# ndas7/Parallel-Systems-MPI-TFIDF

Measured on AMD Instinct MI355X. Metric: corpus GB/s (TF-IDF hot path: tokenize->TF->DF->tf*idf->ordered output), higher is better.
Workload: dtype u8/u32 (f64 score)

## Files before the change

include/tfidf.h:

```cpp
#ifndef TFIDF_H
#define TFIDF_H

#include <stdint.h>
#include <stddef.h>

#ifdef __cplusplus
extern "C" {
#endif

#define TFIDF_ABI_VERSION 2

enum tfidf_status {
    TFIDF_OK = 0,
    TFIDF_E_INVAL = -1,
    TFIDF_E_NOMEM = -2,
    TFIDF_E_HIP = -3,
    TFIDF_E_RCCL = -4,
    TFIDF_E_NODEV = -5,
    TFIDF_E_NOINPUT = -6,
    TFIDF_E_NODOC = -7,
    TFIDF_E_OUTPUT = -8,
    TFIDF_E_CAPACITY = -9,
    TFIDF_E_STATE = -10,
    TFIDF_E_PEER = -11,
// ... 36 lines not shown
typedef struct tfidf_ctx tfidf_ctx;

int tfidf_open(int device, tfidf_ctx** out);
int tfidf_device_count(void);
void tfidf_close(tfidf_ctx* ctx);
const char* tfidf_strerror(int status);
int tfidf_abi_version(void);

#define TFIDF_UNIQUE_ID_BYTES 128
int tfidf_comm_unique_id(uint8_t id[TFIDF_UNIQUE_ID_BYTES]);
int tfidf_comm_init(tfidf_ctx* ctx, const uint8_t id[TFIDF_UNIQUE_ID_BYTES], int rank, int nranks);

#define TFIDF_GROUP_LOCAL 1u
typedef struct tfidf_group tfidf_group;
int tfidf_group_open(int nranks, const int* devices, uint32_t flags, tfidf_group** out);
int tfidf_group_size(const tfidf_group* g);
tfidf_ctx* tfidf_group_ctx(tfidf_group* g, int rank);
int tfidf_group_run(tfidf_group* g, const tfidf_corpus* shards);
int tfidf_group_write_output(tfidf_group* g, const char* path);
void tfidf_group_close(tfidf_group* g);

int tfidf_run(tfidf_ctx* ctx, const tfidf_corpus* corpus);

int tfidf_fetch(tfidf_ctx* ctx, tfidf_result* out);
void tfidf_result_free(tfidf_result* r);

typedef struct tfidf_run_info {
    uint64_t size;
    uint64_t nbytes;
    uint64_t ntokens;
    uint64_t npairs;
    uint32_t nterms;
    uint32_t nterms_global;
    uint64_t nchunks;
    uint64_t partial_records;
    uint32_t ndocs;
    uint32_t vocab_capacity;
    double   ms_total;
    double   ms_tokcount;
    double   ms_stage[16];
    uint32_t nstages;
    uint32_t flags;
    uint64_t device_allocs;
    uint64_t device_alloc_bytes;
    uint64_t idf_logs;
    double   ms_idf_host;
    double   ms_idf_wait;
    uint32_t k1_workgroups;
    uint32_t reserved2;
} tfidf_run_info;
#define TFIDF_RUN_K1_VS   2u
#define TFIDF_RUN_K1_ST   4u
#define TFIDF_RUN_K1_SL   8u
#define TFIDF_RUN_XCHG_DENSE 16u
int tfidf_last_run_info(tfidf_ctx* ctx, tfidf_run_info* info);
typedef struct tfidf_run_totals {
    uint64_t runs;
    double ms_tokcount, ms_total;
    uint64_t idf_logs;
    double ms_idf_host, ms_idf_wait;
} tfidf_run_totals;
int tfidf_run_totals_get(tfidf_ctx* ctx, tfidf_run_totals* out, int reset);
int tfidf_alloc_stats(uint64_t* allocs, uint64_t* bytes);
int tfidf_alloc_live(uint64_t* allocs, uint64_t* bytes);
int tfidf_grid_cus(tfidf_ctx* ctx, uint32_t* ncu);
const char* tfidf_stage_name(int stage);
int tfidf_set_timing(tfidf_ctx* ctx, int enable);
int tfidf_debug_k1_stamps(tfidf_ctx* ctx, uint64_t* out, int n);

int tfidf_hbm_probe(tfidf_ctx* ctx, uint64_t nbytes, int iters, double* read_gbps, double* copy_gbps);


int tfidf_format(tfidf_ctx* ctx, uint64_t* nbytes);
int tfidf_copy_text(tfidf_ctx* ctx, uint64_t off, void* dst, uint64_t n);
int tfidf_write_output_gpu(tfidf_ctx* ctx, const char* path, int append);
typedef struct tfidf_output_info {
    uint64_t size;
    uint64_t text_bytes;
    uint32_t writers;
    uint32_t formatted;
    double   ms_prepare;
    double   ms_d2h_busy;
    double   ms_write;
    double   ms_total;
} tfidf_output_info;
int tfidf_last_output_info(const tfidf_ctx* ctx, tfidf_output_info* info);
int tfidf_format_f64(tfidf_ctx* ctx, const double* vals, uint64_t n, char* out);

int tfidf_write_output(const tfidf_result* r, const char* path);
int tfidf_print_jobs(const tfidf_result* r);


#define TFIDF_QUERY_MAX_K 1024u
#define TFIDF_QUERY_MAX_QUERIES 65536u
typedef struct tfidf_queries {
    const uint8_t*  bytes;
    uint64_t        nbytes;
    const uint64_t* q_off;
    uint32_t        nqueries;
} tfidf_queries;
typedef struct tfidf_hits {
    uint32_t  nqueries, k;
    uint32_t* nhits;
    uint64_t* nmatch;
    uint32_t* nterms_found;
    uint32_t* doc;
// ... 702 lines not shown
```

parallel-systems-mpi-tfidf_amd/csrc/engine.cpp:

```cpp
#include <hip/hip_runtime.h>
#include <rccl/rccl.h>

#include <float.h>
#include <math.h>
#include <stdio.h>
#include <stdlib.h>
#include <string.h>

#include <fcntl.h>
#include <sys/stat.h>
#include <time.h>
#include <unistd.h>

#include <algorithm>
#include <atomic>
#include <chrono>
#include <condition_variable>
#include <memory>
#include <mutex>
#include <string>
#include <thread>
#include <unordered_map>
#include <vector>

// ... 79 lines not shown
    }
    std::atomic_thread_fence(std::memory_order_acquire);
    return hipSuccess;
}

static hipError_t spin_sync(tfidf_ctx* ctx, hipStream_t s) {
    if (g_live_ctx.load() > 1) return hipStreamSynchronize(s);
    hipError_t e = hipEventRecord(ctx->ev_spin, s);
    if (e != hipSuccess) return e;
    while ((e = hipEventQuery(ctx->ev_spin)) == hipErrorNotReady) {
    }
    return e;
}

extern "C" {

int tfidf_device_count(void) {
    int n = 0;
    return hipGetDeviceCount(&n) == hipSuccess && n > 0 ? n : 0;
}

int tfidf_open(int device, tfidf_ctx** out) {
    if (!out) return TFIDF_E_INVAL;
    *out = nullptr;
    int n = 0;
    if (hipGetDeviceCount(&n) != hipSuccess || n <= 0 || device < 0 || device >= n) return TFIDF_E_NODEV;
    hipDeviceProp_t prop;
    if (hipGetDeviceProperties(&prop, device) != hipSuccess) return TFIDF_E_NODEV;
    if (strncmp(prop.gcnArchName, "gfx950", 6) != 0) {
        fprintf(stderr, "tfidf: device %d is %s, need gfx950\n", device, prop.gcnArchName);
        return TFIDF_E_NODEV;
    }
    if (hipSetDevice(device) != hipSuccess) return TFIDF_E_NODEV;
    std::unique_ptr<tfidf_ctx> ctx(new tfidf_ctx());
    ctx->device = device;
    const char* km = getenv("TFIDF_K1");
    if (km && !strcmp(km, "general")) ctx->k1_mode = 2;
    if (km && !strcmp(km, "vs")) ctx->k1_mode = 1;
    if (km && !strcmp(km, "sl")) ctx->k1_mode = 3;
    const char* ks = getenv("TFIDF_STAMPS");
    ctx->stamps_on = ks && ks[0] == '1';
    const char* kx = getenv("TFIDF_TEST_XFAIL_RANK");
    ctx->xfail_rank = kx ? atoi(kx) : -1;
    const char* kxm = getenv("TFIDF_XCHG");
    if (kxm && !strcmp(kxm, "owner")) ctx->xchg_mode = 1;
    if (kxm && !strcmp(kxm, "dense")) ctx->xchg_mode = 2;
    if (kxm && !strcmp(kxm, "dense_table")) ctx->xchg_mode = 3;
    const char* kxa = getenv("TFIDF_XAGG");
    ctx->xagg_table = kxa && !strcmp(kxa, "table");
    const char* kxb = getenv("TFIDF_XB_STAGE_MAX");
    ctx->xb_stage_max = kxb ? (uint32_t)atoi(kxb) : ~0u;
    const char* kds = getenv("TFIDF_DF_SPLIT");
    ctx->df_split = !(kds && !strcmp(kds, "0"));
    const char* kn = getenv("TFIDF_TEST_XNOMEM_RANK");
    ctx->xnomem_rank = kn ? atoi(kn) : -1;
    static_assert(K1_SL_MAX_CAP == 1ull << 25, "knobs.h: TFIDF_SL_MAXCAP's upper bound");
    for (int i = 0; i < KNOB_COUNT; ++i) {
        uint64_t v = 0;
        if (!knob_parse(kKnobs[i], getenv(kKnobs[i].name), &v)) continue;
        switch (i) {
            case KNOB_SL_MAXCAP: ctx->sl_maxcap = v; break;
            case KNOB_QUERY_ACC_MB: ctx->query_acc_bytes = v; break;
            case KNOB_TERMS_MB: ctx->terms_bytes = v; break;
            case KNOB_TRANSFORM_MB: ctx->transform_bytes = v; break;
            case KNOB_DEDUP_MB: ctx->dedup_bytes = v; break;
            case KNOB_NB_MB: ctx->nb_bytes = v; break;
            case KNOB_KMEANS_MB: ctx->kmeans_bytes = v; break;
            case KNOB_KMEANS_SPLIT: ctx->kmeans_split = (uint32_t)v; break;
            case KNOB_AN_GRID: ctx->an_grid = (uint32_t)v; break;
            case KNOB_GRID_CUS: ctx->grid_cus = (uint32_t)v; break;
            case KNOB_VCAP: ctx->vcap = v; break;
            case KNOB_VLOAD_BIG: ctx->vload_big_pct = (uint32_t)v; break;
            case KNOB_VLOAD: ctx->vload_pct = (uint32_t)v; break;
        }
    }
    HIPCHK(ctx->stream.create());
    HIPCHK(ctx->stream2.create());
    HIPCHK(ctx->stream3.create());
    for (Event* e : {&ctx->ev_fork, &ctx->ev_order, &ctx->ev_spin, &ctx->ev_idf_up, &ctx->ev_vrank, &ctx->ev_dfmain})
        HIPCHK(e->create_untimed());
    for (Event& e : ctx->ev) HIPCHK(e.create());
    if (arena_reset(ctx.get(), 64ull << 20) != 0) return TFIDF_E_NOMEM;
    if (ctx->counters.ensure(256) != 0) return TFIDF_E_NOMEM;
    if (ctx->hpin.alloc(256, hipHostMallocCoherent) != hipSuccess) return TFIDF_E_NOMEM;
    if (hipHostGetDevicePointer((void**)&ctx->hpin_dev, ctx->hpin, 0) != hipSuccess || !ctx->hpin_dev) return TFIDF_E_NOMEM;
    if (ctx->k1out_host.alloc(sizeof(K1Out)) != hipSuccess || ctx->k1out_dev.ensure(sizeof(K1Out)) != 0) return TFIDF_E_NOMEM;
    g_live_ctx.fetch_add(1);
    ctx->live = true;
    *out = ctx.release();
    return TFIDF_OK;
}

void tfidf_close(tfidf_ctx* ctx) {
    if (ctx) delete ctx;
}

int tfidf_set_timing(tfidf_ctx* ctx, int enable) {
    if (!ctx) return TFIDF_E_INVAL;
    ctx->timing = enable == 2 ? 2 : (enable != 0 ? 1 : 0);
    return TFIDF_OK;
}

const char* tfidf_stage_name(int stage) { return (stage >= 0 && stage < S_NSTAGES) ? kStageNames[stage] : "?"; }

int tfidf_comm_unique_id(uint8_t id[TFIDF_UNIQUE_ID_BYTES]) {
    ncclUniqueId u;
// ... 316 lines not shown
    if (!rc && any_long) {
        agreed = false;
        rc = exchange_long_check(ctx, V, bytes, &agreed);
    }
    if (rc && rc != TFIDF_E_PEER && !agreed) ctx->xp->abort();
    return rc;
}

static int enqueue_doc_order(tfidf_ctx* ctx, const uint32_t* dev_ids, uint32_t N, hipStream_t s2) {
    ENSURE(ctx->dkey0, (size_t)N * 8 + 8);
    ENSURE(ctx->dkey1, (size_t)N * 8 + 8);
    ENSURE(ctx->dseq0, (size_t)N * 4 + 4);
    ENSURE(ctx->dseq1, (size_t)N * 4 + 4);
    {
        const size_t need2 = (size_t)256 * 4 * ((N + 2047) / 2048 + 1) + (size_t)N * 20 + (1u << 20);
        if (need2 > ctx->arena2_buf.cap && ctx->arena2_buf.ensure(need2) != 0) return TFIDF_E_NOMEM;
        ctx->arena2.base = (uint8_t*)ctx->arena2_buf.p;
        ctx->arena2.cap = ctx->arena2_buf.cap;
        ctx->arena2.used = 0;
        HIPCHK(hipStreamWaitEvent(s2, ctx->ev_fork, 0));
        LCHK(launch_doc_keys(dev_ids, N, ctx->dkey0.as<uint64_t>(), ctx->dseq0.as<uint32_t>(), s2));
        int dc = N <= SORT_TILE_MAXN
            ? tile_sort_u64(ctx->dkey0.as<uint64_t>(), ctx->dseq0.as<uint32_t>(), ctx->dkey1.as<uint64_t>(),
                            ctx->dseq1.as<uint32_t>(), N, ctx->arena2, s2)
            : radix_sort_u64(ctx->dkey0.as<uint64_t>(), ctx->dseq0.as<uint32_t>(), ctx->dkey1.as<uint64_t>(),
                             ctx->dseq1.as<uint32_t>(), N, 0x1Fu, ctx->arena2, s2);
        LCHK(dc);
        ctx->order = dc ? ctx->dseq1.as<uint32_t>() : ctx->dseq0.as<uint32_t>();
        HIPCHK(hipEventRecord(ctx->ev_order, s2));
    }
    return 0;
}

static int run_local(tfidf_ctx* ctx, const CorpusDev& c, const uint32_t* dev_ids, uint64_t Nt) {
    hipStream_t s = ctx->stream;
    Arena& ar = ctx->arena;
    const uint32_t N = c.ndocs;
    ar.used = 0;
    ctx->run_N = N;
    ctx->run_V = 0;
    mark(ctx, S_PREP);
    HIPCHK(hipEventRecord(ctx->ev_fork, s));
    if (ctx->xp) {
        const size_t R = (size_t)ctx->nranks;
        ENSURE(ctx->x_cnt, ((R + 1) * (R + 4)) * 4);
    }
    const uint64_t span = c.hi - c.lo;
    const bool aligned = (((uintptr_t)c.bytes & 15u) == 0);
    ctx->k1_vs = aligned && ctx->k1_mode != 2;
    if (ctx->k1_vs && ctx->vcap > K1_VS_MAX_CAP) return TFIDF_E_CAPACITY;
    ctx->k1_sl = ctx->k1_vs && (ctx->k1_mode == 0 || ctx->k1_mode == 3) &&
                 ctx->vcap <= ctx->sl_maxcap;
    const uint32_t cb = ctx->k1_sl ? (ctx->vcap > K1_ST_MAX_CAP ? CHUNK_BYTES : CHUNK_BYTES_ST) : CHUNK_BYTES;
    const uint64_t nchunks = span ? (span + cb - 1) / cb : 0;
    if (ctx->rec_cap == 0) ctx->rec_cap = span / 6 + 4096;
    if (ctx->part_cap == 0) ctx->part_cap = span / 64 + 4096;
    ENSURE(ctx->chunk_start, (nchunks + 1) * 8);
    ENSURE(ctx->chunk_doc, (nchunks + 1) * 4);
    ENSURE(ctx->vkeys, ctx->vcap * 16);
    ENSURE(ctx->vrep, ctx->vcap * 8);
    ENSURE(ctx->rec_slot, ctx->rec_cap * 4);
    ENSURE(ctx->rec_cnt, ctx->rec_cap * 4);
    ENSURE(ctx->part_doc, ctx->part_cap * 4);
    ENSURE(ctx->part_slot, ctx->part_cap * 4);
    ENSURE(ctx->part_cnt, ctx->part_cap * 4);
    ENSURE(ctx->doc_recoff, (size_t)N * 8 + 8);
    ENSURE(ctx->doc_npairs, (size_t)N * 4 + 4);
    ENSURE(ctx->doc_size, (size_t)N * 4 + 4);
    ENSURE(ctx->doc_flags, (size_t)N + 1);
    unsigned long long* cnt = ctx->counters.as<unsigned long long>();
    {
        FillList fl{};
        auto add = [&](void* p, uint64_t bytes, uint32_t byte) {
            fl.p[fl.n] = p;
            fl.bytes[fl.n] = bytes;
            fl.val[fl.n] = byte * 0x01010101u;
            ++fl.n;
        };
        add(ctx->vkeys.p, ctx->vcap * 16, 0xEEu);
        add(cnt, 256, 0u);
        add(ctx->doc_npairs.p, (size_t)N * 4 + 4, 0u);
        add(ctx->doc_size.p, (size_t)N * 4 + 4, 0u);
        add(ctx->doc_flags.p, (size_t)N + 1, 0u);
        LCHK(launch_fill_multi(fl, s));
    }
    ENSURE(ctx->big_list, (size_t)BIG_LIST_CAP * 4);
    if (nchunks)
        LCHK(launch_plan_chunks(c, nchunks, cb, ctx->chunk_start.as<uint64_t>(), ctx->chunk_doc.as<uint32_t>(),
                                ctx->big_list.as<uint32_t>(), cnt + 6, s));
    mark(ctx, S_TOKCOUNT);
    VocabDev vd{ctx->vkeys.as<uint4>(), ctx->vrep.as<uint64_t>(), ctx->vcap - 1};
    K1Out o{};
    o.rec_slot = ctx->rec_slot.as<uint32_t>();
    o.rec_cnt = ctx->rec_cnt.as<uint32_t>();
    o.rec_alloc = cnt + 0;
    o.rec_cap = ctx->rec_cap;
    o.part_doc = ctx->part_doc.as<uint32_t>();
    o.part_slot = ctx->part_slot.as<uint32_t>();
    o.part_cnt = ctx->part_cnt.as<uint32_t>();
    o.part_alloc = cnt + 1;
    o.part_cap = ctx->part_cap;
    o.doc_recoff = ctx->doc_recoff.as<uint64_t>();
    o.doc_npairs = ctx->doc_npairs.as<uint32_t>();
    o.doc_size = ctx->doc_size.as<uint32_t>();
    o.doc_flags = ctx->doc_flags.as<uint8_t>();
    o.ntokens = cnt + 2;
    o.chunk_ctr = cnt + 5;
    o.chunk_shard = cnt + 16;
    o.status = (uint32_t*)(cnt + 3);
    o.stamps = nullptr;
    if (ctx->stamps_on) {
        ENSURE(ctx->stamps, 8 * K1_DEBUG_WORDS);
        HIPCHK(hipMemsetAsync(ctx->stamps.p, 0, 8 * K1_DEBUG_WORDS, s));
        o.stamps = ctx->stamps.as<unsigned long long>();
    }
    uint32_t k1_wgs = 0;
    if (nchunks && ctx->k1_sl) {
        if (!ctx->k1out_valid || memcmp(ctx->k1out_host, &o, sizeof(K1Out)) != 0) {
            ctx->k1out_valid = false;
            *ctx->k1out_host = o;
            HIPCHK(hipMemcpyAsync(ctx->k1out_dev.p, ctx->k1out_host, sizeof(K1Out), hipMemcpyHostToDevice, s));
            ctx->k1out_valid = true;
        }
        LCHK(launch_tokcount_sl(c, ctx->chunk_start.as<uint64_t>(), ctx->chunk_doc.as<uint32_t>(), 0, nchunks, vd,
                                ctx->k1out_dev.as<K1Out>(), s, ctx_ncu(ctx), &k1_wgs));
    } else if (nchunks && ctx->k1_vs)
        LCHK(launch_tokcount_vs(c, ctx->chunk_start.as<uint64_t>(), ctx->chunk_doc.as<uint32_t>(), 0, nchunks, vd, o, s,
                                ctx_ncu(ctx), &k1_wgs));
    else if (nchunks) {
        LCHK(launch_tokcount(c, ctx->chunk_start.as<uint64_t>(), ctx->chunk_doc.as<uint32_t>(), 0, nchunks, vd, o, s));
        k1_wgs = (uint32_t)nchunks;
    }
    ctx->k1_workgroups = k1_wgs;
    mark(ctx, S_VOCAB);
    const uint64_t cap = ctx->vcap;
    ENSURE(ctx->dense, (cap + 1) * 4);
    LCHK(launch_vocab_flags(vd, cap, ctx->dense.as<uint32_t>(), s));
    LCHK(scan_excl_u32(ctx->dense.as<uint32_t>(), ctx->dense.as<uint32_t>(), cap, ar, s));
    uint64_t* hp = ctx->hpin;
    {
        WordList wl{};
        for (int i = 0; i < 8; ++i) { wl.src[i] = cnt + i; wl.bytes[i] = 8; }
        wl.src[8] = ctx->dense.as<uint32_t>() + cap;
        wl.bytes[8] = 4;
        wl.n = 9;
        HIPCHK(words_wait(ctx, wl, 0, s));
    }
    const uint32_t V = (uint32_t)hp[8];
    unsigned long long hc[8];
    for (int i = 0; i < 8; ++i) hc[i] = hp[i];
    const uint64_t R_main = hc[0], Q = hc[1], nbig = hc[6];
    const uint32_t st = (uint32_t)hc[3];
    ctx->local_long = (st & ST_HAS_LONG) != 0;
    ctx->ntokens = hc[2];
    ctx->nchunks = nchunks;
    ctx->nrec_part = Q;
    if (st & (ST_VOCAB_SPIN | ST_TERM_LONG)) return TFIDF_E_CAPACITY;
    if (st & ST_LONG_COLLIDE) {
        fprintf(stderr, "tfidf: two distinct terms of 16 bytes or more share their 120-bit identity key\n");
        return TFIDF_E_CAPACITY;
    }
    bool retry = false;
    if (st & ST_BOUNDS) {
        fprintf(stderr, "tfidf: internal bounds check tripped in K1 (status 0x%x)\n", st);
        return TFIDF_E_STATE;
    }
    if (st & ST_VOCAB_FULL) {
        if (ctx->vcap >= K1_VS_MAX_CAP) return TFIDF_E_CAPACITY;
        ctx->vcap = ctx->vcap * 4 < K1_VS_MAX_CAP ? ctx->vcap * 4 : K1_VS_MAX_CAP;
        retry = true;
    }
    if (st & ST_REC_FULL) { ctx->rec_cap = R_main + R_main / 4 + 4096; retry = true; }
    if (st & ST_PART_FULL) { ctx->part_cap = Q + Q / 4 + 4096; retry = true; }
    if (retry) return 1;
    if (N > SORT_TILE_MAXN) {
        const int rc = enqueue_doc_order(ctx, dev_ids, N, ctx->stream2);
        if (rc) return rc;
    }
    ctx->V = V;
    if ((uint64_t)V * 100 > cap * (cap < VOCAB_LOW_LOAD_CAP ? ctx->vload_pct : ctx->vload_big_pct)) {
        while ((uint64_t)V * 100 > ctx->vcap * (ctx->vcap < VOCAB_LOW_LOAD_CAP ? ctx->vload_pct : ctx->vload_big_pct))
            ctx->vcap *= 2;
        if (ctx->vcap > K1_VS_MAX_CAP && cap < K1_VS_MAX_CAP) ctx->vcap = K1_VS_MAX_CAP;
        if (ctx->vcap != cap) return 1;
    }
    ENSURE(ctx->vslot, (size_t)V * 4 + 4);
    ENSURE(ctx->skey0, (size_t)V * 16 + 16);
    ENSURE(ctx->skey1, (size_t)V * 16 + 16);
    ENSURE(ctx->seq0, (size_t)V * 4 + 4);
    ENSURE(ctx->seq1, (size_t)V * 4 + 4);
    ENSURE(ctx->rank_of_slot, cap * 4);
    ENSURE(ctx->slot_of_rank, (size_t)V * 4 + 4);
    LCHK(launch_vocab_compact(vd, cap, ctx->dense.as<uint32_t>(), c, ctx->vslot.as<uint32_t>(), ctx->skey0.as<uint4>(),
                              ctx->seq0.as<uint32_t>(), s));
    if (V <= SORT_TILE_MAXN) {
        const int cur = tile_sort_u128(ctx->skey0.as<uint4>(), ctx->seq0.as<uint32_t>(), ctx->skey1.as<uint4>(),
                             ctx->seq1.as<uint32_t>(), V, ar, s);
        LCHK(cur);
        ctx->sorted_skey = cur ? ctx->skey1.as<uint4>() : ctx->skey0.as<uint4>();
        ctx->sorted_dense = cur ? ctx->seq1.as<uint32_t>() : ctx->seq0.as<uint32_t>();
    } else {
        uint32_t vm = 0;
        LCHK(key_varying_bytes_u128(ctx->skey0.as<uint4>(), V, &vm, ar, s));
        uint64_t* const ka = (uint64_t*)ctx->skey1.p;
        uint64_t* const kb = ka + V;
        uint32_t* const sa = ctx->seq0.as<uint32_t>();
        uint32_t* const sbq = ctx->seq1.as<uint32_t>();
        LCHK(launch_sortkey_half(ctx->skey0.as<uint4>(), V, nullptr, 1, ka, s));
        const int c1 = radix_sort_u64(ka, sa, kb, sbq, V, (vm >> 8) & 0xFFu, ar, s);
        LCHK(c1);
        ctx->sorted_dense = c1 ? sbq : sa;
        LCHK(launch_vocab_prefix_ties(c1 ? kb : ka, ctx->sorted_dense, ctx->skey0.as<uint4>(), V, vm & 0xFFu, ar, s));
        ctx->sorted_skey = nullptr;
        if (st & ST_HAS_LONG) {
            LCHK(launch_gather_u128(ctx->skey0.as<uint4>(), ctx->sorted_dense, V, ctx->skey1.as<uint4>(), s));
            ctx->sorted_skey = ctx->skey1.as<uint4>();
        }
    }
    if (st & ST_HAS_LONG)
        LCHK(launch_vocab_long_fixup(ctx->sorted_skey, ctx->sorted_dense, ctx->vslot.as<uint32_t>(), vd, c, V, ar, s));
    uint16_t* r16 = nullptr;
    if (V <= 65536u) { ENSURE(ctx->rank16, cap * 2); r16 = ctx->rank16.as<uint16_t>(); }
    LCHK(launch_vocab_rank(ctx->sorted_dense, ctx->vslot.as<uint32_t>(), V, ctx->rank_of_slot.as<uint32_t>(),
                           ctx->slot_of_rank.as<uint32_t>(), r16, s));
    if (N <= SORT_TILE_MAXN) {
        const int rc = enqueue_doc_order(ctx, dev_ids, N, ctx->stream2);
        if (rc) return rc;
    }
    const bool df_split = ctx->df_split && Q && R_main;
    ENSURE(ctx->df_local, (size_t)V * 4 + 4);
    ENSURE(ctx->df_global, (size_t)V * 4 + 4);
    if (df_split) {
        if (R_main + Q > ctx->rec_cap) {
            uint64_t ncap = R_main + Q + (R_main + Q) / 8 + 4096;
            if (ctx->rec_slot.grow_keep(ncap * 4, R_main * 4, s) || ctx->rec_cnt.grow_keep(ncap * 4, R_main * 4, s))
                return TFIDF_E_NOMEM;
            ctx->rec_cap = ncap;
        }
        const size_t dneed = df_hist_scratch(R_main, V);
        ENSURE(ctx->df_scratch, dneed > ctx->df_scratch_min ? dneed : ctx->df_scratch_min);
        Arena da;
        da.base = (uint8_t*)ctx->df_scratch.p;
        da.cap = ctx->df_scratch.cap;
        HIPCHK(hipEventRecord(ctx->ev_vrank, s));
        HIPCHK(hipStreamWaitEvent(ctx->stream2, ctx->ev_vrank, 0));
        const int dl = launch_df_hist(ctx->rec_slot.as<uint32_t>(), R_main, nullptr, R_main, ctx->rank_of_slot.as<uint32_t>(),
                                      r16, V, cap, (uint32_t*)(cnt + 3), ctx->df_local.as<uint32_t>(), da, ctx->stream2);
        if (dl == -2) {
            ctx->df_scratch_min = da.peak + da.peak / 2 + 4096;
            return 1;
        }
        LCHK(dl);
        HIPCHK(hipEventRecord(ctx->ev_dfmain, ctx->stream2));
    }
    if (ctx->idf_pool.busy && !ctx->idf_early && idf_done(ctx)) {
        idf_join(ctx);
        ENSURE(ctx->idf_vals, (size_t)(Nt + 1) * 8);
        HIPCHK(hipMemcpyAsync(ctx->idf_vals.p, ctx->idf_pin, (size_t)(Nt + 1) * 8, hipMemcpyHostToDevice,
                              ctx->stream3));
        HIPCHK(hipEventRecord(ctx->ev_idf_up, ctx->stream3));
        ctx->idf_pin_busy = true;
        ctx->idf_early = true;
    }
    mark(ctx, S_MERGE);
    uint64_t R_total = R_main;
    const uint32_t* merged_count = nullptr;
    {
        const uint64_t Qc = Q < (1ull << 20) ? (1ull << 20) : Q;
        ENSURE(ctx->pkey0, Qc * 8);
        ENSURE(ctx->pkey1, Qc * 8);
        ENSURE(ctx->pseq0, Qc * 4);
        ENSURE(ctx->pseq1, Qc * 4);
        ENSURE(ctx->phead, (Qc + 1) * 4);
    }
    if (Q) {
        if (R_main + Q > ctx->rec_cap) {
            uint64_t ncap = R_main + Q + (R_main + Q) / 8 + 4096;
            if (ctx->rec_slot.grow_keep(ncap * 4, R_main * 4, s) || ctx->rec_cnt.grow_keep(ncap * 4, R_main * 4, s))
                return TFIDF_E_NOMEM;
            ctx->rec_cap = ncap;
        }
        uint32_t nb = 0;
        if (nbig && V) {
            const uint64_t lim = (256ull << 20) / (4ull * V * DENSE_REP);
            uint64_t m = nbig < (uint64_t)BIG_LIST_CAP ? nbig : (uint64_t)BIG_LIST_CAP;
            nb = (uint32_t)(m < lim ? m : lim);
        }
        uint64_t Qs = Q;
        const uint32_t* scnt = ctx->part_cnt.as<uint32_t>();
        if (nb) {
            ENSURE(ctx->big_idx, (size_t)N * 4 + 4);
            ENSURE(ctx->dense_cnt, (size_t)nb * V * 4 * DENSE_REP);
            ENSURE(ctx->kcnt, Q * 4);
            uint32_t* nkeep = (uint32_t*)(cnt + 7);
            HIPCHK(hipMemsetAsync(ctx->big_idx.p, 0xFF, (size_t)N * 4 + 4, s));
            HIPCHK(hipMemsetAsync(ctx->dense_cnt.p, 0, (size_t)nb * V * 4 * DENSE_REP, s));
            LCHK(launch_set_big_idx(ctx->big_list.as<uint32_t>(), nb, ctx->big_idx.as<uint32_t>(), s));
            LCHK(launch_part_dense(ctx->part_doc.as<uint32_t>(), ctx->part_slot.as<uint32_t>(), ctx->part_cnt.as<uint32_t>(),
                                   Q, ctx->big_idx.as<uint32_t>(), ctx->rank_of_slot.as<uint32_t>(), V,
                                   ctx->dense_cnt.as<uint32_t>(), ctx->pkey0.as<uint64_t>(), ctx->pseq0.as<uint32_t>(),
// ... 6 lines not shown
            scnt = ctx->kcnt.as<uint32_t>();
        } else {
            LCHK(launch_part_keys(ctx->part_doc.as<uint32_t>(), ctx->part_slot.as<uint32_t>(),
                                  ctx->rank_of_slot.as<uint32_t>(), Q, ctx->pkey0.as<uint64_t>(),
                                  ctx->pseq0.as<uint32_t>(), s));
        }
        uint32_t* ph = ctx->phead.as<uint32_t>();
        if (Qs) {
            uint32_t pm = 0;
            {
                const uint32_t rb = V > 1 ? 32u - (uint32_t)__builtin_clz(V - 1) : 1u;
                const uint32_t db = N > 1 ? 32u - (uint32_t)__builtin_clz(N - 1) : 1u;
                for (uint32_t b = 0; b < (rb + 7) / 8; ++b) pm |= 1u << b;
                for (uint32_t b = 0; b < (db + 7) / 8; ++b) pm |= 1u << (4 + b);
            }
            int pc = Qs <= SORT_TILE_MAXN
                ? tile_sort_u64(ctx->pkey0.as<uint64_t>(), ctx->pseq0.as<uint32_t>(), ctx->pkey1.as<uint64_t>(),
                                ctx->pseq1.as<uint32_t>(), Qs, ar, s)
                : radix_sort_u64(ctx->pkey0.as<uint64_t>(), ctx->pseq0.as<uint32_t>(), ctx->pkey1.as<uint64_t>(),
                                 ctx->pseq1.as<uint32_t>(), Qs, pm, ar, s);
            LCHK(pc);
            uint64_t* pk = pc ? ctx->pkey1.as<uint64_t>() : ctx->pkey0.as<uint64_t>();
            uint32_t* ps = pc ? ctx->pseq1.as<uint32_t>() : ctx->pseq0.as<uint32_t>();
            LCHK(launch_part_heads(pk, Qs, ph, s));
            LCHK(scan_excl_u32(ph, ph, Qs, ar, s));
            LCHK(launch_part_merge(pk, ps, scnt, ph, Qs, ctx->slot_of_rank.as<uint32_t>(), R_main,
                                   ctx->rec_slot.as<uint32_t>(), ctx->rec_cnt.as<uint32_t>(),
                                   ctx->doc_recoff.as<uint64_t>(), ctx->doc_npairs.as<uint32_t>(),
                                   ctx->doc_flags.as<uint8_t>(), s));
        } else {
            HIPCHK(hipMemsetAsync(ph, 0, 4, s));
        }
        if (nb) {
            const uint64_t nt = ((uint64_t)V + 1023) / 1024;
            ENSURE(ctx->tile_cnt, (nt * nb + 1) * 4);
            LCHK(launch_dense_emit(ctx->dense_cnt.as<uint32_t>(), nb, V, ctx->big_list.as<uint32_t>(),
                                   ctx->slot_of_rank.as<uint32_t>(), R_main, ph + Qs, ctx->tile_cnt.as<uint32_t>(),
                                   ctx->rec_slot.as<uint32_t>(), ctx->rec_cnt.as<uint32_t>(),
                                   ctx->doc_recoff.as<uint64_t>(), ctx->doc_npairs.as<uint32_t>(),
                                   ctx->doc_flags.as<uint8_t>(), ar, s));
        }
        merged_count = ph + Qs;
        R_total = R_main + Q;
    }
    mark(ctx, S_DF);
    if (df_split) {
        HIPCHK(hipStreamWaitEvent(s, ctx->ev_dfmain, 0));
        LCHK(launch_df_hist(ctx->rec_slot.as<uint32_t>() + R_main, 0, merged_count, R_total - R_main,
                            ctx->rank_of_slot.as<uint32_t>(), r16, V, cap, (uint32_t*)(cnt + 3),
                            ctx->df_local.as<uint32_t>(), ar, s, true));
    } else {
        LCHK(launch_df_hist(ctx->rec_slot.as<uint32_t>(), R_main, merged_count, R_total,
                            ctx->rank_of_slot.as<uint32_t>(), r16, V, cap, (uint32_t*)(cnt + 3),
                            ctx->df_local.as<uint32_t>(), ar, s));
    }
    ctx->run_V = V;
    ctx->run_cap = cap;
    ctx->run_R_total = R_total;
    ctx->run_merged = merged_count;
    const size_t post_need = scan_scratch(Nt + 1) + (size_t)(Nt + 2) * 4 + 512 + scan_scratch(N) +
                             scan_scratch(3ull * ((N + 255) / 256) + 1);
    if (ar.cap - ar.used < post_need) {
        ar.peak = ar.used + post_need > ar.peak ? ar.used + post_need : ar.peak;
        return 1;
    }
    return 0;
}

#define IDF_POOL 8
static void idf_worker(tfidf_ctx::IdfPool* P, unsigned i) {
    uint64_t seen = 0;
    for (;;) {
        std::unique_lock<std::mutex> lk(P->mu);
        P->go.wait(lk, [&] { return P->stop || P->gen != seen; });
        if (P->stop) return;
        seen = P->gen;
        if (i >= P->active) continue;
        double* lut = P->lut;
        const uint32_t* vals = P->vals;
        const uint64_t Nt = P->Nt, n = P->n, lo = (n * i) / P->active, hi = (n * (i + 1)) / P->active;
        const uint32_t mode = P->mode;
        const auto t0 = P->t0;
        lk.unlock();
        if (mode != TFIDF_IDF_REF) {
            if (vals)
                for (uint64_t k = lo; k < hi; ++k) lut[k] = tfidf_weight_idf(mode, Nt, vals[k]);
            else
                for (uint64_t d = lo + 1; d < hi + 1; ++d) lut[d] = tfidf_weight_idf(mode, Nt, (uint32_t)d);
        } else if (vals)
            for (uint64_t k = lo; k < hi; ++k) lut[k] = log(1.0 * (double)Nt / (double)vals[k]);
        else
            for (uint64_t d = lo + 1; d < hi + 1; ++d) lut[d] = log(1.0 * (double)Nt / (double)d);
        const int64_t e = std::chrono::duration_cast<std::chrono::nanoseconds>(std::chrono::steady_clock::now() - t0).count();
        lk.lock();
        P->end_ns = e > P->end_ns ? e : P->end_ns;
        if (--P->left == 0) P->done.notify_all();
    }
}
static void idf_pool_stop(tfidf_ctx* ctx) {
    tfidf_ctx::IdfPool& P = ctx->idf_pool;
    {
        std::unique_lock<std::mutex> lk(P.mu);
        P.done.wait(lk, [&] { return P.left == 0; });
        P.stop = true;
    }
    P.go.notify_all();
    for (auto& t : P.th) t.join();
// ... 117 lines not shown
        if (idf_pin_reserve(ctx, (size_t)K + 1)) return TFIDF_E_NOMEM;
        if (K) {
            if (K < 2 * 16384) {
                const auto t0 = std::chrono::steady_clock::now();
                for (uint32_t k = 0; k < K; ++k) ctx->idf_pin[k] = log(1.0 * (double)Nt / (double)vals[k]);
                ctx->ms_idf_host = std::chrono::duration<double, std::milli>(std::chrono::steady_clock::now() - t0).count();
            } else {
                idf_post(ctx, ctx->idf_pin, Nt, vals.data(), K);
                idf_join(ctx);
            }
            HIPCHK(hipMemcpyAsync(ctx->idf_vals.p, ctx->idf_pin, (size_t)K * 8, hipMemcpyHostToDevice, s));
            ctx->idf_pin_busy = true;
        }
        ctx->idf_logs = K;
    }
    const uint64_t Pmax = R_total;
    mark(ctx, S_SCORE);
    ENSURE(ctx->out_term, Pmax * 4 + 4);
    ENSURE(ctx->out_cnt, Pmax * 4 + 4);
    ENSURE(ctx->out_score, Pmax * 8 + 8);
    ENSURE(ctx->idf_rank, (size_t)V * 8 + 8);
    ENSURE(ctx->large_list, (size_t)N * 8 + 16);
    K5Args a{};
    a.order = ctx->order;
    a.meta = ctx->doc_meta.as<uint4>();
    a.out_off = ctx->out_off.as<uint64_t>();
    a.doc_recoff = ctx->doc_recoff.as<uint64_t>();
    a.doc_npairs = ctx->doc_npairs.as<uint32_t>();
    a.doc_size = ctx->doc_size.as<uint32_t>();
    a.doc_flags = ctx->doc_flags.as<uint8_t>();
    a.rec_slot = ctx->rec_slot.as<uint32_t>();
    a.rec_cnt = ctx->rec_cnt.as<uint32_t>();
    a.rank_of_slot = ctx->rank_of_slot.as<uint32_t>();
    a.df_of_rank = df_of_run(ctx);
    a.idf_idx = full_lut ? nullptr : ctx->present.as<uint32_t>();
    a.idf = ctx->idf_vals.as<double>();
    a.idf_rank = ctx->idf_rank.as<double>();
    a.idf_by_df = (full_lut && V > (1u << 21)) ? 1u : 0u;
    a.large_list = ctx->large_list.as<uint32_t>() + 1;
    a.large_count = ctx->large_list.as<uint32_t>();
    a.cls_nblk = (N + 255) / 256;
    a.cls_list = ctx->large_list.as<uint32_t>() + N + 2;
    ENSURE(ctx->cls_off, ((size_t)3 * a.cls_nblk + 8) * 4);
    a.cls_off = ctx->cls_off.as<uint32_t>();
    {
        const uint64_t cap_t = 2 * R_total / 4096 + 64;
        ENSURE(ctx->split_tasks, cap_t * 8 + 8);
        a.split_count = ctx->split_tasks.as<uint32_t>();
        a.split_tasks = ctx->split_tasks.as<uint2>() + 1;
        a.split_cap = (uint32_t)(cap_t < 0xFFFFFFFFull ? cap_t : 0xFFFFFFFFull);
    }
    a.ndocs = N;
    a.nterms = V;
    a.rank_bits = V > 1 ? 32u - (uint32_t)__builtin_clz(V - 1) : 1u;
    a.rec_total = R_total;
    a.slot_cap = cap;
    a.status = (uint32_t*)(cnt + 3);
    a.out_term = ctx->out_term.as<uint32_t>();
    a.out_cnt = ctx->out_cnt.as<uint32_t>();
    a.out_score = ctx->out_score.as<double>();
    XCHK(launch_score_order(a, ar, s, ctx->stream2, ctx->ev_fork, ctx->ev_order, ctx_ncu(ctx)));
    mark(ctx, S_NSTAGES);
    {
        WordList wl{};
        wl.src[0] = cnt + 3;
        wl.bytes[0] = 4;
        wl.src[1] = ctx->out_off.as<uint64_t>() + N;
        wl.bytes[1] = 8;
        wl.src[2] = cnt + 12;
        wl.bytes[2] = 4;
        wl.n = ctx->xp ? 3 : 2;
        if (ctx->xp) {
            XCHK(launch_words_to_host(wl, ctx->hpin_dev + 24, s));
            XSYNC(s);
        } else {
            HIPCHK(words_wait(ctx, wl, 24, s));
        }
    }
    ctx->idf_pin_busy = false;
    const uint32_t st_end = (uint32_t)ctx->hpin[24];
    const uint64_t P = ctx->hpin[25];
    ctx->npairs = P;
    if (ctx->xp) ctx->Vg = (uint32_t)ctx->hpin[26];
    if (st_end & ST_BOUNDS) {
        fprintf(stderr, "tfidf: internal bounds check tripped (status 0x%x)\n", st_end);
        return TFIDF_E_STATE;
    }
    return 0;
}

static int run_once(tfidf_ctx* ctx, const CorpusDev& c, const uint32_t* dev_ids, uint64_t Nt) {
    int rc = run_local(ctx, c, dev_ids, Nt);
    mark(ctx, S_EXCHANGE);
    if (ctx->xp) {
        rc = exchange_df(ctx, rc, ctx->run_V, c.bytes);
        if (rc) return rc;
    } else {
        if (rc) return rc;
        ctx->Vg = ctx->run_V;
    }
    return run_post(ctx, Nt);
}

static int run_prepare(tfidf_ctx* ctx, const tfidf_corpus* in, CorpusDev& c, const uint32_t*& dev_ids, uint64_t& Nt) {
    if (in->ndocs && !in->doc_off) return TFIDF_E_INVAL;
    if (in->nbytes && !in->bytes) return TFIDF_E_INVAL;
    HIPCHK(hipSetDevice(ctx->device));
// ... 160 lines not shown
    }
    if (!rc) {
        *read_gbps = ms_r > 0 ? (double)nbytes * iters / (ms_r * 1e-3) / 1e9 : 0.0;
        *copy_gbps = ms_c > 0 ? 2.0 * (double)nbytes * iters / (ms_c * 1e-3) / 1e9 : 0.0;
    }
    (void)hipEventDestroy(e0);
    (void)hipEventDestroy(e1);
    (void)hipStreamSynchronize(s);
    return rc;
}

extern "C" int tfidf_grid_cus(tfidf_ctx* ctx, uint32_t* ncu) {
    if (!ctx || !ncu) return TFIDF_E_INVAL;
    *ncu = ctx_ncu(ctx);
    return TFIDF_OK;
}

extern "C" int tfidf_alloc_stats(uint64_t* allocs, uint64_t* bytes) {
    if (!allocs || !bytes) return TFIDF_E_INVAL;
    *allocs = g_dev_allocs.load(std::memory_order_relaxed);
    *bytes = g_dev_alloc_bytes.load(std::memory_order_relaxed);
    return TFIDF_OK;
}

extern "C" int tfidf_alloc_live(uint64_t* allocs, uint64_t* bytes) {
    if (!allocs || !bytes) return TFIDF_E_INVAL;
    *allocs = g_dev_allocs.load(std::memory_order_relaxed) - g_dev_frees.load(std::memory_order_relaxed);
    *bytes = g_dev_alloc_bytes.load(std::memory_order_relaxed) - g_dev_free_bytes.load(std::memory_order_relaxed);
    return TFIDF_OK;
}

extern "C" int tfidf_last_run_info(tfidf_ctx* ctx, tfidf_run_info* out) {
    tfidf_run_info* info = out;
    if (!ctx || !info || info->size < 16) return TFIDF_E_INVAL;
    if (!ctx->have_info) return TFIDF_E_STATE;
    const size_t want = info->size < sizeof(tfidf_run_info) ? (size_t)info->size : sizeof(tfidf_run_info);
    tfidf_run_info full;
    memset(&full, 0, sizeof(full));
    info = &full;
    info->nbytes = ctx->run_nbytes;
    info->ntokens = ctx->ntokens;
    info->npairs = ctx->info_npairs;
    info->nterms = ctx->info_V;
    info->nterms_global = ctx->Vg;
    info->nchunks = ctx->nchunks;
    info->partial_records = ctx->nrec_part;
    info->ndocs = ctx->ndocs;
    info->vocab_capacity = (uint32_t)ctx->vcap;
    info->ms_total = ctx->ms_total;
    info->ms_tokcount = ctx->ms_stage[S_TOKCOUNT];
    for (int i = 0; i < S_NSTAGES; ++i) info->ms_stage[i] = ctx->ms_stage[i];
    info->nstages = S_NSTAGES;
    info->flags = (ctx->k1_vs ? TFIDF_RUN_K1_VS : 0u) | (ctx->k1_sl ? TFIDF_RUN_K1_SL : 0u) |
                  (ctx->xp && ctx->last_dense ? TFIDF_RUN_XCHG_DENSE : 0u);
    info->device_allocs = g_dev_allocs.load(std::memory_order_relaxed);
    info->device_alloc_bytes = g_dev_alloc_bytes.load(std::memory_order_relaxed);
    info->idf_logs = ctx->idf_logs;
    info->ms_idf_host = ctx->ms_idf_host;
    info->ms_idf_wait = ctx->ms_idf_wait;
    info->k1_workgroups = ctx->k1_workgroups;
    full.size = want;
    memcpy(out, &full, want);
    return TFIDF_OK;
}


extern "C" void tfidf_result_free(tfidf_result* r) {
    if (!r) return;
    free(r->pair_doc); free(r->pair_term); free(r->pair_count); free(r->pair_docsize); free(r->pair_df);
    free(r->pair_score); free(r->doc_id); free(r->doc_size); free(r->term_off); free(r->term_bytes);
    free(r->term_df);
    memset(r, 0, sizeof(*r));
}

extern "C" int tfidf_fetch(tfidf_ctx* ctx, tfidf_result* r) {
    if (!ctx || !r) return TFIDF_E_INVAL;
    if (!ctx->have_result) return TFIDF_E_STATE;
    HIPCHK(hipSetDevice(ctx->device));
    hipStream_t s = ctx->stream;
    memset(r, 0, sizeof(*r));
    const uint64_t P = ctx->npairs;
    const uint32_t N = ctx->ndocs, V = ctx->V;
    r->npairs = P;
    r->ndocs = N;
    r->nterms = V;
    r->ndocs_total = ctx->ndocs_total;
    size_t p4 = (size_t)P * 4 + 4;
    r->pair_doc = (uint32_t*)malloc(p4);
    r->pair_term = (uint32_t*)malloc(p4);
    r->pair_count = (uint32_t*)malloc(p4);
    r->pair_docsize = (uint32_t*)malloc(p4);
    r->pair_df = (uint32_t*)malloc(p4);
    r->pair_score = (double*)malloc((size_t)P * 8 + 8);
    r->doc_id = (uint32_t*)malloc((size_t)N * 4 + 4);
    r->doc_size = (uint32_t*)malloc((size_t)N * 4 + 4);
    r->term_df = (uint32_t*)malloc((size_t)V * 4 + 4);
    r->term_off = (uint64_t*)malloc(((size_t)V + 1) * 8);
    if (!r->pair_doc || !r->pair_term || !r->pair_count || !r->pair_docsize || !r->pair_df || !r->pair_score ||
        !r->doc_id || !r->doc_size || !r->term_df || !r->term_off) {
        tfidf_result_free(r);
        return TFIDF_E_NOMEM;
    }
    std::vector<uint32_t> order(N);
    std::vector<uint64_t> ooff((size_t)N + 1);
    if (P) {
        HIPCHK(hipMemcpyAsync(r->pair_term, ctx->out_term.p, P * 4, hipMemcpyDeviceToHost, s));
// ... 380 lines not shown
```

parallel-systems-mpi-tfidf_amd/csrc/engine_ctx.h:

```cpp
#ifndef TFIDF_ENGINE_CTX_H
#define TFIDF_ENGINE_CTX_H

#include <hip/hip_runtime.h>

#include <stdio.h>
#include <stdlib.h>
#include <string.h>

#include <chrono>
#include <condition_variable>
#include <mutex>
#include <thread>
#include <vector>

#include "../../include/tfidf.h"
#include "kernels.h"
#include "xport.h"
#include "devbuf.h"

struct Stream {
    hipStream_t s = nullptr;
    Stream() = default;
    Stream(const Stream&) = delete;
    Stream& operator=(const Stream&) = delete;
// ... 13 lines not shown
};
template <typename T> struct Pinned {
    T* p = nullptr;
    Pinned() = default;
    Pinned(const Pinned&) = delete;
    Pinned& operator=(const Pinned&) = delete;
    ~Pinned() { release(); }
    operator T*() const { return p; }
    T* operator->() const { return p; }
    hipError_t alloc(size_t bytes, unsigned flags = hipHostMallocDefault) {
        release();
        const hipError_t e = hipHostMalloc((void**)&p, bytes, flags);
        if (e != hipSuccess) p = nullptr;
        return e;
    }
    void release() {
        if (p) (void)hipHostFree(p);
        p = nullptr;
    }
};
enum Stage { S_PREP, S_TOKCOUNT, S_VOCAB, S_MERGE, S_DF, S_EXCHANGE, S_IDF, S_ORDER, S_SCORE, S_NSTAGES };

struct tfidf_ctx {
    ~tfidf_ctx();
    bool live = false;
    int device = 0;
    Stream stream;
    Xport* xp = nullptr;
    int rank = 0, nranks = 1;
    int timing = 1;
    int k1_mode = 0;
    bool stamps_on = false;
    int xfail_rank = -1;
    int xnomem_rank = -1;
    DevBuf stamps;
    bool k1_vs = false;
    bool k1_sl = false;
    uint64_t sl_maxcap = K1_SL_MAX_CAP;
    Pinned<K1Out> k1out_host;
    DevBuf k1out_dev;
    bool k1out_valid = false;
    Event ev[S_NSTAGES + 1];
    Arena arena;
    DevBuf arena_buf;
    Stream stream2;
    Event ev_fork, ev_order;
    Event ev_spin;
    uint64_t wait_token = 0;
    Stream stream3;
    Event ev_idf_up;
    bool idf_early = false;
    bool df_split = true;
    Event ev_vrank, ev_dfmain;
    DevBuf df_scratch;
    size_t df_scratch_min = 0;
    Arena arena2;
    DevBuf arena2_buf;
    DevBuf in_bytes, in_off, in_ids;
    DevBuf syn_bytes, syn_off, syn_ids, syn_ntok, syn_blkfirst, syn_blkbytes, syn_cdf;
    DevBuf chunk_start, chunk_doc;
    DevBuf vkeys, vrep;
    uint64_t vcap = 1ull << 20;
#define VOCAB_LOW_LOAD_CAP (1ull << 24)
#define IDF_FULL_MAX (1ull << 18)
    uint32_t vload_pct = 12;
    uint32_t vload_big_pct = 45;
    DevBuf rec_slot, rec_cnt;
    uint64_t rec_cap = 0;
    DevBuf part_doc, part_slot, part_cnt;
    uint64_t part_cap = 0;
    DevBuf doc_recoff, doc_npairs, doc_size, doc_flags;
    DevBuf counters;
    Pinned<uint64_t> hpin;
    uint64_t* hpin_dev = nullptr;
    DevBuf dense, vslot, skey0, skey1, seq0, seq1, rank_of_slot, slot_of_rank, rank16;
    DevBuf pkey0, pkey1, pseq0, pseq1, phead;
    DevBuf big_list, big_idx, dense_cnt, kcnt, tile_cnt;
    DevBuf df_local, df_global, present, idf_vals;
    uint64_t idf_full_n = 0;
    Pinned<double> idf_pin;
    size_t idf_pin_n = 0;
    bool idf_pin_busy = false;
    struct IdfPool {
        std::mutex mu;
        std::condition_variable go, done;
        std::vector<std::thread> th;
        uint64_t gen = 0;
        bool stop = false, busy = false;
        unsigned active = 0, left = 0;
        double* lut = nullptr;
        uint64_t Nt = 0;
        const uint32_t* vals = nullptr;
        uint64_t n = 0;
        uint32_t mode = 0;
        std::chrono::steady_clock::time_point t0;
        int64_t end_ns = 0;
    } idf_pool;
    uint64_t idf_logs = 0;
    tfidf_run_totals totals{};
    double ms_idf_host = 0, ms_idf_wait = 0;
    DevBuf dkey0, dkey1, dseq0, dseq1, npairs_ord, out_off, doc_meta;
    DevBuf out_term, out_cnt, out_score, idf_rank, large_list, split_tasks, cls_off;
    DevBuf x_mine, x_srec, x_sidx, x_back, x_cnt;
    DevBuf x_rrec, x_rslot, x_reply, x_tkey, x_tdf;
    DevBuf x_gkeys, x_pos, x_dense;
    DevBuf x_lloc, x_lsend, x_lgath, x_ltab;
// ... 298 lines not shown
```

parallel-systems-mpi-tfidf_amd/csrc/finalize.hip:

```cpp
#include "dev_common.h"
#include "dev_vocab.h"
#include "kernels.h"
#include "synth.h"

#include <type_traits>
#define G(p) ((GLOBAL_AS std::remove_pointer_t<decltype(p)>*)(p))
template <class T> __device__ __forceinline__ void sto(T* p, T v) { *(GLOBAL_AS T*)p = v; }

namespace {
constexpr int NT = 256;
inline unsigned grid_for(uint64_t n, int nt = NT) { return n ? (unsigned)((n + nt - 1) / nt) : 1u; }
inline int ok() { return hipGetLastError() == hipSuccess ? 0 : -1; }

__device__ __forceinline__ uint4 u128_from(uint64_t lo, uint64_t hi) {
    return make_uint4((uint32_t)lo, (uint32_t)(lo >> 32), (uint32_t)hi, (uint32_t)(hi >> 32));
}
__device__ __forceinline__ bool u128_eq(uint4 a, uint4 b) { return a.x == b.x && a.y == b.y && a.z == b.z && a.w == b.w; }
}


__global__ void k_vocab_flags(VocabDev v, uint64_t cap, uint32_t* __restrict__ flags) {
    uint64_t s = (uint64_t)blockIdx.x * blockDim.x + threadIdx.x;
    if (s >= cap) return;
    uint4 k = v.keys[s];
// ... 585 lines not shown
    uint32_t v[4], c = 0;
#pragma unroll
    for (int k = 0; k < 4; ++k) {
        v[k] = r0 + k < V ? dense_sum(dense, b, V, r0 + k) : 0u;
        c += v[k] ? 1u : 0u;
    }
    uint32_t tot;
    uint32_t o = block_excl_scan<NT, false>(c, wsum, &tot);
    const uint64_t base = rec_base + *merged_count + tile_off[(uint64_t)b * nt + t];
#pragma unroll
    for (int k = 0; k < 4; ++k)
        if (v[k]) { rec_slot[base + o] = r0 + k; rec_cnt[base + o] = v[k]; ++o; }
    if (t == 0 && threadIdx.x == 0) {
        const uint32_t d = big_list[b];
        const uint64_t first = tile_off[(uint64_t)b * nt], last = tile_off[(uint64_t)(b + 1) * nt];
        doc_recoff[d] = rec_base + *merged_count + first;
        doc_npairs[d] = (uint32_t)(last - first);
        doc_flags[d] = DF_PARTIAL | DF_PRESORTED;
    }
}
__global__ void k_add_count(uint32_t* __restrict__ merged_count, const uint32_t* __restrict__ add) {
    merged_count[0] += add[0];
}
int launch_dense_emit(const uint32_t* dense, uint32_t nb, uint32_t V, const uint32_t* big_list,
                      const uint32_t* slot_of_rank, uint64_t rec_base, uint32_t* merged_count, uint32_t* tile_cnt,
                      uint32_t* rec_slot, uint32_t* rec_cnt, uint64_t* doc_recoff, uint32_t* doc_npairs,
                      uint8_t* doc_flags, Arena& ar, hipStream_t s) {
    if (!nb || !V) return 0;
    const uint32_t nt = (V + DENSE_TILE - 1) / DENSE_TILE;
    const dim3 grid(nt, nb);
    k_dense_count<<<grid, NT, 0, s>>>(dense, V, nt, tile_cnt);
    if (ok()) return -1;
    if (scan_excl_u32(tile_cnt, tile_cnt, (uint64_t)nt * nb, ar, s)) return -1;
    k_dense_write<<<grid, NT, 0, s>>>(dense, V, nt, big_list, slot_of_rank, rec_base, merged_count, tile_cnt, rec_slot,
                                      rec_cnt, doc_recoff, doc_npairs, doc_flags);
    if (ok()) return -1;
    k_add_count<<<1, 1, 0, s>>>(merged_count, tile_cnt + (uint64_t)nt * nb);
    return ok();
}


constexpr uint32_t DFH_ROUNDS = 4;

constexpr int DFH_NT = 1024;
#ifndef DFH_B_N
#define DFH_B_N 16
#endif
constexpr int DFH_B = DFH_B_N;
#ifndef DFH_CK_BITS
#define DFH_CK_BITS 12
#endif
constexpr uint32_t DFH_CK = 1u << DFH_CK_BITS;
__device__ __forceinline__ uint32_t dfh_cslot(uint32_t slot) { return (slot * 0x9E3779B1u) >> (32 - DFH_CK_BITS); }
template <bool WIDE>
__global__ __launch_bounds__(DFH_NT) void k_df_hist_lds(uint32_t* __restrict__ rec_slot, uint64_t nrec,
                                                        const uint32_t* __restrict__ nrec_extra,
                                                        const uint32_t* __restrict__ rank_of_slot,
                                                        const uint16_t* __restrict__ rank16, uint32_t V,
                                                        uint64_t slot_cap, uint64_t ranked_from,
                                                        uint32_t* __restrict__ status, uint64_t per,
                                                        uint32_t* __restrict__ part ,
                                                        uint32_t* __restrict__ df) {
    extern __shared__ __attribute__((aligned(16))) uint32_t bins[];
    const uint32_t W = (V + 1) / 2;
    for (uint32_t k = threadIdx.x; k < W; k += DFH_NT) bins[k] = 0;
    unsigned long long* cache = reinterpret_cast<unsigned long long*>(bins + ((W + 1) & ~1u));
    for (uint32_t k = threadIdx.x; k < DFH_CK; k += DFH_NT) cache[k] = 0ull;
    __syncthreads();
    if (nrec_extra) nrec += *nrec_extra;
    const uint64_t r0 = (uint64_t)blockIdx.x * per;
    const uint64_t r1 = r0 + per < nrec ? r0 + per : nrec;
    const uint32_t nr = r1 > r0 ? (uint32_t)(r1 - r0) : 0u;
    const uint32_t rk = ranked_from <= r0 ? 0u : ranked_from - r0 >= nr ? nr : (uint32_t)(ranked_from - r0);
    const __amdgpu_buffer_rsrc_t rs = __builtin_amdgcn_make_buffer_rsrc((void*)(rec_slot + r0), 0, (int)(nr * 4u),
                                                                        0x00020000);
    const __amdgpu_buffer_rsrc_t ms = __builtin_amdgcn_make_buffer_rsrc(
        rank16 ? (void*)rank16 : (void*)rank_of_slot, 0,
        (int)(slot_cap * (rank16 ? 2u : 4u) < 0x7FFFFFF0ull ? slot_cap * (rank16 ? 2u : 4u) : 0x7FFFFFF0ull), 0x00020000);
    uint32_t rp[DFH_B];
    uint32_t pofs = 0xFFFFFFF0u;
    uint32_t pvalid = 0;
#pragma unroll
    for (int q = 0; q < DFH_B; ++q) rp[q] = 0u;
    auto store_prev = [&]() {
#pragma unroll
        for (int q = 0; q < DFH_B; ++q)
            __builtin_amdgcn_raw_buffer_store_b32(rp[q], rs,
                                                  ((pvalid >> q) & 1u) ? pofs + (uint32_t)q * DFH_NT * 4u : 0xFFFFFFF0u,
                                                  0, 2 );
    };
    for (uint32_t j = threadIdx.x; j < nr; j += (uint32_t)DFH_B * DFH_NT) {
        uint32_t sl[DFH_B], r[DFH_B], g[DFH_B];
        const uint32_t ofs = j * 4u;
#pragma unroll
        for (int q = 0; q < DFH_B; ++q) {
            const uint32_t v = __builtin_amdgcn_raw_buffer_load_b32(rs, ofs + (uint32_t)q * DFH_NT * 4u, 0, 2 );
            sl[q] = j + (uint32_t)q * DFH_NT < nr ? v : 0xFFFFFFFFu;
        }
        store_prev();
        uint32_t miss = 0;
#pragma unroll
        for (int q = 0; q < DFH_B; ++q) {
            const bool ranked = j + (uint32_t)q * DFH_NT >= rk;
            if (sl[q] != 0xFFFFFFFFu && sl[q] >= (ranked ? (uint64_t)V : slot_cap)) {
                atomicOr(status, ST_BOUNDS);
                sl[q] = 0xFFFFFFFFu;
            }
            const unsigned long long e = cache[dfh_cslot(sl[q])];
            const bool hit = (uint32_t)(e >> 32) == sl[q] + 1u;
            const bool need = sl[q] != 0xFFFFFFFFu && !ranked && !hit;
            miss |= need ? 1u << q : 0u;
            r[q] = ranked ? sl[q] : (uint32_t)e;
        }
        if (rank16) {
#pragma unroll
            for (int q = 0; q < DFH_B; ++q)
                g[q] = __builtin_amdgcn_raw_buffer_load_b16(ms, ((miss >> q) & 1u) ? sl[q] * 2u : 0u, 0, 0);
        } else {
#pragma unroll
            for (int q = 0; q < DFH_B; ++q)
                g[q] = __builtin_amdgcn_raw_buffer_load_b32(ms, ((miss >> q) & 1u) ? sl[q] * 4u : 0u, 0, 0);
        }
#pragma unroll
        for (int q = 0; q < DFH_B; ++q) {
            if ((miss >> q) & 1u) {
                r[q] = g[q];
                cache[dfh_cslot(sl[q])] = ((unsigned long long)(sl[q] + 1u) << 32) | r[q];
            }
        }
        pvalid = 0;
#pragma unroll
        for (int q = 0; q < DFH_B; ++q) {
            rp[q] = r[q];
            pvalid |= sl[q] != 0xFFFFFFFFu && j + (uint32_t)q * DFH_NT < rk ? 1u << q : 0u;
            if (sl[q] == 0xFFFFFFFFu) continue;
            const uint32_t sh = 16 * (r[q] & 1);
            if (WIDE) {
                const uint32_t old = atomicAdd(&bins[r[q] >> 1], 1u << sh);
                if (((old >> sh) & 0xFFFFu) == 0x7FFFu) {
                    atomicSub(&bins[r[q] >> 1], 0x8000u << sh);
                    atomicAdd(&df[r[q]], 0x8000u);
                }
            } else {
                atomicAdd(&bins[r[q] >> 1], 1u << sh);
            }
        }
        pofs = ofs;
    }
    store_prev();
    __syncthreads();
    uint32_t* out = part + (uint64_t)blockIdx.x * W;
    for (uint32_t k = threadIdx.x; k < W; k += DFH_NT) out[k] = bins[k];
}
constexpr uint32_t DFC_G = 32;
__global__ void k_df_colsum(const uint32_t* __restrict__ part, uint32_t nparts, uint32_t V, uint32_t* __restrict__ df) {
    const uint32_t r = blockIdx.x * blockDim.x + threadIdx.x;
    if (r >= V) return;
    const uint32_t W = (V + 1) / 2, sh = 16 * (r & 1);
    const uint32_t p0 = blockIdx.y * DFC_G;
    uint32_t v[DFC_G];
#pragma unroll
    for (uint32_t q = 0; q < DFC_G; ++q)
        v[q] = p0 + q < nparts ? part[(uint64_t)(p0 + q) * W + (r >> 1)] : 0u;
    uint32_t sum = 0;
#pragma unroll
    for (uint32_t q = 0; q < DFC_G; ++q) sum += (v[q] >> sh) & 0xFFFFu;
    if (sum) atomicAdd(&df[r], sum);
}
constexpr int DFA_B = 8;
__global__ void k_df_hist_atomic(uint32_t* __restrict__ rec_slot, uint64_t nrec, const uint32_t* __restrict__ nrec_extra,
                                 const uint32_t* __restrict__ rank_of_slot, uint64_t slot_cap, uint64_t ranked_from,
                                 uint32_t V, uint32_t* __restrict__ status, uint32_t* __restrict__ df) {
    if (nrec_extra) nrec += *nrec_extra;
    const uint64_t stride = (uint64_t)gridDim.x * blockDim.x;
    for (uint64_t i0 = (uint64_t)blockIdx.x * blockDim.x + threadIdx.x; i0 < nrec; i0 += stride * DFA_B) {
        uint32_t sl[DFA_B], r[DFA_B];
#pragma unroll
        for (int k = 0; k < DFA_B; ++k) {
            const uint64_t i = i0 + (uint64_t)k * stride;
            sl[k] = i < nrec ? rec_slot[i] : 0xFFFFFFFFu;
        }
#pragma unroll
        for (int k = 0; k < DFA_B; ++k) {
            const bool ranked = i0 + (uint64_t)k * stride >= ranked_from;
            r[k] = ranked ? sl[k] : sl[k] < slot_cap ? rank_of_slot[sl[k]] : 0xFFFFFFFFu;
        }
// ... 80 lines not shown
    for (uint32_t i0 = b + threadIdx.x; i0 < e; i0 += B * DFS_NT) {
        uint32_t r[B];
#pragma unroll
        for (int q = 0; q < B; ++q) r[q] = i0 + q * DFS_NT < e ? part[i0 + q * DFS_NT] : 0xFFFFFFFFu;
#pragma unroll
        for (int q = 0; q < B; ++q)
            if (r[q] != 0xFFFFFFFFu) atomicAdd(&sbins[r[q] - s0], 1u);
    }
    __syncthreads();
    for (uint32_t j = threadIdx.x; j < sw; j += DFS_NT) df[s0 + j] = accumulate ? df[s0 + j] + sbins[j] : sbins[j];
}

static void df_lds_plan(uint64_t nrec_max, uint32_t V, uint64_t* per_out, uint32_t* nparts_out) {
    uint64_t nparts = (nrec_max + DFH_RECS - 1) / DFH_RECS;
    const uint32_t W = (V + 1) / 2;
    static int ncu = 0;
    if (!ncu) {
        int dev = 0;
        if (hipGetDevice(&dev) != hipSuccess ||
            hipDeviceGetAttribute(&ncu, hipDeviceAttributeMultiprocessorCount, dev) != hipSuccess || ncu <= 0)
            ncu = 256;
    }
    const uint64_t wg_lds = (uint64_t)((W + 1) & ~1u) * 4 + (uint64_t)DFH_CK * 8;
    const uint64_t per_cu = (uint64_t)163840 / wg_lds >= 2 ? 2 : 1;
    const uint64_t slots = (uint64_t)ncu * per_cu;
    uint64_t full = (nparts + slots - 1) / slots * slots;
    if (full > DFH_ROUNDS * slots) full = slots;
    const char* fe = getenv("TFIDF_DF_WGS");
    const uint64_t forced = fe ? strtoull(fe, nullptr, 0) : 0ull;
    if (forced >= 1 && forced <= (1u << 20)) full = forced;
    uint64_t per = (nrec_max + full - 1) / full;
    if (per < 8192u && !forced) per = 8192u;
    if (per > (1u << 28)) per = 1u << 28;
    if (per == 0) per = 1;
    *per_out = per;
    *nparts_out = (uint32_t)((nrec_max + per - 1) / per);
}

size_t df_hist_scratch(uint64_t nrec_max, uint32_t V) {
    if (V == 0 || nrec_max == 0) return 256;
    if (V <= DFH_MAXV) {
        uint64_t per = 0;
        uint32_t nparts = 0;
        df_lds_plan(nrec_max, V, &per, &nparts);
        return (size_t)nparts * ((V + 1) / 2) * 4 + 256;
    }
    const uint64_t nsl = ((uint64_t)V + DFS_SLICE - 1) / DFS_SLICE;
    const uint64_t ntiles = (nrec_max + DFS_TILE - 1) / DFS_TILE;
    return (size_t)((ntiles * nsl + 1) * 4 + nrec_max * 4 + (ntiles * nsl) / 16 + 8192 + 1024);
}

int launch_df_hist(uint32_t* rec_slot, uint64_t nrec, const uint32_t* nrec_extra, uint64_t nrec_max,
                   const uint32_t* rank_of_slot, const uint16_t* rank16, uint32_t V, uint64_t slot_cap,
                   uint32_t* status, uint32_t* df, Arena& ar, hipStream_t s, bool accumulate) {
    const uint64_t ranked_from = nrec;
    if (V == 0) return 0;
    if (nrec_max < nrec) nrec_max = nrec;
    if (nrec_max == 0)
        return accumulate ? 0 : hipMemsetAsync(df, 0, (size_t)V * 4, s) == hipSuccess ? 0 : -1;
    if (V <= DFH_MAXV) {
        uint64_t per = 0;
        uint32_t nparts = 0;
        df_lds_plan(nrec_max, V, &per, &nparts);
        const uint32_t W = (V + 1) / 2;
        size_t m = ar.mark();
        uint32_t* part = (uint32_t*)ar.get((size_t)nparts * W * 4);
        if (!part) return -2;
        if (!accumulate && hipMemsetAsync(df, 0, (size_t)V * 4, s) != hipSuccess) return -1;
        const size_t lds = (size_t)((W + 1) & ~1u) * 4 + (size_t)DFH_CK * 8;
        if (per > DFH_RECS)
            k_df_hist_lds<true><<<nparts, DFH_NT, lds, s>>>(rec_slot, nrec, nrec_extra, rank_of_slot, rank16, V,
                                                            slot_cap, ranked_from, status, per, part, df);
        else
            k_df_hist_lds<false><<<nparts, DFH_NT, lds, s>>>(rec_slot, nrec, nrec_extra, rank_of_slot, rank16, V,
                                                             slot_cap, ranked_from, status, per, part, df);
        k_df_colsum<<<dim3(grid_for(V), (nparts + DFC_G - 1) / DFC_G), NT, 0, s>>>(part, nparts, V, df);
        ar.release(m);
        return ok();
    }
    {
        const uint32_t nsl = (uint32_t)(((uint64_t)V + DFS_SLICE - 1) / DFS_SLICE);
        const uint64_t ntiles = (nrec_max + DFS_TILE - 1) / DFS_TILE;
        if (nsl <= DFS_MAXSL && nrec_max < (1ull << 32) && ntiles * nsl < (1ull << 31)) {
            size_t m = ar.mark();
            uint32_t* cnt = (uint32_t*)ar.get((size_t)(ntiles * nsl + 1) * 4);
            uint32_t* part = (uint32_t*)ar.get((size_t)nrec_max * 4);
            if (!cnt || !part) return -2;
            {
                k_dfs_count<<<(uint32_t)ntiles, DFS_NT, 0, s>>>(rec_slot, nrec, nrec_extra, rank_of_slot, slot_cap,
                                                               ranked_from, V, nsl, status, cnt);
                if (ok()) return -1;
                if (scan_excl_u32(cnt, cnt, ntiles * nsl, ar, s)) return -1;
                k_dfs_scatter<<<(uint32_t)ntiles, DFS_NT, 0, s>>>(rec_slot, nrec, nrec_extra, V, nsl, cnt, part);
                if (ok()) return -1;
                k_dfs_slice<<<nsl, DFS_NT, (size_t)(V < DFS_SLICE ? V : DFS_SLICE) * 4, s>>>(part, cnt, (uint32_t)ntiles,
                                                                                           V, df, accumulate);
                ar.release(m);
                return ok();
            }
        }
    }
    if (!accumulate && hipMemsetAsync(df, 0, (size_t)V * 4, s) != hipSuccess) return -1;
    k_df_hist_atomic<<<4096, NT, 0, s>>>(rec_slot, nrec, nrec_extra, rank_of_slot, slot_cap, ranked_from, V, status,
                                         df);
    return ok();
}

__global__ void k_df_mark(const uint32_t* __restrict__ df, uint32_t V, uint32_t* __restrict__ present) {
    uint32_t r = blockIdx.x * blockDim.x + threadIdx.x;
    if (r < V) present[df[r]] = 1u;
}
int launch_df_mark(const uint32_t* df, uint32_t V, uint32_t* present, hipStream_t s) {
    if (!V) return 0;
    k_df_mark<<<grid_for(V), NT, 0, s>>>(df, V, present);
    return ok();
}
__global__ void k_df_list(const uint32_t* __restrict__ ps, uint64_t nvals, uint32_t* __restrict__ vals) {
    const uint64_t stride = (uint64_t)gridDim.x * blockDim.x;
    for (uint64_t x = (uint64_t)blockIdx.x * blockDim.x + threadIdx.x; x < nvals; x += stride)
        if (ps[x + 1] != ps[x]) vals[ps[x]] = (uint32_t)x;
}
int launch_df_list(const uint32_t* present_scan, uint64_t nvals, uint32_t* vals, hipStream_t s) {
    const unsigned full = grid_for(nvals), cap = 1u << 20;
    k_df_list<<<full < cap ? full : cap, NT, 0, s>>>(present_scan, nvals, vals);
    return ok();
}


__global__ void k_doc_keys(const uint32_t* __restrict__ ids, uint32_t n, uint64_t* __restrict__ keys,
                           uint32_t* __restrict__ seq) {
    uint32_t i = blockIdx.x * blockDim.x + threadIdx.x;
    if (i >= n) return;
    uint32_t id = ids ? ids[i] : i + 1;
    uint32_t dg[10];
    int k = 0;
    do { dg[k++] = id % 10; id /= 10; } while (id);
    uint64_t key = 0;
    for (int p = 0; p < 10; ++p) key = key * 11 + (p < k ? dg[k - 1 - p] : 10u);
    keys[i] = key;
    seq[i] = i;
}
int launch_doc_keys(const uint32_t* doc_ids, uint32_t ndocs, uint64_t* keys, uint32_t* seq, hipStream_t s) {
    if (!ndocs) return 0;
    k_doc_keys<<<grid_for(ndocs), NT, 0, s>>>(doc_ids, ndocs, keys, seq);
    return ok();
}
__global__ void k_gather_meta(const uint32_t* __restrict__ order, const uint32_t* __restrict__ np,
                              const uint64_t* __restrict__ recoff, const uint32_t* __restrict__ dsize,
                              const uint8_t* __restrict__ flags, uint32_t n, uint64_t* __restrict__ out,
                              uint4* __restrict__ meta) {
    uint32_t i = blockIdx.x * blockDim.x + threadIdx.x;
    if (i >= n) return;
    const uint32_t d = order[i];
    const uint32_t c = np[d];
    const uint64_t rb = c ? recoff[d] : 0ull;
    out[i] = c;
    meta[i] = make_uint4((uint32_t)rb, (uint32_t)(rb >> 32), (c & 0x3FFFFFFFu) | ((uint32_t)(flags[d] & 3u) << 30), dsize[d]);
}
int launch_gather_meta(const uint32_t* order, const uint32_t* doc_npairs, const uint64_t* doc_recoff,
                       const uint32_t* doc_size, const uint8_t* doc_flags, uint32_t ndocs, uint64_t* npairs_ord,
// ... 6 lines not shown


constexpr int K5_MAX = K5_MAX_PAIRS;
constexpr uint32_t K5_SMALL = 64;
constexpr int K5_BATCH = 8;
#ifndef K5_EB
#define K5_EB 4
#endif
#ifndef K5_EMIT
#define K5_EMIT 2
#endif
#ifndef K5_WPS
#define K5_WPS 4
#endif
#ifndef K5_WPS_WIDE
#define K5_WPS_WIDE 4
#endif
constexpr uint32_t K5_NB = 1u << K5_NB_BITS;
#ifndef K5L_EB
#define K5L_EB 8
#endif

__global__ void k_idf_of_rank(const uint32_t* __restrict__ df_of_rank, const uint32_t* __restrict__ idf_idx,
                              const double* __restrict__ idf, uint32_t V, double* __restrict__ out) {
    uint32_t r = blockIdx.x * blockDim.x + threadIdx.x;
    if (r < V) out[r] = idf_idx ? idf[idf_idx[df_of_rank[r]]] : idf[df_of_rank[r]];
}

template <bool BYDF>
__device__ __forceinline__ double k5_idf(const K5Args& a, uint32_t r) {
    if constexpr (BYDF) return G(a.idf)[G(a.df_of_rank)[r]];
    else return G(a.idf_rank)[r];
}

template <bool BYDF>
__device__ __forceinline__ void k5_emit(const K5Args& a, uint64_t o, double ds, uint32_t rank, uint32_t cnt) {
    const double tf = (double)cnt / ds;
    sto(&a.out_term[o], (uint32_t)(rank));
    sto(&a.out_cnt[o], (uint32_t)(cnt));
    sto(&a.out_score[o], (double)(tf * k5_idf<BYDF>(a, rank)));
}

__device__ __forceinline__ uint32_t k5_rank(const K5Args& a, uint32_t r) {
    if (r >= a.nterms) { atomicOr(a.status, ST_BOUNDS); r = 0; }
    return r;
}

constexpr uint32_t K5_WIDE_BITS = 32 - K5_IDX_BITS + K5_NB_BITS;
__device__ __forceinline__ bool k5_by_wave(const K5Args& a, uint32_t n, bool presorted) {
    if (presorted) return n <= K5_WAVE;
    return n <= K5_SMALL || (n <= K5_WAVE && a.rank_bits <= K5_WIDE_BITS);
}

__device__ __noinline__ void k5_radix(uint32_t rank_bits, const uint32_t* rec_cnt, const double* idf_rank,
                                      uint32_t* out_term, uint32_t* out_cnt, double* out_score, uint32_t* buf0,
                                      uint32_t* buf1, uint32_t* h, uint32_t n, uint64_t rb, uint64_t ob, double ds) {
    const uint32_t lane = threadIdx.x & 63;
    const uint64_t below = (1ull << lane) - 1ull;
    uint32_t cur = 0;
    for (uint32_t sh = K5_IDX_BITS; sh < K5_IDX_BITS + rank_bits; sh += 8) {
        const uint32_t* src = cur ? buf1 : buf0;
        uint32_t* dst = cur ? buf0 : buf1;
        h[4 * lane] = 0; h[4 * lane + 1] = 0; h[4 * lane + 2] = 0; h[4 * lane + 3] = 0;
        __builtin_amdgcn_fence(__ATOMIC_RELEASE, "wavefront");
        __builtin_amdgcn_fence(__ATOMIC_ACQUIRE, "wavefront");
        for (uint32_t j = lane; j < n; j += 64) atomicAdd(&h[(src[j] >> sh) & 0xFFu], 1u);
        __builtin_amdgcn_fence(__ATOMIC_RELEASE, "wavefront");
        __builtin_amdgcn_fence(__ATOMIC_ACQUIRE, "wavefront");
        {
            const uint32_t v0 = h[4 * lane], v1 = h[4 * lane + 1], v2 = h[4 * lane + 2], v3 = h[4 * lane + 3];
            const uint32_t tot = v0 + v1 + v2 + v3;
            const uint32_t ex = wave_incl_scan(tot) - tot;
            h[4 * lane] = ex; h[4 * lane + 1] = ex + v0; h[4 * lane + 2] = ex + v0 + v1; h[4 * lane + 3] = ex + v0 + v1 + v2;
        }
        __builtin_amdgcn_fence(__ATOMIC_RELEASE, "wavefront");
        __builtin_amdgcn_fence(__ATOMIC_ACQUIRE, "wavefront");
        for (uint32_t r0 = 0; r0 < n; r0 += 64) {
            const uint32_t j = r0 + lane;
            const bool valid = j < n;
            const uint32_t key = valid ? src[j] : 0u;
            const uint32_t dg = (key >> sh) & 0xFFu;
            uint64_t m = __ballot(valid);
#pragma unroll
            for (int b = 0; b < 8; ++b) {
                const bool bit = (dg >> b) & 1u;
                const uint64_t bb = __ballot(valid && bit);
                m &= bit ? bb : ~bb;
            }
            const uint32_t lrank = (uint32_t)__popcll(m & below);
            const uint32_t cnt = (uint32_t)__popcll(m);
            const uint32_t base = valid ? h[dg] : 0u;
            __builtin_amdgcn_fence(__ATOMIC_RELEASE, "wavefront");
            __builtin_amdgcn_fence(__ATOMIC_ACQUIRE, "wavefront");
            if (valid) {
                dst[base + lrank] = key;
                if (lrank == cnt - 1u) h[dg] = base + cnt;
            }
            __builtin_amdgcn_fence(__ATOMIC_RELEASE, "wavefront");
            __builtin_amdgcn_fence(__ATOMIC_ACQUIRE, "wavefront");
        }
        cur ^= 1u;
    }
    const uint32_t* fin = cur ? buf1 : buf0;
    for (uint32_t j0 = 0; j0 < n; j0 += 64 * K5_BATCH) {
        uint32_t key[K5_BATCH], cnt[K5_BATCH];
        double idf[K5_BATCH];
#pragma unroll
        for (int q = 0; q < K5_BATCH; ++q) {
            const uint32_t j = j0 + 64 * q + lane;
            key[q] = j < n ? fin[j] : 0u;
        }
#pragma unroll
        for (int q = 0; q < K5_BATCH; ++q) {
            cnt[q] = rec_cnt[rb + (key[q] & ((1u << K5_IDX_BITS) - 1u))];
            idf[q] = G(idf_rank)[key[q] >> K5_IDX_BITS];
        }
#pragma unroll
        for (int q = 0; q < K5_BATCH; ++q) {
            const uint32_t j = j0 + 64 * q + lane;
            if (j < n) {
                sto(&out_term[ob + j], (uint32_t)(key[q] >> K5_IDX_BITS));
                sto(&out_cnt[ob + j], (uint32_t)(cnt[q]));
                sto(&out_score[ob + j], (double)(((double)cnt[q] / ds) * idf[q]));
            }
        }
    }
}

constexpr int K5_PF = 8;
constexpr int K5_RQ = K5_WAVE / 64;
__device__ __forceinline__ void k5_prefetch(const K5Args& a, const uint4& m, uint32_t lane, uint32_t (&s)[K5_PF],
                                            uint32_t (&c)[K5_PF]) {
    const uint32_t n = m.z & 0x3FFFFFFFu;
    const uint64_t rb = ((uint64_t)m.y << 32) | m.x;
    const bool ok = n != 0u && n <= K5_WAVE && rb + n <= a.rec_total;
#pragma unroll
    for (int q = 0; q < K5_PF; ++q) {
        const uint32_t j = 64u * q + lane;
        const bool v = ok && j < n;
        s[q] = v ? a.rec_slot[rb + j] : 0u;
        c[q] = v ? a.rec_cnt[rb + j] : 0u;
    }
}

__device__ __forceinline__ uint32_t lane_id_fresh() {
    uint32_t l;
    asm volatile("v_mbcnt_lo_u32_b32 %0, -1, 0\n\tv_mbcnt_hi_u32_b32 %0, -1, %0" : "=v"(l));
    return l;
}

template <bool WIDE, bool BYDF>
__global__ __launch_bounds__(NT, WIDE ? K5_WPS_WIDE : K5_WPS) void k_score_wave(K5Args a) {
    static_assert(WIDE || !BYDF, "idf by df only with wide ranks (V > 2^21; k5_radix reads idf by rank)");
    __shared__ __attribute__((aligned(16))) uint32_t kb[NT / 64][2][K5_WAVE];
    __shared__ uint32_t hist[NT / 64][K5_NB];
    const uint32_t w = threadIdx.x >> 6, lane = threadIdx.x & 63;
    const uint32_t stride = gridDim.x * (NT / 64);
    uint32_t* buf0 = kb[w][0];
    uint32_t* buf1 = kb[w][1];
    uint32_t* h = hist[w];
    const uint32_t* L = nullptr;
    uint32_t lcount = a.ndocs;
    if (a.cls_list) {
        const uint32_t lo = G(a.cls_off)[a.cls_nblk];
        L = a.cls_list + lo;
        lcount = G(a.cls_off)[2 * a.cls_nblk] - lo;
    }
    auto pos_of = [&](uint32_t li) -> uint32_t { return L ? G(L)[li] : li; };
    uint32_t li = blockIdx.x * (NT / 64) + w;
    uint32_t i_cur = li < lcount ? pos_of(li) : 0u;
    uint32_t i_nxt = li + stride < lcount ? pos_of(li + stride) : 0u;
    uint4 m_cur = li < lcount ? gload(a.meta + (i_cur)) : make_uint4(0, 0, 0, 0);
    uint4 m_nxt = li + stride < lcount ? gload(a.meta + (i_nxt)) : make_uint4(0, 0, 0, 0);
    uint64_t ob_cur = li < lcount ? G(a.out_off)[i_cur] : 0ull;
    uint32_t s_cur[K5_PF], c_cur[K5_PF];
    k5_prefetch(a, m_cur, lane, s_cur, c_cur);
    for (; li < lcount; li += stride) {
        const uint32_t lane = lane_id_fresh();
        const uint32_t i = i_cur;
        const uint4 mc = m_cur;
        const uint64_t ob = ob_cur;
        const uint32_t n = mc.z & 0x3FFFFFFFu;
        const bool presorted = ((mc.z >> 30) & DF_PRESORTED) != 0;
        const uint64_t rb = ((uint64_t)mc.y << 32) | mc.x;
        const double ds = (double)mc.w;
        const bool small_doc = n != 0u && k5_by_wave(a, n, presorted) && rb + n <= a.rec_total;
        uint32_t r[K5_RQ];
#pragma unroll
        for (int q = 0; q < K5_PF; ++q) {
            const uint32_t j = 64u * q + lane;
            r[q] = (small_doc && j < n) ? k5_rank(a, s_cur[q]) : 0xFFFFFFFFu;
            if (small_doc && j < n) buf0[j] = c_cur[q];
        }
        if (small_doc && n > 64u * K5_PF) {
            uint32_t sx[K5_RQ - K5_PF];
#pragma unroll
            for (int q = K5_PF; q < K5_RQ; ++q) {
                const uint32_t j = 64u * q + lane;
                sx[q - K5_PF] = j < n ? a.rec_slot[rb + j] : 0u;
                if (j < n) buf0[j] = a.rec_cnt[rb + j];
            }
#pragma unroll
            for (int q = K5_PF; q < K5_RQ; ++q) {
                const uint32_t j = 64u * q + lane;
                r[q] = j < n ? k5_rank(a, sx[q - K5_PF]) : 0xFFFFFFFFu;
            }
        } else {
#pragma unroll
            for (int q = K5_PF; q < K5_RQ; ++q) r[q] = 0xFFFFFFFFu;
        }
        __builtin_amdgcn_fence(__ATOMIC_RELEASE, "wavefront");
        __builtin_amdgcn_fence(__ATOMIC_ACQUIRE, "wavefront");
        {
            const uint32_t inx = li + stride;
            m_cur = m_nxt;
            i_cur = i_nxt;
            ob_cur = inx < lcount ? G(a.out_off)[i_cur] : 0ull;
            i_nxt = inx + stride < lcount ? pos_of(inx + stride) : 0u;
            m_nxt = inx + stride < lcount ? gload(a.meta + (i_nxt)) : make_uint4(0, 0, 0, 0);
            k5_prefetch(a, m_cur, lane, s_cur, c_cur);
        }
        if (n == 0) continue;
        if (!k5_by_wave(a, n, presorted)) {
            if (WIDE && lane == 0) G(a.large_list)[atomicAdd(a.large_count, 1u)] = i;
            continue;
        }
        if (rb + n > a.rec_total) { if (lane == 0) atomicOr(a.status, ST_BOUNDS); continue; }
        if (presorted) {
#pragma unroll
            for (int q = 0; q < K5_RQ; ++q) {
                const uint32_t j = 64u * q + lane;
                if (j < n) k5_emit<BYDF>(a, ob + j, ds, r[q], buf0[j]);
            }
            continue;
        }
#ifndef K5_CNT
#define K5_CNT 128
#endif
        if (n <= (uint32_t)K5_CNT) {
            constexpr int QC = K5_CNT / 64;
#pragma unroll
            for (int q = 0; q < QC; ++q) {
                const uint32_t j = 64u * q + lane;
                if (j < n) buf1[j] = r[q];
            }
            const uint32_t n4 = (n + 3u) & ~3u;
            if (lane < 4u && n + lane < n4) buf1[n + lane] = 0xFFFFFFFFu;
            __builtin_amdgcn_fence(__ATOMIC_RELEASE, "wavefront");
            __builtin_amdgcn_fence(__ATOMIC_ACQUIRE, "wavefront");
            uint32_t pos[QC];
#pragma unroll
            for (int q = 0; q < QC; ++q) pos[q] = 0u;
            const uint4* k4p = reinterpret_cast<const uint4*>(buf1);
            for (uint32_t i4 = 0; i4 < n4 / 4u; ++i4) {
                const uint4 k4 = k4p[i4];
#pragma unroll
                for (int q = 0; q < QC; ++q)
                    pos[q] += (k4.x < r[q] ? 1u : 0u) + (k4.y < r[q] ? 1u : 0u) + (k4.z < r[q] ? 1u : 0u) +
                              (k4.w < r[q] ? 1u : 0u);
            }
            double idf[QC];
#pragma unroll
            for (int q = 0; q < QC; ++q) idf[q] = (64u * q + lane < n) ? k5_idf<BYDF>(a, r[q]) : 0.0;
#pragma unroll
            for (int q = 0; q < QC; ++q) {
                const uint32_t j = 64u * q + lane;
                if (j < n) {
                    const uint64_t o = ob + pos[q];
                    const uint32_t cnt = buf0[j];
                    sto(&a.out_term[o], (uint32_t)(r[q]));
                    sto(&a.out_cnt[o], (uint32_t)(cnt));
                    sto(&a.out_score[o], (double)(((double)cnt / ds) * idf[q]));
                }
            }
            __builtin_amdgcn_fence(__ATOMIC_RELEASE, "wavefront");
            __builtin_amdgcn_fence(__ATOMIC_ACQUIRE, "wavefront");
            continue;
        }
        if (n <= K5_SMALL) {
            uint32_t key = r[0], val = lane < n ? buf0[lane] : 0u;
#pragma unroll
            for (uint32_t k = 2; k <= 64; k <<= 1) {
#pragma unroll
                for (uint32_t j = k >> 1; j > 0; j >>= 1) {
                    uint32_t pk = __shfl_xor(key, j, 64), pv = __shfl_xor(val, j, 64);
                    bool take_min = ((lane & k) == 0) == ((lane & j) == 0);
                    if (take_min ? (pk < key) : (pk > key)) { key = pk; val = pv; }
                }
            }
            if (lane < n) k5_emit<BYDF>(a, ob + lane, ds, key, val);
            continue;
        }
        const uint32_t hsh = a.rank_bits > K5_NB_BITS ? a.rank_bits - K5_NB_BITS : 0u;
#pragma unroll
        for (uint32_t q = 0; q < K5_NB / 64; ++q) h[q * 64 + lane] = 0;
        __builtin_amdgcn_fence(__ATOMIC_RELEASE, "wavefront");
        __builtin_amdgcn_fence(__ATOMIC_ACQUIRE, "wavefront");
#pragma unroll
        for (int q = 0; q < K5_RQ; ++q)
            if (64u * q + lane < n) atomicAdd(&h[r[q] >> hsh], 1u);
        __builtin_amdgcn_fence(__ATOMIC_RELEASE, "wavefront");
        __builtin_amdgcn_fence(__ATOMIC_ACQUIRE, "wavefront");
        uint32_t gmax;
        {
            constexpr uint32_t PER = K5_NB / 64;
            uint32_t v[PER], tot = 0, mx = 0;
#pragma unroll
            for (uint32_t q = 0; q < PER; ++q) { v[q] = h[lane * PER + q]; tot += v[q]; mx = v[q] > mx ? v[q] : mx; }
            uint32_t run = wave_incl_scan(tot) - tot;
#pragma unroll
            for (uint32_t q = 0; q < PER; ++q) { h[lane * PER + q] = run; run += v[q]; }
            gmax = wave_max(mx);
        }
        __builtin_amdgcn_fence(__ATOMIC_RELEASE, "wavefront");
        __builtin_amdgcn_fence(__ATOMIC_ACQUIRE, "wavefront");
        const bool wide = WIDE;
        if (gmax > K5_GROUP_MAX && wide) {
            if (lane == 0) G(a.large_list)[atomicAdd(a.large_count, 1u)] = i;
            continue;
        }
        if constexpr (WIDE) if (wide) {
            const uint32_t lm = (1u << hsh) - 1u;
#pragma unroll
            for (int q = 0; q < K5_RQ; ++q) {
                const uint32_t j = 64u * q + lane;
                if (j < n) buf1[atomicAdd(&h[r[q] >> hsh], 1u)] = ((r[q] & lm) << K5_IDX_BITS) | j;
            }
            __builtin_amdgcn_fence(__ATOMIC_RELEASE, "wavefront");
            __builtin_amdgcn_fence(__ATOMIC_ACQUIRE, "wavefront");
            constexpr int EB = K5_EB;
#pragma unroll
            for (int q0 = 0; q0 < K5_RQ; q0 += EB) {
                if (64u * q0 >= n) continue;
                uint32_t pos[EB], cnt[EB];
                double idf[EB];
#pragma unroll
                for (int e = 0; e < EB; ++e) {
                    const uint32_t j = 64u * (q0 + e) + lane;
                    const uint32_t rk = r[q0 + e];
                    pos[e] = 0u;
                    cnt[e] = 0u;
                    if (j < n) {
                        const uint32_t d = rk >> hsh, k = ((rk & lm) << K5_IDX_BITS) | j;
                        const uint32_t gs = d ? h[d - 1] : 0u, ge = h[d];
                        uint32_t less = 0;
                        for (uint32_t f = gs; f < ge; ++f) less += buf1[f] < k ? 1u : 0u;
                        pos[e] = gs + less;
                        cnt[e] = buf0[j];
                    }
                    idf[e] = j < n ? k5_idf<BYDF>(a, rk) : 0.0;
                }
#pragma unroll
                for (int e = 0; e < EB; ++e) {
                    if (64u * (q0 + e) + lane < n) {
                        const uint64_t o = ob + pos[e];
                        sto(&a.out_term[o], (uint32_t)(r[q0 + e]));
                        sto(&a.out_cnt[o], (uint32_t)(cnt[e]));
                        sto(&a.out_score[o], (double)(((double)cnt[e] / ds) * idf[e]));
                    }
                }
            }
            __builtin_amdgcn_fence(__ATOMIC_RELEASE, "wavefront");
            __builtin_amdgcn_fence(__ATOMIC_ACQUIRE, "wavefront");
            continue;
        }
        if (gmax > K5_GROUP_MAX) {
#pragma unroll
            for (int q = 0; q < K5_RQ; ++q) {
                const uint32_t j = 64u * q + lane;
                if (j < n) buf0[j] = (r[q] << K5_IDX_BITS) | j;
            }
            __builtin_amdgcn_fence(__ATOMIC_RELEASE, "wavefront");
            __builtin_amdgcn_fence(__ATOMIC_ACQUIRE, "wavefront");
            if constexpr (!WIDE)
                k5_radix(a.rank_bits, a.rec_cnt, a.idf_rank, a.out_term, a.out_cnt, a.out_score, buf0, buf1, h, n,
                         rb, ob, ds);
            continue;
        }
#pragma unroll
        for (int q = 0; q < K5_RQ; ++q) {
            const uint32_t j = 64u * q + lane;
            if (j < n) buf1[atomicAdd(&h[r[q] >> hsh], 1u)] = (r[q] << K5_IDX_BITS) | j;
        }
        __builtin_amdgcn_fence(__ATOMIC_RELEASE, "wavefront");
        __builtin_amdgcn_fence(__ATOMIC_ACQUIRE, "wavefront");
        uint32_t pp[K5_RQ];
#pragma unroll
        for (int q = 0; q < K5_RQ; ++q) {
            const uint32_t j = 64u * q + lane;
            pp[q] = 0u;
            if (j < n) {
                const uint32_t k = (r[q] << K5_IDX_BITS) | j, d = r[q] >> hsh;
                const uint32_t gs = d ? h[d - 1] : 0u, ge = h[d];
                uint32_t less = 0;
                for (uint32_t f = gs; f < ge; ++f) less += buf1[f] < k ? 1u : 0u;
                pp[q] = gs + less;
            }
        }
        __builtin_amdgcn_fence(__ATOMIC_RELEASE, "wavefront");
        __builtin_amdgcn_fence(__ATOMIC_ACQUIRE, "wavefront");
#pragma unroll
        for (int q = 0; q < K5_RQ; ++q)
            if (64u * q + lane < n) buf1[pp[q]] = (r[q] << K5_IDX_BITS) | (64u * q + lane);
        __builtin_amdgcn_fence(__ATOMIC_RELEASE, "wavefront");
        __builtin_amdgcn_fence(__ATOMIC_ACQUIRE, "wavefront");
        constexpr int EB = K5_EMIT;
        for (uint32_t j0 = 0; j0 < n; j0 += 64 * EB) {
            double idf[EB];
#pragma unroll
            for (int q = 0; q < EB; ++q) {
                const uint32_t j = j0 + 64 * q + lane;
                idf[q] = k5_idf<BYDF>(a, (j < n ? buf1[j] : 0u) >> K5_IDX_BITS);
            }
#pragma unroll
            for (int q = 0; q < EB; ++q) {
                const uint32_t j = j0 + 64 * q + lane;
                if (j < n) {
                    const uint32_t key = buf1[j], cnt = buf0[key & ((1u << K5_IDX_BITS) - 1u)];
                    sto(&a.out_term[ob + j], (uint32_t)(key >> K5_IDX_BITS));
                    sto(&a.out_cnt[ob + j], (uint32_t)(cnt));
                    sto(&a.out_score[ob + j], (double)(((double)cnt / ds) * idf[q]));
                }
            }
        }
        __builtin_amdgcn_fence(__ATOMIC_RELEASE, "wavefront");
        __builtin_amdgcn_fence(__ATOMIC_ACQUIRE, "wavefront");
    }
}

template <uint32_t MAXN, uint32_t NBB, bool BYDF>
__global__ __launch_bounds__(NT) void k_score_large(K5Args a) {
    constexpr uint32_t NB = 1u << NBB;
    __shared__ uint32_t kbuf[2][MAXN];
    __shared__ uint32_t vbuf[2][MAXN];
    union Scratch {
        struct {
            uint32_t hist[256], run[256];
            uint32_t wcnt[NT / 64][256];
        } r;
        uint32_t bh[NB];
    };
    __shared__ Scratch U;
    uint32_t (&hist)[256] = U.r.hist;
    uint32_t (&run)[256] = U.r.run;
    uint32_t (&wcnt)[NT / 64][256] = U.r.wcnt;
    uint32_t (&bh)[NB] = U.bh;
    __shared__ uint32_t wsum[NT / 64];
    __shared__ uint32_t bmax;
    const uint32_t tid = threadIdx.x, lane = tid & 63, w = tid >> 6;
    const uint32_t* LL = a.large_list;
    uint32_t nlarge;
    if (a.cls_list) {
        const uint32_t lo = G(a.cls_off)[2 * a.cls_nblk];
        LL = a.cls_list + lo;
        nlarge = G(a.cls_off)[3 * a.cls_nblk] - lo;
    } else {
        nlarge = *a.large_count;
    }
    for (uint32_t li = blockIdx.x; li < nlarge; li += gridDim.x) {
    const uint32_t i = G(LL)[li];
    const uint32_t d = G(a.order)[i];
    const uint32_t n = G(a.doc_npairs)[d];
    const bool presorted = (G(a.doc_flags)[d] & DF_PRESORTED) != 0;
    if (MAXN < (uint32_t)K5_MAX ? (!presorted && n > MAXN) : (presorted || n <= (uint32_t)K5_MAX / 2)) continue;
    const uint64_t ob = G(a.out_off)[i], rb = G(a.doc_recoff)[d];
    const double ds = (double)G(a.doc_size)[d];
    if (rb + n > a.rec_total) {
        if (tid == 0) atomicOr(a.status, ST_BOUNDS);
        continue;
    }
    if (presorted || n > (uint32_t)K5_MAX) {
        if (n > (uint32_t)K5_MAX && !presorted) { if (tid == 0) atomicOr(a.status, ST_BOUNDS); continue; }
        for (uint32_t j0 = 0; j0 < n; j0 += NT * K5L_EB) {
            uint32_t rk[K5L_EB], cn[K5L_EB];
            double f[K5L_EB];
#pragma unroll
            for (int e = 0; e < K5L_EB; ++e) {
                const uint32_t j = j0 + NT * e + tid;
                rk[e] = j < n ? a.rec_slot[rb + j] : 0u;
                cn[e] = j < n ? a.rec_cnt[rb + j] : 0u;
            }
#pragma unroll
            for (int e = 0; e < K5L_EB; ++e) {
                const uint32_t j = j0 + NT * e + tid;
                if (j < n) rk[e] = k5_rank(a, rk[e]);
                f[e] = j < n ? k5_idf<BYDF>(a, rk[e]) : 0.0;
            }
#pragma unroll
            for (int e = 0; e < K5L_EB; ++e) {
                const uint32_t j = j0 + NT * e + tid;
                if (j < n) {
                    sto(&a.out_term[ob + j], (uint32_t)(rk[e]));
                    sto(&a.out_cnt[ob + j], (uint32_t)(cn[e]));
                    sto(&a.out_score[ob + j], (double)(((double)cn[e] / ds) * f[e]));
                }
            }
        }
        continue;
    }
    for (uint32_t j0 = 0; j0 < n; j0 += NT * K5L_EB) {
        uint32_t sl[K5L_EB], cn[K5L_EB];
#pragma unroll
        for (int e = 0; e < K5L_EB; ++e) {
            const uint32_t j = j0 + NT * e + tid;
            sl[e] = j < n ? a.rec_slot[rb + j] : 0u;
            cn[e] = j < n ? a.rec_cnt[rb + j] : 0u;
        }
#pragma unroll
        for (int e = 0; e < K5L_EB; ++e) {
            const uint32_t j = j0 + NT * e + tid;
            if (j < n) {
                kbuf[0][j] = k5_rank(a, sl[e]);
                vbuf[0][j] = cn[e];
            }
        }
    }
    {
        const uint32_t hsh = a.rank_bits > NBB ? a.rank_bits - NBB : 0u;
        for (uint32_t q = tid; q < NB; q += NT) bh[q] = 0u;
        if (tid == 0) bmax = 0u;
        __syncthreads();
        for (uint32_t j = tid; j < n; j += NT) atomicAdd(&bh[kbuf[0][j] >> hsh], 1u);
        __syncthreads();
        constexpr uint32_t PER = NB / NT;
        uint32_t v[PER], tot = 0, mx = 0;
#pragma unroll
        for (uint32_t q = 0; q < PER; ++q) { v[q] = bh[tid * PER + q]; tot += v[q]; mx = v[q] > mx ? v[q] : mx; }
        uint32_t all;
        uint32_t run = block_excl_scan<NT>(tot, wsum, &all);
#pragma unroll
        for (uint32_t q = 0; q < PER; ++q) { bh[tid * PER + q] = run; run += v[q]; }
        mx = wave_max(mx);
        if (lane == 0) atomicMax(&bmax, mx);
        __syncthreads();
        if (bmax <= K5L_GROUP_MAX) {
            for (uint32_t j = tid; j < n; j += NT) {
                const uint32_t k = kbuf[0][j];
                const uint32_t q = atomicAdd(&bh[k >> hsh], 1u);
                kbuf[1][q] = k;
                vbuf[1][q] = j;
            }
            __syncthreads();
            for (uint32_t p0 = 0; p0 < n; p0 += NT * K5L_EB) {
                uint32_t kk[K5L_EB], ps[K5L_EB], cn[K5L_EB];
                double f[K5L_EB];
#pragma unroll
                for (int e = 0; e < K5L_EB; ++e) {
                    const uint32_t p = p0 + NT * e + tid;
                    kk[e] = 0u; ps[e] = 0u; cn[e] = 0u;
                    if (p < n) {
                        const uint32_t k = kbuf[1][p], d = k >> hsh;
                        const uint32_t gs = d ? bh[d - 1] : 0u, ge = bh[d];
                        uint32_t less = 0;
                        for (uint32_t g = gs; g < ge; ++g) less += kbuf[1][g] < k ? 1u : 0u;
                        kk[e] = k;
                        ps[e] = gs + less;
                        cn[e] = vbuf[0][vbuf[1][p]];
                    }
                    f[e] = p < n ? k5_idf<BYDF>(a, kk[e]) : 0.0;
                }
#pragma unroll
                for (int e = 0; e < K5L_EB; ++e) {
                    if (p0 + NT * e + tid < n) {
                        const uint64_t o = ob + ps[e];
                        sto(&a.out_term[o], (uint32_t)(kk[e]));
                        sto(&a.out_cnt[o], (uint32_t)(cn[e]));
// ... 69 lines not shown
    if (threadIdx.x < 3) c3[threadIdx.x] = 0u;
    __syncthreads();
    const uint32_t i = blockIdx.x * 256u + threadIdx.x;
    const uint32_t c = k5_class(a, i);
    if (c >= 1u && c <= 3u) atomicAdd(&c3[c - 1u], 1u);
    if (c == 4u) {
        const uint32_t n = gload(a.meta + (i)).z & 0x3FFFFFFFu;
        const uint32_t nt = (n + K5_PS_SPLIT - 1) / K5_PS_SPLIT;
        const uint32_t b = atomicAdd(a.split_count, nt);
        for (uint32_t k = 0; k < nt; ++k) {
            if (b + k < a.split_cap) a.split_tasks[b + k] = make_uint2(i, k);
            else atomicOr(a.status, ST_BOUNDS);
        }
    }
    __syncthreads();
    if (threadIdx.x < 3) a.cls_off[threadIdx.x * a.cls_nblk + blockIdx.x] = c3[threadIdx.x];
    if (blockIdx.x == 0 && threadIdx.x == 3) a.cls_off[3 * a.cls_nblk] = 0u;
}
__global__ __launch_bounds__(256) void k_k5_scatter(K5Args a) {
    __shared__ uint32_t wc[4][3];
    const uint32_t i = blockIdx.x * 256u + threadIdx.x, lane = threadIdx.x & 63, w = threadIdx.x >> 6;
    const uint32_t c = k5_class(a, i);
    uint32_t rk = 0;
#pragma unroll
    for (uint32_t k = 1; k <= 3; ++k) {
        const uint64_t m = __ballot(c == k);
        if (lane == 0) wc[w][k - 1] = (uint32_t)__popcll(m);
        if (c == k) rk = (uint32_t)__popcll(m & ((1ull << lane) - 1ull));
    }
    __syncthreads();
    if (c >= 1u && c <= 3u) {
        uint32_t base = G(a.cls_off)[(c - 1) * a.cls_nblk + blockIdx.x];
        for (uint32_t q = 0; q < w; ++q) base += wc[q][c - 1];
        a.cls_list[base + rk] = i;
    }
}

struct K5SDoc {
    uint64_t rb, ob;
    uint32_t n;
    bool presorted;
    double ds;
};
__device__ __forceinline__ void k5s_batch(const K5Args& a, const uint32_t* L, uint32_t d, uint32_t d1, uint4& m,
                                          uint64_t& ob) {
    m = make_uint4(0, 0, 0, 0);
    ob = 0;
    if (d < d1) {
        const uint32_t i = G(L)[d];
        m = gload(a.meta + i);
        ob = G(a.out_off)[i];
    }
}
template <bool BYDF>
__global__ __launch_bounds__(256, K5S_OCC) void k_score_small(K5Args a) {
    __shared__ __attribute__((aligned(16))) uint32_t kb[K5S_WG][K5_SMALL_DOC + 4];
    __shared__ uint4 bm[K5S_WG][64];
    __shared__ uint64_t bo[K5S_WG][64];
    constexpr int Q = K5_SMALL_DOC / 64;
    const uint32_t w = threadIdx.x >> 6, lane = threadIdx.x & 63;
    uint32_t* buf = kb[w];
    const uint32_t nsmall = G(a.cls_off)[a.cls_nblk];
    const uint32_t nw = gridDim.x * K5S_WG, wid = blockIdx.x * K5S_WG + w;
    const uint32_t per = (nsmall + nw - 1) / nw;
    const uint32_t d0 = wid * per;
    const uint32_t d1 = d0 + per < nsmall ? d0 + per : nsmall;
    if (d0 >= d1) return;
    const uint32_t cnt = d1 - d0;
    const uint32_t* L = a.cls_list;
    uint4 mnxt;
    uint64_t onxt;
    k5s_batch(a, L, d0 + lane, d1, mnxt, onxt);
    bm[w][lane] = mnxt;
    bo[w][lane] = onxt;
    k5s_batch(a, L, d0 + 64 + lane, d1, mnxt, onxt);
    __builtin_amdgcn_fence(__ATOMIC_RELEASE, "wavefront");
    __builtin_amdgcn_fence(__ATOMIC_ACQUIRE, "wavefront");
    uint32_t curb = 0;
    auto doc_at = [&](uint32_t k) -> K5SDoc {
        K5SDoc d;
        if (k >= cnt) { d.rb = 0; d.ob = 0; d.n = 0; d.presorted = true; d.ds = 1.0; return d; }
        const int l = (int)(k & 63u);
        uint32_t mx, my, mz, mw, olo, ohi;
        if ((k >> 6) == curb) {
            const uint4 m = bm[w][l];
            const uint64_t o = bo[w][l];
            mx = __builtin_amdgcn_readfirstlane(m.x); my = __builtin_amdgcn_readfirstlane(m.y);
            mz = __builtin_amdgcn_readfirstlane(m.z); mw = __builtin_amdgcn_readfirstlane(m.w);
            olo = __builtin_amdgcn_readfirstlane((uint32_t)o);
            ohi = __builtin_amdgcn_readfirstlane((uint32_t)(o >> 32));
        } else {
            mx = __builtin_amdgcn_readlane(mnxt.x, l); my = __builtin_amdgcn_readlane(mnxt.y, l);
            mz = __builtin_amdgcn_readlane(mnxt.z, l); mw = __builtin_amdgcn_readlane(mnxt.w, l);
            olo = __builtin_amdgcn_readlane((uint32_t)onxt, l);
            ohi = __builtin_amdgcn_readlane((uint32_t)(onxt >> 32), l);
        }
        d.rb = ((uint64_t)my << 32) | mx;
        d.ob = ((uint64_t)ohi << 32) | olo;
        d.n = mz & 0x3FFFFFFFu;
        d.presorted = ((mz >> 30) & DF_PRESORTED) != 0;
        d.ds = (double)mw;
        if (d.n > K5_SMALL_DOC || d.rb + d.n > a.rec_total) {
            if (lane == 0) atomicOr(a.status, ST_BOUNDS);
            d.n = 0;
        }
        return d;
    };
    auto load_rec = [&](const K5SDoc& d, uint32_t (&r)[Q], uint32_t (&c)[Q]) {
#pragma unroll
        for (int q = 0; q < Q; ++q) {
            const uint32_t j = 64u * q + lane;
            const bool v = j < d.n;
            r[q] = v ? a.rec_slot[d.rb + j] : 0xFFFFFFFFu;
            c[q] = v ? a.rec_cnt[d.rb + j] : 0u;
        }
    };
    auto load_idf = [&](const K5SDoc& d, uint32_t (&r)[Q], double (&f)[Q]) {
#pragma unroll
        for (int q = 0; q < Q; ++q) {
            const bool v = 64u * q + lane < d.n;
            if (v) r[q] = k5_rank(a, r[q]);
            f[q] = v ? k5_idf<BYDF>(a, r[q]) : 0.0;
        }
    };
    K5SDoc D0 = doc_at(0), D1 = doc_at(1);
    uint32_t r0[Q], c0[Q], r1[Q], c1[Q];
    double f0[Q];
    load_rec(D0, r0, c0);
    load_rec(D1, r1, c1);
    load_idf(D0, r0, f0);
    for (uint32_t k = 0; k < cnt; ++k) {
        if (k && (k & 63u) == 0u) {
            bm[w][lane] = mnxt;
            bo[w][lane] = onxt;
            __builtin_amdgcn_fence(__ATOMIC_RELEASE, "wavefront");
            __builtin_amdgcn_fence(__ATOMIC_ACQUIRE, "wavefront");
            ++curb;
            k5s_batch(a, L, d0 + 64u * (curb + 1) + lane, d1, mnxt, onxt);
        }
        const K5SDoc D2 = doc_at(k + 2);
        uint32_t r2[Q], c2[Q];
        double f1[Q];
        load_rec(D2, r2, c2);
        load_idf(D1, r1, f1);
        const uint32_t n = D0.n;
        uint32_t pos[Q];
#pragma unroll
        for (int q = 0; q < Q; ++q) pos[q] = 64u * q + lane;
        if (!D0.presorted && n > 1u) {
#pragma unroll
            for (int q = 0; q < Q; ++q) {
                const uint32_t j = 64u * q + lane;
                if (j < n) buf[j] = r0[q];
            }
            const uint32_t n4 = (n + 3u) & ~3u;
            if (lane < 4u && n + lane < n4) buf[n + lane] = 0xFFFFFFFFu;
            __builtin_amdgcn_fence(__ATOMIC_RELEASE, "wavefront");
            __builtin_amdgcn_fence(__ATOMIC_ACQUIRE, "wavefront");
#pragma unroll
            for (int q = 0; q < Q; ++q) pos[q] = 0u;
            const uint4* k4p = reinterpret_cast<const uint4*>(buf);
            for (uint32_t i4 = 0; i4 < n4 / 4u; ++i4) {
                const uint4 k4 = k4p[i4];
#pragma unroll
                for (int q = 0; q < Q; ++q)
                    pos[q] += (k4.x < r0[q] ? 1u : 0u) + (k4.y < r0[q] ? 1u : 0u) + (k4.z < r0[q] ? 1u : 0u) +
                              (k4.w < r0[q] ? 1u : 0u);
            }
            __builtin_amdgcn_fence(__ATOMIC_RELEASE, "wavefront");
            __builtin_amdgcn_fence(__ATOMIC_ACQUIRE, "wavefront");
        }
#pragma unroll
        for (int q = 0; q < Q; ++q) {
            if (64u * q + lane < n) {
                const uint64_t o = D0.ob + pos[q];
                sto(&a.out_term[o], (uint32_t)(r0[q]));
                sto(&a.out_cnt[o], (uint32_t)(c0[q]));
                sto(&a.out_score[o], (double)(((double)c0[q] / D0.ds) * f0[q]));
            }
        }
        D0 = D1;
        D1 = D2;
#pragma unroll
        for (int q = 0; q < Q; ++q) {
            r0[q] = r1[q]; c0[q] = c1[q]; f0[q] = f1[q];
            r1[q] = r2[q]; c1[q] = c2[q];
        }
    }
}
template <bool BYDF>
__global__ __launch_bounds__(256) void k_emit_split(K5Args a) {
    const uint32_t nt = *a.split_count < a.split_cap ? *a.split_count : a.split_cap;
    for (uint32_t t = blockIdx.x; t < nt; t += gridDim.x) {
        const uint2 tk = a.split_tasks[t];
        const uint4 m = gload(a.meta + tk.x);
        const uint32_t n = m.z & 0x3FFFFFFFu;
        const uint64_t rb = ((uint64_t)m.y << 32) | m.x;
        const uint64_t ob = G(a.out_off)[tk.x];
        const double ds = (double)m.w;
        if (rb + n > a.rec_total) { if (threadIdx.x == 0) atomicOr(a.status, ST_BOUNDS); continue; }
        const uint32_t j1 = (tk.y + 1) * K5_PS_SPLIT < n ? (tk.y + 1) * K5_PS_SPLIT : n;
        for (uint32_t j0 = tk.y * K5_PS_SPLIT; j0 < j1; j0 += 256 * K5L_EB) {
            uint32_t rk[K5L_EB], cn[K5L_EB];
            double f[K5L_EB];
#pragma unroll
            for (int e = 0; e < K5L_EB; ++e) {
                const uint32_t j = j0 + 256u * e + threadIdx.x;
                rk[e] = j < j1 ? a.rec_slot[rb + j] : 0u;
                cn[e] = j < j1 ? a.rec_cnt[rb + j] : 0u;
            }
#pragma unroll
            for (int e = 0; e < K5L_EB; ++e) {
                const uint32_t j = j0 + 256u * e + threadIdx.x;
                if (j < j1) rk[e] = k5_rank(a, rk[e]);
                f[e] = j < j1 ? k5_idf<BYDF>(a, rk[e]) : 0.0;
            }
#pragma unroll
            for (int e = 0; e < K5L_EB; ++e) {
                const uint32_t j = j0 + 256u * e + threadIdx.x;
                if (j < j1) {
                    sto(&a.out_term[ob + j], (uint32_t)(rk[e]));
                    sto(&a.out_cnt[ob + j], (uint32_t)(cn[e]));
                    sto(&a.out_score[ob + j], (double)(((double)cn[e] / ds) * f[e]));
                }
            }
        }
    }
}
static void launch_score_wave(const K5Args& a, bool wide, uint32_t wg, hipStream_t s) {
    if (!wide) k_score_wave<false, false><<<wg, NT, 0, s>>>(a);
    else if (a.idf_by_df) k_score_wave<true, true><<<wg, NT, 0, s>>>(a);
    else k_score_wave<true, false><<<wg, NT, 0, s>>>(a);
}
static void launch_emit_split(const K5Args& a, int ncu, hipStream_t s) {
    if (a.idf_by_df) k_emit_split<true><<<(unsigned)ncu * 4u, 256, 0, s>>>(a);
    else k_emit_split<false><<<(unsigned)ncu * 4u, 256, 0, s>>>(a);
}
static void launch_score_large(const K5Args& a, uint32_t grid, hipStream_t s) {
    static_assert(K5_MAX % 2 == 0 && K5_MAX / 2 >= 1024, "k_score_large instances");
    if (a.idf_by_df) {
        k_score_large<(uint32_t)K5_MAX / 2, 10, true><<<grid, NT, 0, s>>>(a);
        k_score_large<(uint32_t)K5_MAX, 11, true><<<grid, NT, 0, s>>>(a);
    } else {
        k_score_large<(uint32_t)K5_MAX / 2, 10, false><<<grid, NT, 0, s>>>(a);
        k_score_large<(uint32_t)K5_MAX, 11, false><<<grid, NT, 0, s>>>(a);
    }
}
int launch_score_order(const K5Args& a, Arena& ar, hipStream_t s, hipStream_t s2, hipEvent_t ev_fork,
                       hipEvent_t ev_join, uint32_t ncu_ctx) {
    if (!a.ndocs) return 0;
    {
        FillList fl{};
        fl.p[0] = a.large_count;
        fl.bytes[0] = 4;
        fl.n = 1;
        if (a.split_count) {
            fl.p[1] = a.split_count;
            fl.bytes[1] = 4;
            fl.n = 2;
        }
        if (launch_fill_multi(fl, s)) return -1;
    }
    if (!a.idf_by_df)
        k_idf_of_rank<<<grid_for(a.nterms ? a.nterms : 1), NT, 0, s>>>(a.df_of_rank, a.idf_idx, a.idf, a.nterms,
                                                                      a.idf_rank);
    static int ncu_dev = 0;
    if (!ncu_ctx && !ncu_dev) {
        int dev = 0;
        if (hipGetDevice(&dev) != hipSuccess ||
            hipDeviceGetAttribute(&ncu_dev, hipDeviceAttributeMultiprocessorCount, dev) != hipSuccess || ncu_dev <= 0)
            ncu_dev = 256;
    }
    const int ncu = ncu_ctx ? (int)ncu_ctx : ncu_dev;
    const uint32_t wg_need = (a.ndocs + NT / 64 - 1) / (NT / 64);
    const bool wide = a.rank_bits + K5_IDX_BITS > 32;
    const uint32_t wg_cu = wide ? (uint32_t)K5_WPS_WIDE : 4u;
    const uint32_t wg = wg_need < (uint32_t)ncu * wg_cu ? wg_need : (uint32_t)ncu * wg_cu;
    const uint32_t grid = a.ndocs < 2048u ? a.ndocs : 2048u;
    K5Args hand = a;
    hand.cls_list = nullptr;
    if (!a.cls_list || !a.cls_off) return -1;
    k_k5_classify<<<a.cls_nblk, 256, 0, s>>>(a);
    if (scan_excl_u32(a.cls_off, a.cls_off, 3ull * a.cls_nblk + 1, ar, s)) return -1;
    k_k5_scatter<<<a.cls_nblk, 256, 0, s>>>(a);
    if (a.idf_by_df && !wide) return -1;
    if (a.idf_by_df) k_score_small<true><<<(unsigned)ncu * (unsigned)K5S_OCC, 256, 0, s>>>(a);
    else k_score_small<false><<<(unsigned)ncu * (unsigned)K5S_OCC, 256, 0, s>>>(a);
    launch_score_wave(a, wide, wg, s);
    if (a.split_count) launch_emit_split(a, ncu, s);
    launch_score_large(a, grid, s);
    if (wide) launch_score_large(hand, grid, s);
    return ok();
}


__global__ void k_keys_by_rank(const uint4* __restrict__ vkeys, const uint32_t* __restrict__ slot_of_rank, uint32_t V,
                               uint4* __restrict__ out) {
    uint32_t r = blockIdx.x * blockDim.x + threadIdx.x;
    if (r < V) out[r] = vkeys[slot_of_rank[r]];
}
int launch_keys_by_rank(const uint4* vkeys, const uint32_t* slot_of_rank, uint32_t V, uint4* out, hipStream_t s) {
    if (!V) return 0;
    k_keys_by_rank<<<grid_for(V), NT, 0, s>>>(vkeys, slot_of_rank, V, out);
    return ok();
}
__device__ __forceinline__ uint32_t owner_of(const uint4 k, uint32_t R) {
    const uint64_t lo = ((uint64_t)k.y << 32) | k.x, hi = ((uint64_t)k.w << 32) | k.z;
    const uint64_t h = mix64(lo ^ (hi * 0x9E3779B97F4A7C15ull) ^ 0x5851F42D4C957F2Dull);
    return (uint32_t)(((h >> 32) * (uint64_t)R) >> 32);
}
constexpr uint32_t XO_MAXR = 1024;
__device__ __forceinline__ uint4 owner_key(const OwnerKeySrc& ks, uint32_t i) {
    const uint4 s = gload(ks.skey + i);
    const uint32_t b15 = s.x & 0xFFu;
    if (b15 == 0x00u || b15 == 0x09u)
        return make_uint4(__builtin_bswap32(s.w), __builtin_bswap32(s.z), __builtin_bswap32(s.y), __builtin_bswap32(s.x));
    return gload(ks.vkeys + G(ks.slot_of_rank)[i]);
}
__global__ void k_owner_count(const OwnerKeySrc ks, uint32_t V, uint32_t R, uint32_t* __restrict__ cnt) {
    __shared__ uint32_t h[XO_MAXR];
    for (uint32_t o = threadIdx.x; o < R; o += blockDim.x) h[o] = 0;
    __syncthreads();
    for (uint32_t r = blockIdx.x * blockDim.x + threadIdx.x; r < V; r += gridDim.x * blockDim.x)
        atomicAdd(&h[owner_of(owner_key(ks, r), R)], 1u);
    __syncthreads();
    for (uint32_t o = threadIdx.x; o < R; o += blockDim.x)
        if (h[o]) atomicAdd(&cnt[o], h[o]);
}
__global__ void k_owner_scatter(const OwnerKeySrc ks, const uint32_t* __restrict__ df, uint32_t V, uint32_t R,
                                const uint32_t* __restrict__ cnt, uint32_t* __restrict__ cur, uint32_t* __restrict__ srec,
                                uint32_t* __restrict__ sidx) {
    __shared__ uint32_t h[XO_MAXR], base[XO_MAXR], seg[XO_MAXR];
    if (threadIdx.x == 0) {
        uint32_t acc = 0;
        for (uint32_t o = 0; o < R; ++o) { seg[o] = acc; acc += cnt[o]; }
    }
    for (uint32_t o = threadIdx.x; o < R; o += blockDim.x) h[o] = 0;
    __syncthreads();
    const uint32_t r0 = blockIdx.x * blockDim.x * 8;
    uint32_t own[8], pos[8];
// ... 704 lines not shown
```

parallel-systems-mpi-tfidf_amd/csrc/kernels.h:

```cpp
#ifndef TFIDF_KERNELS_H
#define TFIDF_KERNELS_H

#include <hip/hip_runtime.h>
#include <stdint.h>

#include "prims.h"

#define K1_NT        256
#define K1_WIN       (K1_NT * 16)
#ifndef CHUNK_BYTES
#define CHUNK_BYTES  12288u
#endif
#ifndef CHUNK_BYTES_ST
#define CHUNK_BYTES_ST 24576u
#endif
#ifndef DENSE_DOC
#define DENSE_DOC    (4ull << 20)
#endif
#define BIG_LIST_CAP 4096u
#define DENSE_REP    16u
#ifndef BIG_DOC
#define BIG_DOC      49152u
#endif
#ifndef K5_MAX_PAIRS
// ... 35 lines not shown
struct CorpusDev {
    const uint8_t* bytes;
    uint64_t nbytes;
    const uint64_t* doc_off;
    uint32_t ndocs;
    uint64_t lo, hi;
};

struct VocabDev {
    uint4* keys;
    uint64_t* rep;
    uint64_t mask;
};

struct K1Out {
    uint32_t* rec_slot;
    uint32_t* rec_cnt;
    unsigned long long* rec_alloc;
    uint64_t rec_cap;
    uint32_t* part_doc;
    uint32_t* part_slot;
    uint32_t* part_cnt;
    unsigned long long* part_alloc;
    uint64_t part_cap;
    uint64_t* doc_recoff;
    uint32_t* doc_npairs;
    uint32_t* doc_size;
    uint8_t* doc_flags;
    uint32_t* status;
    unsigned long long* ntokens;
    unsigned long long* chunk_ctr;
    unsigned long long* chunk_shard;
    unsigned long long* stamps;
};
#define K1_NSTAMP 17
#define K1_NCOUNT 4
#define K1_STAMP_WORDS (K1_NSTAMP + 1 + K1_NCOUNT)
#define K1_DEBUG_WORDS 16384

int launch_plan_chunks(const CorpusDev& c, uint64_t nchunks, uint32_t chunk_bytes, uint64_t* chunk_start,
                       uint32_t* chunk_doc, uint32_t* big_list, unsigned long long* big_ctr, hipStream_t s);
int launch_tokcount(const CorpusDev& c, const uint64_t* chunk_start, const uint32_t* chunk_doc,
                    uint64_t c0, uint64_t c1, const VocabDev& v, const K1Out& o, hipStream_t s);

int launch_tokcount_vs(const CorpusDev& c, const uint64_t* chunk_start, const uint32_t* chunk_doc, uint64_t c0,
                       uint64_t c1, const VocabDev& v, const K1Out& o, hipStream_t s, uint32_t ncu = 0,
                       uint32_t* grid = nullptr);
#define K1_VS_MAX_CAP (1ull << 28)

#define K1_ST_MAX_CAP (1ull << 22)
#define K1_SL_MAX_CAP (1ull << 25)
int launch_tokcount_sl(const CorpusDev& c, const uint64_t* chunk_start, const uint32_t* chunk_doc, uint64_t c0,
                       uint64_t c1, const VocabDev& v, const K1Out* o_dev, hipStream_t s, uint32_t ncu = 0,
                       uint32_t* grid = nullptr);


int launch_vocab_flags(const VocabDev& v, uint64_t cap, uint32_t* flags, hipStream_t s);
int launch_vocab_compact(const VocabDev& v, uint64_t cap, const uint32_t* dense_of_slot, const CorpusDev& c,
                         uint32_t* vslot, uint4* sortkey, uint32_t* seq, hipStream_t s);
int launch_sortkey_half(const uint4* k, uint64_t n, const uint32_t* seq, int hi, uint64_t* out, hipStream_t s);
int launch_gather_u128(const uint4* k, const uint32_t* seq, uint64_t n, uint4* out, hipStream_t s);
constexpr int FILL_MAX = 8;
struct FillList {
    void* p[FILL_MAX];
    uint64_t bytes[FILL_MAX];
    uint32_t val[FILL_MAX];
    uint32_t n;
};
int launch_fill_multi(const FillList& l, hipStream_t s);
constexpr int WORDS_MAX = 16;
struct WordList {
    const void* src[WORDS_MAX];
    uint32_t bytes[WORDS_MAX];
    uint32_t n;
    uint64_t token;
};
int launch_words_to_host(const WordList& l, uint64_t* host_dst, hipStream_t s);
int launch_vocab_rank(const uint32_t* sorted_dense, const uint32_t* vslot, uint32_t V, uint32_t* rank_of_slot,
                      uint32_t* slot_of_rank, uint16_t* rank16, hipStream_t s);
int launch_vocab_prefix_ties(const uint64_t* sorted_hi, uint32_t* sorted_dense, const uint4* skey, uint32_t V,
                             uint32_t low_mask, Arena& ar, hipStream_t s);
int launch_vocab_long_fixup(const uint4* sorted_keys, uint32_t* sorted_dense, const uint32_t* vslot,
                            const VocabDev& v, const CorpusDev& c, uint32_t V, Arena& ar, hipStream_t s);

int launch_part_keys(const uint32_t* part_doc, const uint32_t* part_slot, const uint32_t* rank_of_slot, uint64_t n,
                     uint64_t* keys, uint32_t* seq, hipStream_t s);
int launch_part_heads(const uint64_t* keys, uint64_t n, uint32_t* head, hipStream_t s);
int launch_part_merge(const uint64_t* keys, const uint32_t* seq, const uint32_t* part_cnt, const uint32_t* head_pos,
                      uint64_t n, const uint32_t* slot_of_rank, uint64_t rec_base, uint32_t* rec_slot,
                      uint32_t* rec_cnt, uint64_t* doc_recoff, uint32_t* doc_npairs, uint8_t* doc_flags,
                      hipStream_t s);
int launch_part_dense(const uint32_t* part_doc, const uint32_t* part_slot, const uint32_t* part_cnt, uint64_t q,
                      const uint32_t* big_idx, const uint32_t* rank_of_slot, uint32_t V, uint32_t* dense,
                      uint64_t* keys, uint32_t* seq, uint32_t* cnt_out, uint32_t* nkeep, hipStream_t s);
int launch_set_big_idx(const uint32_t* big_list, uint32_t nb, uint32_t* big_idx, hipStream_t s);
int launch_dense_emit(const uint32_t* dense, uint32_t nb, uint32_t V, const uint32_t* big_list,
                      const uint32_t* slot_of_rank, uint64_t rec_base, uint32_t* merged_count, uint32_t* tile_cnt,
                      uint32_t* rec_slot, uint32_t* rec_cnt, uint64_t* doc_recoff, uint32_t* doc_npairs,
                      uint8_t* doc_flags, Arena& ar, hipStream_t s);

int launch_df_hist(uint32_t* rec_slot, uint64_t nrec, const uint32_t* nrec_extra, uint64_t nrec_max,
                   const uint32_t* rank_of_slot, const uint16_t* rank16, uint32_t V, uint64_t slot_cap,
                   uint32_t* status, uint32_t* df, Arena& ar, hipStream_t s, bool accumulate = false);
size_t df_hist_scratch(uint64_t nrec_max, uint32_t V);
int launch_df_mark(const uint32_t* df, uint32_t V, uint32_t* present, hipStream_t s);
int launch_df_list(const uint32_t* present_scan, uint64_t nvals, uint32_t* vals, hipStream_t s);

int launch_doc_keys(const uint32_t* doc_ids, uint32_t ndocs, uint64_t* keys, uint32_t* seq, hipStream_t s);
int launch_gather_meta(const uint32_t* order, const uint32_t* doc_npairs, const uint64_t* doc_recoff,
                       const uint32_t* doc_size, const uint8_t* doc_flags, uint32_t ndocs, uint64_t* npairs_ord,
                       uint4* meta, hipStream_t s);
struct K5Args {
    const uint32_t* order;
    const uint4* meta;
    const uint64_t* out_off;
    const uint64_t* doc_recoff;
    const uint32_t* doc_npairs;
    const uint32_t* doc_size;
    const uint8_t* doc_flags;
    const uint32_t* rec_slot;
    const uint32_t* rec_cnt;
    const uint32_t* rank_of_slot;
    const uint32_t* df_of_rank;
    const uint32_t* idf_idx;
    const double* idf;
    double* idf_rank;
    uint32_t* large_list;
    uint32_t* large_count;
    uint32_t* cls_list;
    uint32_t* cls_off;
    uint32_t cls_nblk;
    uint2* split_tasks;
    uint32_t* split_count;
    uint32_t split_cap;
    uint32_t ndocs;
    uint32_t nterms;
    uint32_t rank_bits;
    uint32_t idf_by_df;
    uint64_t rec_total;
    uint64_t slot_cap;
    uint32_t* status;
    uint32_t* out_term;
    uint32_t* out_cnt;
    double* out_score;
};
int launch_score_order(const K5Args& a, Arena& ar, hipStream_t s, hipStream_t s2, hipEvent_t ev_fork,
                       hipEvent_t ev_join, uint32_t ncu = 0);

int launch_keys_by_rank(const uint4* vkeys, const uint32_t* slot_of_rank, uint32_t V, uint4* out, hipStream_t s);
struct OwnerKeySrc {
    const uint4* skey;
    const uint32_t* slot_of_rank;
    const uint4* vkeys;
};
int launch_owner_partition(const OwnerKeySrc& ks, const uint32_t* df, uint32_t V, uint32_t R, uint32_t* cnt, uint32_t* cur,
                           uint32_t* srec, uint32_t* sidx, hipStream_t s);
int launch_owner_offsets(const uint32_t* m, uint32_t R, uint32_t me, uint32_t* soff, uint32_t* roff, hipStream_t s);
int launch_owner_aggregate(const uint32_t* rrec, uint64_t n, const uint32_t* roff, uint32_t R, uint4* tkey, uint64_t tcap,
                           uint32_t* tdf, uint32_t* rslot, uint32_t* reply, unsigned long long* used, uint32_t* status,
                           hipStream_t s);
size_t owner_bucket_scratch(uint64_t n);
int launch_owner_aggregate_buckets(const uint32_t* rrec, uint64_t n, const uint32_t* roff, uint32_t R, void* scratch,
                                   size_t scratch_bytes, uint32_t* reply, unsigned long long* used, uint32_t* status,
                                   uint32_t stage_max, hipStream_t s);
int launch_owner_back(const uint32_t* back, const uint32_t* soff, uint32_t R, const uint32_t* sidx, uint32_t V,
                      uint32_t* df_global, uint32_t* vg, hipStream_t s);
int launch_sum_rows_u32(const uint32_t* rows, uint32_t nrows, uint64_t n, uint32_t* out, hipStream_t s);
#define XCOPY_MAX 64
struct XCopyList {
    const uint32_t* src[XCOPY_MAX];
    uint32_t* dst[XCOPY_MAX];
    uint64_t off[XCOPY_MAX + 1];
    uint32_t n;
};
int launch_xcopy(const XCopyList& l, hipStream_t s);
int launch_xsum_slice(const XCopyList& l, uint64_t lo, uint64_t len, uint32_t* out, hipStream_t s);
int launch_dense_ids(const uint4* gkeys, uint64_t n, uint4* tkey, uint32_t* tpos, uint64_t tcap,
                     unsigned long long* used, uint32_t* status, hipStream_t s);
int launch_dense_scatter(const uint4* mine, const uint32_t* df, uint32_t V, const uint4* tkey, uint64_t tcap,
                         const uint32_t* tpos, uint32_t* pos, uint32_t* dense, uint32_t* status, hipStream_t s);
int launch_dense_gather(const uint32_t* dense, const uint32_t* pos, uint32_t V, uint32_t* df_global, hipStream_t s);
int launch_dense_merge_ids(const uint4* gkeys, uint64_t maxv, uint32_t R, uint32_t me, uint32_t V, uint32_t* lbm,
                           const uint32_t* df, uint64_t sumv, uint32_t* pos, uint32_t* dense, hipStream_t s);

struct LongEnt {
    uint4 key;
    uint32_t len, pad;
    uint64_t boff;
};
int launch_long_list(const uint4* vkeys, const uint64_t* vrep, const uint32_t* slot_of_rank, uint32_t V, LongEnt* ents,
                     uint64_t* src, unsigned long long* cnt, hipStream_t s);
int launch_long_bytes(const LongEnt* ents, const uint64_t* src, uint32_t n, const uint8_t* bytes, uint8_t* blob,
                      hipStream_t s);
int launch_long_verify(const LongEnt* g, uint64_t n, uint64_t lcap, const uint8_t* gblob, uint64_t bcap, uint4* tkey,
                       uint32_t* tpos, uint64_t tcap, uint32_t* status, hipStream_t s);

struct SynSpecDev;
// ... 723 lines not shown
```

parallel-systems-mpi-tfidf_amd/csrc/tokcount_sl.hip:

```cpp
#include "dev_common.h"
#include "dev_vocab.h"
#include "kernels.h"

#if defined(SL_ABL_NOVOCAB) || defined(SL_ABL_NOCOUNT) || defined(SL_ABL_NOROUNDS) || defined(SL_ABL_NOWRITE) || \
    defined(SL_ABL_NOALLOC) || defined(SL_ABL_L2C)
#define SL_ABL 1
#else
#define SL_ABL 0
#endif
#ifdef SL_ABL_NOALLOC
#define SL_ABL_ST 0
#else
#define SL_ABL_ST SL_ABL
#endif

namespace {

#ifndef SL_NT
#define SL_NT 256
#endif
constexpr int NT = SL_NT;
constexpr int NWAVE = NT / 64;
#ifndef SL_WGCU
#define SL_WGCU 4
// ... 162 lines not shown
    return 0u;
}

__device__ __noinline__ uint32_t resolve_slow(const uint8_t* __restrict__ bytes, uint4* keys, uint64_t* reps,
                                              uint64_t mask, uint32_t* status, uint32_t kind, uint32_t k0,
                                              uint32_t k1, uint32_t k2, uint32_t k3, uint64_t p0, uint64_t dend) {
    if (kind == 1u)
        return vocab_insert_s(keys, reps, mask, ((uint64_t)k1 << 32) | k0, ((uint64_t)k3 << 32) | k2, 0, status);
    uint64_t p = p0;
    while (p < dend && !is_ws(bytes[p])) ++p;
    uint64_t n = 0;
    while (p0 + n < p && bytes[p0 + n] != 0) ++n;
    uint64_t klo, khi;
    if (n < 16) {
        uint64_t lo = 0, hi = 0;
        for (uint32_t k = 0; k < n; ++k) {
            const uint64_t b = bytes[p0 + k];
            if (k < 8) lo |= b << (8 * k); else hi |= b << (8 * (k - 8));
        }
        make_short_key(lo, hi, (uint32_t)n, &klo, &khi);
        return vocab_insert_s(keys, reps, mask, klo, khi, 0, status);
    }
    make_long_key(bytes + p0, n, &klo, &khi);
    if (n > 0xFFFFFFull) atomicOr(status, ST_TERM_LONG);
    const uint64_t rep = ((n < 0xFFFFFFull ? n : 0xFFFFFFull) << 40) | p0;
    return vocab_insert_s(keys, reps, mask, klo, khi, rep, status, bytes);
}

__device__ __forceinline__ void wave_agg_add(uint32_t* ctr, uint32_t idx) {
    const uint32_t i0 = (uint32_t)__builtin_amdgcn_readfirstlane((int)idx);
    const uint64_t am = __ballot(1);
    if (__ballot(idx != i0) == 0ull) {
        if (__builtin_amdgcn_mbcnt_hi((uint32_t)(am >> 32), __builtin_amdgcn_mbcnt_lo((uint32_t)am, 0u)) == 0u)
            atomicAdd(&ctr[i0], (uint32_t)__popcll(am));
    } else {
        atomicAdd(&ctr[idx], 1u);
    }
}
__device__ __forceinline__ uint32_t wave_agg_add_rtn(uint32_t* ctr, uint32_t idx) {
    const uint32_t i0 = (uint32_t)__builtin_amdgcn_readfirstlane((int)idx);
    const uint64_t am = __ballot(1);
    uint32_t k;
    if (__ballot(idx != i0) == 0ull) {
        const uint32_t rank = __builtin_amdgcn_mbcnt_hi((uint32_t)(am >> 32), __builtin_amdgcn_mbcnt_lo((uint32_t)am, 0u));
        uint32_t b = 0;
        if (rank == 0u) b = atomicAdd(&ctr[i0], (uint32_t)__popcll(am));
        k = (uint32_t)__builtin_amdgcn_readfirstlane((int)b) + rank;
    } else {
        k = atomicAdd(&ctr[idx], 1u);
    }
    return k;
}

__device__ __forceinline__ void sl_write_staged(SlShared& S, const K1Out* o, uint32_t gd0, uint32_t sb, uint32_t nrec,
                                                uint32_t npart, unsigned long long rb, unsigned long long pb,
                                                bool rec_ok, bool part_ok) {
    const int tid = threadIdx.x;
    uint32_t* const rec_slot = o->rec_slot;
    uint32_t* const rec_cnt = o->rec_cnt;
    uint32_t* const part_doc = o->part_doc;
    uint32_t* const part_slot = o->part_slot;
    uint32_t* const part_cnt = o->part_cnt;
    const uint32_t smask = (1u << sb) - 1u;
    lds_barrier();
    if (rec_ok && !SL_ABL_ST)
        for (uint32_t i = (uint32_t)tid; i < nrec; i += NT) {
            gmem(rec_slot)[rb + i] = S.TK[i] & smask;
            gmem(rec_cnt)[rb + i] = S.TC[i];
        }
    if (part_ok && !SL_ABL_ST)
        for (uint32_t i = (uint32_t)tid; i < npart; i += NT) {
            const uint32_t k = S.TK[nrec + i];
            gmem(part_doc)[pb + i] = gd0 + ((k & 0x7FFFFFFFu) >> sb);
            gmem(part_slot)[pb + i] = k & smask;
            gmem(part_cnt)[pb + i] = S.TC[nrec + i];
        }
    lds_barrier();
    uint4* t = reinterpret_cast<uint4*>(S.TK);
#pragma unroll
    for (int j = tid; j < 2 * TB / 4; j += NT) t[j] = make_uint4(0, 0, 0, 0);
}

__device__ __forceinline__ void sl_flush(SlShared& S, const K1Out* o, uint32_t gd0, uint32_t ng, uint32_t sb) {
    const int tid = threadIdx.x;
    lds_barrier();
    if (tid < GCAP) { S.f.dcnt[tid] = 0; S.f.drun[tid] = 0; }
    lds_barrier();
    uint32_t ek[EPT], ec[EPT];
#pragma unroll
    for (int j = 0; j < EPT; ++j) {
        ek[j] = S.TK[j * NT + tid];
        ec[j] = S.TC[j * NT + tid];
        if (ek[j]) wave_agg_add(&S.f.dcnt[0], (ek[j] & 0x7FFFFFFFu) >> sb);
    }
    lds_barrier();
    uint32_t packed = 0;
    if ((uint32_t)tid < ng) {
        uint8_t st = 0;
        const uint32_t cnt = S.f.dcnt[tid];
        const bool part = S.dpart[tid] != 0;
        if (cnt) {
            const bool complete = !part && S.dfull[tid] && cnt <= (uint32_t)K5_MAX_PAIRS;
            st = complete ? 2 : 1;
            packed = complete ? cnt : (cnt << 16);
        }
        if ((st == 1 || part) && !SL_ABL) gmem(o->doc_flags)[gd0 + tid] = DF_PARTIAL;
        S.f.dstate[tid] = st;
    }
    uint32_t tot;
    const uint32_t off = block_excl_scan<NT, true>(packed, S.wsum, &tot);
    if ((uint32_t)tid < ng) S.f.doff[tid] = off;
    const uint32_t nrec = tot & 0xFFFFu, npart = tot >> 16;
    if (tid == 0) {
        const unsigned long long rb = (nrec && !SL_ABL) ? gatomic_add(o->rec_alloc, (unsigned long long)nrec) : 0ull;
        if (rb + nrec > o->rec_cap) atomicOr(o->status, ST_REC_FULL);
        S.rec_base = rb;
    } else if (tid == 64) {
        const unsigned long long pb = (npart && !SL_ABL) ? gatomic_add(o->part_alloc, (unsigned long long)npart) : 0ull;
        if (pb + npart > o->part_cap) atomicOr(o->status, ST_PART_FULL);
        S.part_base = pb;
    }
    lds_barrier();
    const unsigned long long rb = S.rec_base, pb = S.part_base;
    const bool rec_ok = rb + nrec <= o->rec_cap, part_ok = pb + npart <= o->part_cap;
    if ((uint32_t)tid < ng && S.f.dstate[tid] == 2) {
        gmem(o->doc_recoff)[gd0 + tid] = rb + (off & 0xFFFFu);
        gmem(o->doc_npairs)[gd0 + tid] = SL_ABL ? 0u : S.f.dcnt[tid];
    }
#pragma unroll
    for (int j = 0; j < EPT; ++j) {
        const uint32_t key = ek[j];
        if (key) {
            const uint32_t rel = (key & 0x7FFFFFFFu) >> sb;
            const uint32_t k = wave_agg_add_rtn(&S.f.drun[0], rel);
            const uint32_t dof = S.f.doff[rel];
            const uint32_t loc = (S.f.dstate[rel] == 2 ? (dof & 0xFFFFu) : nrec + (dof >> 16)) + k;
            S.TK[loc] = key;
            S.TC[loc] = ec[j];
        }
    }
    sl_write_staged(S, o, gd0, sb, nrec, npart, rb, pb, rec_ok, part_ok);
}

constexpr uint32_t FEW = 8;
#ifdef SL_STAMPS
#define SLF_STAMP(k)                                                        \
    do {                                                                    \
        const unsigned long long t_ = __builtin_amdgcn_s_memtime();         \
        st_acc[k] += t_ - st_t;                                             \
        st_t = t_;                                                          \
    } while (0)
#define SLF_ARGS , unsigned long long* st_acc, unsigned long long& st_t
#else
#define SLF_STAMP(k) do {} while (0)
#define SLF_ARGS
#endif
__device__ __forceinline__ void sl_flush_few(SlShared& S, const K1Out* o, uint32_t gd0, uint32_t ng, uint32_t sb SLF_ARGS) {
    const int tid = threadIdx.x;
    const int lane = tid & 63, w = tid >> 6;
    lds_barrier();
    uint32_t ek[EPT], ec[EPT];
    uint32_t c4 = 0;
#pragma unroll
    for (int j = 0; j < EPT; ++j) {
        ek[j] = S.TK[j * NT + tid];
        ec[j] = S.TC[j * NT + tid];
        c4 += (ek[j] >> 31) << (4u * ((ek[j] & 0x7FFFFFFFu) >> sb));
    }
    static_assert(EPT < 16 && FEW == 8, "4-bit per-document entry counts of eight documents");
    uint32_t pk[FEW / 2], inc[FEW / 2];
#pragma unroll
    for (uint32_t q = 0; q < FEW / 2; ++q) {
        pk[q] = ((c4 >> (8u * q)) & 15u) | (((c4 >> (8u * q + 4u)) & 15u) << 16);
        inc[q] = wave_incl_scan(pk[q]);
        if (lane == 63) S.q.wtot[w * (FEW / 2) + q] = inc[q];
    }
    SLF_STAMP(9);
    lds_barrier();
    uint32_t rank[FEW / 2], tot[FEW / 2];
#pragma unroll
    for (uint32_t q = 0; q < FEW / 2; ++q) {
        uint32_t base = 0, t = 0;
#pragma unroll
        for (int k = 0; k < NWAVE; ++k) {
            const uint32_t x = S.q.wtot[k * (FEW / 2) + q];
            base += k < w ? x : 0u;
            t += x;
        }
        rank[q] = base + inc[q] - pk[q];
        tot[q] = t;
    }
    if (w == 0) {
        const uint32_t d = (uint32_t)lane;
        uint32_t cnt = 0, packed = 0;
        uint8_t st = 0;
        if (d < ng) {
#pragma unroll
            for (uint32_t q = 0; q < FEW / 2; ++q)
                if ((d >> 1) == q) cnt = (tot[q] >> (16 * (d & 1u))) & 0xFFFFu;
            const bool part = S.dpart[d] != 0;
            if (cnt) {
                const bool complete = !part && S.dfull[d] && cnt <= (uint32_t)K5_MAX_PAIRS;
                st = complete ? 2 : 1;
                packed = complete ? cnt : (cnt << 16);
            }
            if ((st == 1 || part) && !SL_ABL) gmem(o->doc_flags)[gd0 + d] = DF_PARTIAL;
        }
        const uint32_t incl = wave_incl_scan(packed);
        const uint32_t all = (uint32_t)__builtin_amdgcn_readlane((int)incl, 63);
        const uint32_t off = incl - packed;
        const uint32_t nrec = all & 0xFFFFu, npart = all >> 16;
        unsigned long long a0 = 0, a1 = 0;
        if (lane == 0 && nrec && !SL_ABL) a0 = gatomic_add(o->rec_alloc, (unsigned long long)nrec);
        if (lane == 32 && npart && !SL_ABL) a1 = gatomic_add(o->part_alloc, (unsigned long long)npart);
        const unsigned long long rb = ((unsigned long long)(uint32_t)__builtin_amdgcn_readlane((int)(a0 >> 32), 0) << 32) |
                                      (uint32_t)__builtin_amdgcn_readlane((int)(uint32_t)a0, 0);
        const unsigned long long pb = ((unsigned long long)(uint32_t)__builtin_amdgcn_readlane((int)(a1 >> 32), 32) << 32) |
                                      (uint32_t)__builtin_amdgcn_readlane((int)(uint32_t)a1, 32);
        const bool rec_ok = rb + nrec <= o->rec_cap, part_ok = pb + npart <= o->part_cap;
        if (lane == 0 && !rec_ok) atomicOr(o->status, ST_REC_FULL);
        if (lane == 0 && !part_ok) atomicOr(o->status, ST_PART_FULL);
        if (d < ng && st == 2) {
            gmem(o->doc_recoff)[gd0 + d] = rb + (off & 0xFFFFu);
            gmem(o->doc_npairs)[gd0 + d] = SL_ABL ? 0u : cnt;
        }
        if (d < FEW) S.lbase[d] = d >= ng ? 0u : (st == 2 ? (off & 0xFFFFu) : nrec + (off >> 16));
        if (lane == 0) {
            S.fl_nrec = nrec;
            S.fl_npart = npart;
            S.rec_base = rec_ok ? rb : ~0ull;
            S.part_base = part_ok ? pb : ~0ull;
        }
    }
    lds_barrier();
    SLF_STAMP(10);
    {
        const uint4 lb0 = *reinterpret_cast<const uint4*>(&S.lbase[0]);
        const uint4 lb1 = *reinterpret_cast<const uint4*>(&S.lbase[4]);
        S.q.lrank[tid] = make_uint4(rank[0] + (lb0.x | (lb0.y << 16)), rank[1] + (lb0.z | (lb0.w << 16)),
                                    rank[2] + (lb1.x | (lb1.y << 16)), rank[3] + (lb1.z | (lb1.w << 16)));
    }
    const uint16_t* const lr16 = reinterpret_cast<const uint16_t*>(&S.q.lrank[tid]);
    uint32_t run = 0;
#pragma unroll
    for (int j = 0; j < EPT; ++j) {
        const uint32_t key = ek[j];
        if (key) {
            const uint32_t rel4 = 4u * ((key & 0x7FFFFFFFu) >> sb);
            const uint32_t loc = (uint32_t)lr16[rel4 >> 2] + ((run >> rel4) & 15u);
            run += 1u << rel4;
            S.TK[loc] = key;
            S.TC[loc] = ec[j];
        }
    }
    const unsigned long long rb = S.rec_base, pb = S.part_base;
    sl_write_staged(S, o, gd0, sb, S.fl_nrec, S.fl_npart, rb, pb, rb != ~0ull, pb != ~0ull);
}

#ifdef SL_STAMPS
#define SL_STC , st_cnt
#define SL_STC_ARG , unsigned long long* st_cnt
#else
#define SL_STC
#define SL_STC_ARG
#endif
template <bool FAST> __device__ __forceinline__ bool claims_over(SlShared& S, uint32_t wclaims) {
    if (wclaims < WAVE_CLAIMS) return false;
    if (!FAST) return true;
    const uint32_t w = threadIdx.x >> 6;
    uint32_t sum = wclaims;
#pragma unroll
    for (uint32_t k = 0; k < (uint32_t)NWAVE; ++k)
        sum += k == w ? 0u : __hip_atomic_load(&S.wcl[k], __ATOMIC_RELAXED, __HIP_MEMORY_SCOPE_WORKGROUP);
    return sum >= (uint32_t)NWAVE * WAVE_CLAIMS;
}
__device__ __forceinline__ void claims_publish(SlShared& S, uint32_t wclaims) {
    __hip_atomic_store(&S.wcl[threadIdx.x >> 6], wclaims, __ATOMIC_RELAXED, __HIP_MEMORY_SCOPE_WORKGROUP);
}

template <bool FAST>
__device__ __forceinline__ uint32_t lds_count_full(SlShared& S, const K1Out* o, uint32_t key, uint32_t wclaims, uint32_t gd0,
                                                uint32_t sb SL_STC_ARG) {
    const bool over = claims_over<FAST>(S, wclaims);
    const uint32_t b = bkt_hash(key);
    const BktK kk = bkt_read(S.TK, b);
    const bool m0 = kk.a.x == key, m1 = kk.a.y == key, m2 = kk.a.z == key, m3 = kk.a.w == key;
    const bool m4 = kk.b.x == key, m5 = kk.b.y == key, m6 = kk.b.z == key, m7 = kk.b.w == key;
    const uint32_t j = ((m1 | m3 | m5 | m7) ? 1u : 0u) | ((m2 | m3 | m6 | m7) ? 2u : 0u) | ((m4 | m5 | m6 | m7) ? 4u : 0u);
    const bool found = m0 | m1 | m2 | m3 | m4 | m5 | m6 | m7;
    const uint32_t pref = bkt_pref(key);
    uint32_t occ = bkt_occ(kk);
    const uint32_t n = bkt_pick(occ, pref);
    const bool hit = key != 0u && found;
    const bool claim = key != 0u && !found && n < BW && !over;
    const uint32_t idx = bkt_slot(b, found ? j : (n & (BW - 1u)));
    const uint32_t old = atomicCAS(&S.TK[idx], hit ? key : (claim ? 0u : 0x7FFFFFFFu), key);
    const bool ok = key != 0u && (old == key || (claim && old == 0u));
    atomicAdd(&S.TC[idx], ok ? 1u : 0u);
    bool claimed = claim && old == 0u;
    bool slow = key != 0u && !ok;
#ifdef SL_STAMPS
    st_cnt[0] += __ballot(slow) != 0ull ? 1u : 0u;
    st_cnt[1] += (uint32_t)__popcll(__ballot(slow));
    st_cnt[2] += (uint32_t)__popcll(__ballot(claim && !ok));
    ++st_cnt[4];
#endif
    uint32_t nn = n;
#pragma unroll
    for (int t = 0; t < 2; ++t) {
// ... 76 lines not shown
#ifdef SL_STAMPS
    ++st_cnt[8];
    st_cnt[9] += (uint32_t)__popcll(__ballot(ok && old != 0u));
    st_cnt[10] += (uint32_t)__popcll(cm);
    st_cnt[11] += (uint32_t)__popcll(sm);
#endif
    if (sm != 0ull) {
        if (slow) pq[npend + __builtin_amdgcn_mbcnt_hi((uint32_t)(sm >> 32), __builtin_amdgcn_mbcnt_lo((uint32_t)sm, 0u))] = key;
        npend += (uint32_t)__popcll(sm);
        if (npend >= 64u) {
            pq_fence();
            npend -= 64u;
            claims_publish(S, wclaims);
            wclaims = lds_count_full<true>(S, o, pq[npend + (threadIdx.x & 63u)], wclaims, gd0, sb SL_STC);
        }
    }
    claims_publish(S, wclaims);
}
template <bool FAST>
__device__ __forceinline__ void lds_drain(SlShared& S, const K1Out* o, uint32_t& wclaims, uint32_t& npend, uint32_t* pq,
                                          uint32_t gd0, uint32_t sb SL_STC_ARG) {
    while (npend) {
        pq_fence();
        const uint32_t m = npend < 64u ? npend : 64u, l = threadIdx.x & 63u;
        npend -= m;
        wclaims = lds_count_full<FAST>(S, o, l < m ? pq[npend + l] : 0u, wclaims, gd0, sb SL_STC);
        claims_publish(S, wclaims);
    }
}

__device__ __forceinline__ uint32_t perm_sel(uint32_t n, uint32_t k) {
    uint32_t s = 0;
    for (uint32_t j = 0; j < 4; ++j) {
        const uint32_t p = 4 * k + j;
        const uint32_t b = p < n ? j : (p == n ? 4u : 12u);
        s |= b << (8 * j);
    }
    return s;
}

struct Round {
    uint32_t k0, k1, k2, k3;
    uint32_t h;
    uint32_t rel, kind;
    int32_t ap;
#ifdef SL_DEBUG
    uint32_t ent;
#endif
    uint4 s0, s1;
};

}

template <bool FAST>
__global__ __launch_bounds__(NT, WG_PER_CU * NT / 256) void k_tokcount_sl(CorpusDev c, const uint64_t* __restrict__ chunk_start,
                                                               const uint32_t* __restrict__ chunk_doc, uint64_t c0,
                                                               uint64_t c1, VocabDev v, const K1Out* __restrict__ o,
                                                               uint32_t sb, uint32_t gcap) {
    __shared__ __attribute__((aligned(16))) SlShared S;
    const int tid = threadIdx.x, lane = tid & 63;
    const int wid = __builtin_amdgcn_readfirstlane(tid >> 6);
    unsigned long long tokens_w = 0;
    bool clean = false;
#ifdef SL_STAMPS
    unsigned long long st_acc[SL_NPH] = {};
    unsigned long long st_t = __builtin_amdgcn_s_memtime(), st_chunks = 0;
    unsigned long long st_cnt[12] = {};
#define SL_STAMP(k)                                                         \
    do {                                                                    \
        const unsigned long long t_ = __builtin_amdgcn_s_memtime();         \
        st_acc[k] += t_ - st_t;                                             \
        st_t = t_;                                                          \
    } while (0)
#else
#define SL_STAMP(k) do {} while (0)
#endif
    if (tid == 0) S.next_chunk = c0 + gatomic_add(o->chunk_ctr, 1ull);
    lds_barrier();
    unsigned long long claim = 0;
    for (uint64_t chunk = (uint64_t)__builtin_amdgcn_readfirstlane((int)(uint32_t)S.next_chunk) |
                          ((uint64_t)__builtin_amdgcn_readfirstlane((int)(uint32_t)(S.next_chunk >> 32)) << 32);
         chunk < c1;) {
    if (tid == 0) claim = c0 + gatomic_add(o->chunk_ctr, 1ull);
    const uint64_t cs = chunk_start[chunk], ce = chunk_start[chunk + 1];
    const uint32_t dfirst = chunk_doc[chunk], dlast = chunk_doc[chunk + 1];
#ifdef SL_STAMPS
    ++st_chunks;
#endif
    if (cs < ce) {

    const uint64_t b0 = cs & ~(uint64_t)15;
    const uint64_t rb = b0 >= 16 ? b0 - 16 : 0;
    const int32_t shift = (int32_t)(b0 - rb);
    const uint64_t avail = c.nbytes > rb ? ((c.nbytes - rb + 15) & ~(uint64_t)15) : 0;
    const __amdgpu_buffer_rsrc_t crs = __builtin_amdgcn_make_buffer_rsrc(
        (void*)(c.bytes + rb), 0, (int)(avail < 0x7FFFFFF0ull ? avail : 0x7FFFFFF0ull), RSRC_WORD3);
    const __amdgpu_buffer_rsrc_t vrs = __builtin_amdgcn_make_buffer_rsrc((void*)v.keys, 0, (int)((v.mask + 1) * 16),
                                                                         RSRC_WORD3);
    const int32_t span = (int32_t)(ce - b0);
    const int32_t cs_rel = (int32_t)(cs - b0);
    const int32_t lo_rel = c.lo > b0 ? (c.lo - b0 > (uint64_t)span ? span : (int32_t)(c.lo - b0)) : -64;
    const int32_t hi_rel = c.hi - b0 > (uint64_t)span + 64 ? span + 64 : (int32_t)(c.hi - b0);

    const uint32_t ng0 = (dlast + 1 - dfirst) < gcap ? (dlast + 1 - dfirst) : gcap;
    const uint64_t dpre = (uint32_t)tid <= ng0 ? c.doc_off[dfirst + tid] : 0ull;
    uint4 pf = bload16<2>(crs, wid * WSTEP + 16 * lane - 16 + shift);
    if (!clean) {
// ... 193 lines not shown
                        }
                    } else {
                        uint32_t sm = starts, idx = incl - nmine;
                        while (sm) {
                            const uint32_t i = __builtin_ctz(sm);
                            sm &= sm - 1;
                            if (idx - tb < (uint32_t)TLW) {
                                const uint32_t e = ((stop32 >> i) & ~1u) | (nul32 >> i);
                                const uint32_t len = e ? (uint32_t)__builtin_ctz(e) : LEN_LONG;
                                uint32_t rel = base;
                                if (ds & ((2u << i) - 1u))
                                    while (rel + 1 < ng && S.gdoc[rel + 1] <= gpos + (int32_t)i) ++rel;
                                tl[idx - tb] = ((uint32_t)lane << 4 | i) | ((len < 16u ? len : LEN_LONG) << 10) | (rel << 16);
                                if (multi) atomicAdd(&S.dsz[rel], 1u);
                            }
                            ++idx;
                        }
                    }
                    __builtin_amdgcn_fence(__ATOMIC_RELEASE, "wavefront");
                    __builtin_amdgcn_wave_barrier();
                    __builtin_amdgcn_fence(__ATOMIC_ACQUIRE, "wavefront");
                    const uint32_t cnt = (ntok - tb) < (uint32_t)TLW ? (ntok - tb) : (uint32_t)TLW;
                    SL_STAMP(2);
                    for (uint32_t t = 0; t < cnt;) {
                        const uint32_t m = (64u - fill) < (cnt - t) ? (64u - fill) : (cnt - t);
                        if ((uint32_t)lane >= fill && (uint32_t)lane < fill + m) {
                            const uint32_t e = tl[t + (uint32_t)lane - fill];
                            build(acc, e, sbp);
                        }
                        t += m;
                        fill += m;
                        if (fill == 64u) {
                            SL_STAMP(3);
                            turn();
                            SL_STAMP(4);
                        }
                    }
                    __builtin_amdgcn_fence(__ATOMIC_RELEASE, "wavefront");
                    __builtin_amdgcn_wave_barrier();
                    __builtin_amdgcn_fence(__ATOMIC_ACQUIRE, "wavefront");
                }
            }
        }
        SL_STAMP(3);
        if (fill) turn();
        finish(pend);
        lds_drain<FAST>(S, o, wclaims, npend, pq, gd0, sb SL_STC);
#ifdef SL_STAMPS
        SL_STAMP(5);
        lds_barrier();
        SL_STAMP(7);
#endif
#ifdef SL_STAMPS
        if (ng <= FEW) sl_flush_few(S, o, gd0, ng, sb, st_acc, st_t);
#else
        if (ng <= FEW) sl_flush_few(S, o, gd0, ng, sb);
#endif
        else sl_flush(S, o, gd0, ng, sb);
        if ((uint32_t)tid < ng) {
            const uint32_t n = S.dsz[tid];
            if (n) {
                if (S.dfull[tid]) gmem(o->doc_size)[gd0 + tid] = n;
                else atomicAdd(&o->doc_size[gd0 + tid], n);
            }
        }
        lds_barrier();
        SL_STAMP(8);
        if (gd0 + gcap < gd0) break;
    }
    }
    if (tid == 0) S.next_chunk = claim;
    lds_barrier();
    chunk = (uint64_t)(uint32_t)__builtin_amdgcn_readfirstlane((int)(uint32_t)S.next_chunk) |
            ((uint64_t)(uint32_t)__builtin_amdgcn_readfirstlane((int)(uint32_t)(S.next_chunk >> 32)) << 32);
    SL_STAMP(6);
    }
    if (lane == 0 && tokens_w) atomicAdd(o->ntokens, tokens_w);
#ifdef SL_STAMPS
    SL_STAMP(6);
    if (lane == 0 && o->stamps) {
        for (int k = 0; k < SL_NPH; ++k) atomicAdd(&o->stamps[k], st_acc[k]);
        atomicAdd(&o->stamps[SL_NPH], st_chunks);
        atomicAdd(&o->stamps[SL_NPH + 1], 1ull);
        for (int k = 0; k < 12; ++k) atomicAdd(&o->stamps[SL_NPH + 2 + k], st_cnt[k]);
    }
#endif
}

int launch_tokcount_sl(const CorpusDev& c, const uint64_t* chunk_start, const uint32_t* chunk_doc, uint64_t c0,
                       uint64_t c1, const VocabDev& v, const K1Out* o_dev, hipStream_t s, uint32_t ncu_ctx,
                       uint32_t* grid_out) {
    if (grid_out) *grid_out = 0;
    if (c1 <= c0) return 0;
    if (v.mask >= (1ull << SLOT_BITS)) return -3;
    static_assert(sizeof(SlShared) * WG_PER_CU <= 163840, "LDS of WG_PER_CU workgroups per CU");
    static_assert(TB % NT == 0 && TB % BW == 0, "table rows");
    const uint32_t sbits = (uint32_t)__builtin_popcountll(v.mask);
    const uint32_t gcap = (1u << (31u - sbits)) >= (uint32_t)GCAP ? (uint32_t)GCAP : (1u << (31u - sbits));
    static int ncu = 0;
    if (!ncu_ctx && !ncu) {
        int dev = 0;
        if (hipGetDevice(&dev) != hipSuccess ||
            hipDeviceGetAttribute(&ncu, hipDeviceAttributeMultiprocessorCount, dev) != hipSuccess || ncu <= 0)
            ncu = 256;
    }
    const uint64_t wgs = (uint64_t)(ncu_ctx ? ncu_ctx : (uint32_t)ncu) * WG_PER_CU;
    const uint64_t grid = (c1 - c0) < wgs ? (c1 - c0) : wgs;
    if (grid_out) *grid_out = (uint32_t)grid;
    if (v.mask + 1 > K1_ST_MAX_CAP)
        k_tokcount_sl<false><<<(unsigned)grid, NT, 0, s>>>(c, chunk_start, chunk_doc, c0, c1, v, o_dev, sbits, gcap);
    else
        k_tokcount_sl<true><<<(unsigned)grid, NT, 0, s>>>(c, chunk_start, chunk_doc, c0, c1, v, o_dev, sbits, gcap);
    return hipGetLastError() == hipSuccess ? 0 : -1;
}
```

parallel-systems-mpi-tfidf_amd/python/tfidf_abi.py:

```python
from __future__ import annotations

import contextlib
import ctypes as C
import os

import numpy as np

PKG_DIR = os.path.dirname(os.path.dirname(os.path.abspath(__file__)))
_VARIANT = os.environ.get("TFIDF_LIB", "")
LIB_PATH = os.path.join(PKG_DIR, "lib", "libtfidf_hip_%s.so" % _VARIANT if _VARIANT else "libtfidf_hip.so")
CLI_PATH = os.path.join(PKG_DIR, "bin", "tfidf")

TFIDF_CORPUS_DEVICE = 1
UNIQUE_ID_BYTES = 128
RUN_K1_VS = 2
RUN_K1_ST = 4
RUN_K1_SL = 8
RUN_XCHG_DENSE = 16
ABI_VERSION = 2

EXPORTS = [
    "tfidf_open", "tfidf_close", "tfidf_strerror", "tfidf_abi_version", "tfidf_comm_unique_id",
    "tfidf_comm_init", "tfidf_run", "tfidf_fetch", "tfidf_result_free", "tfidf_last_run_info", "tfidf_alloc_stats",
    "tfidf_alloc_live", "tfidf_grid_cus",
    "tfidf_stage_name", "tfidf_set_timing", "tfidf_write_output", "tfidf_print_jobs",
    "tfidf_ingest_dir", "tfidf_free", "tfidf_synth_host", "tfidf_synth_device",
    "tfidf_format", "tfidf_copy_text", "tfidf_write_output_gpu", "tfidf_format_f64",
    "tfidf_ingest_dir_device", "tfidf_hbm_probe", "tfidf_group_open", "tfidf_group_size", "tfidf_group_ctx",
    "tfidf_group_run", "tfidf_group_write_output", "tfidf_group_close", "tfidf_plan_dir", "tfidf_plan_free",
    "tfidf_ingest_shard_device", "tfidf_doc_name_order", "tfidf_shard_split", "tfidf_device_count",
    "tfidf_last_output_info", "tfidf_run_totals_get",
    "tfidf_query", "tfidf_hits_free", "tfidf_group_query", "tfidf_last_query_info",
    "tfidf_top_terms", "tfidf_doc_terms_free", "tfidf_group_top_terms", "tfidf_last_terms_info",
    "tfidf_similar", "tfidf_neighbors_free", "tfidf_group_similar", "tfidf_last_similar_info",
    "tfidf_kmeans", "tfidf_clusters_free", "tfidf_last_kmeans_info",
    "tfidf_query_bm25", "tfidf_group_query_bm25", "tfidf_last_bm25_info",
    "tfidf_clauses_check", "tfidf_query_clauses", "tfidf_group_query_clauses", "tfidf_last_clause_info",
    "tfidf_transform", "tfidf_rows_free", "tfidf_group_transform", "tfidf_last_transform_info",
    "tfidf_model_check", "tfidf_model_export", "tfidf_group_model_export", "tfidf_model_import",
    "tfidf_model_save", "tfidf_model_load", "tfidf_model_free", "tfidf_last_model_info",
    "tfidf_analyzer_check", "tfidf_analyze_host", "tfidf_analyze", "tfidf_last_analyze_info",
    "tfidf_stem_porter",
    "tfidf_ngram_check", "tfidf_ngrams_host", "tfidf_ngrams", "tfidf_last_ngram_info",
    "tfidf_prune_check", "tfidf_prune", "tfidf_group_prune", "tfidf_last_prune_info", "tfidf_model_prune",
    "tfidf_weighting_check", "tfidf_reweight", "tfidf_weighting_get", "tfidf_group_reweight",
    "tfidf_last_reweight_info", "tfidf_result_reweight",
    "tfidf_dedup_check", "tfidf_minhash", "tfidf_signatures_free", "tfidf_near_dups", "tfidf_dups_free",
    "tfidf_last_dedup_info", "tfidf_result_minhash", "tfidf_result_near_dups", "tfidf_dedup_groups",
    "tfidf_nb_check", "tfidf_nb_model_free", "tfidf_nb_labels_free", "tfidf_nb_fit", "tfidf_nb_predict",
    "tfidf_nb_predict_rows", "tfidf_nb_export", "tfidf_last_nb_info", "tfidf_result_nb_fit", "tfidf_nb_model_predict",
    "tfidf_match_check", "tfidf_match_terms", "tfidf_term_matches_free", "tfidf_group_match_terms",
    "tfidf_model_match_terms", "tfidf_last_match_info",
    "tfidf_snippets_check", "tfidf_snippets_free", "tfidf_snippet", "tfidf_group_snippet", "tfidf_result_snippet",
    "tfidf_last_snippet_info",
]
QUERY_MAX_K = 1024
RANK_TFIDF = 0
RANK_BM25 = 1
CLAUSE_MAX_TERMS = 4095
CLAUSE_MAX_NOT = 255
TERMS_MAX_K = 1024
SIMILAR_MAX_K = 1024
KMEANS_MAX_K = 256
KMEANS_MAX_TERMS = 64
NO_CLUSTER = 0xFFFFFFFF
NO_POS = 0xFFFFFFFF
E_INVAL = -1
E_STATE = -10
TFIDF_GROUP_LOCAL = 1
# ... 1921 lines not shown
```

Baseline: 342.6.

## Pack per-record term count into slot word to halve record traffic

The tokenizer writes each (slot, count) record as one 32-bit word with the count in the high bits, instead of writing two separate arrays. The DF histogram and the scoring/ordering kernel read the packed word directly and carry the count through the radix sort key, so the rec_cnt gather goes away. When the packing does not fit the vocabulary, an unpack kernel restores the old layout. This cuts global memory writes and reads of record data. It adds overflow marking for large counts and more kernel template variants.

```diff
diff --git a/include/tfidf.h b/include/tfidf.h
--- a/include/tfidf.h
+++ b/include/tfidf.h
@@ -112,6 +112,8 @@
 #define TFIDF_RUN_K1_VS   2u
 #define TFIDF_RUN_K1_ST   4u
 #define TFIDF_RUN_K1_SL   8u
+#define TFIDF_RUN_REC_PACK 32u
+#define TFIDF_RUN_REC_PACK_KEPT 64u
 #define TFIDF_RUN_XCHG_DENSE 16u
 int tfidf_last_run_info(tfidf_ctx* ctx, tfidf_run_info* info);
 typedef struct tfidf_run_totals {
diff --git a/parallel-systems-mpi-tfidf_amd/csrc/engine.cpp b/parallel-systems-mpi-tfidf_amd/csrc/engine.cpp
--- a/parallel-systems-mpi-tfidf_amd/csrc/engine.cpp
+++ b/parallel-systems-mpi-tfidf_amd/csrc/engine.cpp
@@ -155,6 +155,8 @@
     ctx->xb_stage_max = kxb ? (uint32_t)atoi(kxb) : ~0u;
     const char* kds = getenv("TFIDF_DF_SPLIT");
     ctx->df_split = !(kds && !strcmp(kds, "0"));
+    const char* krp = getenv("TFIDF_REC_PACK");
+    ctx->rec_pack = !(krp && !strcmp(krp, "0"));
     const char* kn = getenv("TFIDF_TEST_XNOMEM_RANK");
     ctx->xnomem_rank = kn ? atoi(kn) : -1;
     static_assert(K1_SL_MAX_CAP == 1ull << 25, "knobs.h: TFIDF_SL_MAXCAP's upper bound");
@@ -577,6 +579,9 @@
     ctx->k1_sl = ctx->k1_vs && (ctx->k1_mode == 0 || ctx->k1_mode == 3) &&
                  ctx->vcap <= ctx->sl_maxcap;
     const uint32_t cb = ctx->k1_sl ? (ctx->vcap > K1_ST_MAX_CAP ? CHUNK_BYTES : CHUNK_BYTES_ST) : CHUNK_BYTES;
+    ctx->run_pack = ctx->rec_pack && ctx->k1_sl && ctx->vcap <= K1_ST_MAX_CAP;
+    ctx->run_pack_kept = false;
+    const uint32_t sbits = (uint32_t)__builtin_popcountll(ctx->vcap - 1);
     const uint64_t nchunks = span ? (span + cb - 1) / cb : 0;
     if (ctx->rec_cap == 0) ctx->rec_cap = span / 6 + 4096;
     if (ctx->part_cap == 0) ctx->part_cap = span / 64 + 4096;
@@ -648,7 +653,7 @@
             ctx->k1out_valid = true;
         }
         LCHK(launch_tokcount_sl(c, ctx->chunk_start.as<uint64_t>(), ctx->chunk_doc.as<uint32_t>(), 0, nchunks, vd,
-                                ctx->k1out_dev.as<K1Out>(), s, ctx_ncu(ctx), &k1_wgs));
+                                ctx->k1out_dev.as<K1Out>(), s, ctx_ncu(ctx), &k1_wgs, ctx->run_pack ? 1u : 0u));
     } else if (nchunks && ctx->k1_vs)
         LCHK(launch_tokcount_vs(c, ctx->chunk_start.as<uint64_t>(), ctx->chunk_doc.as<uint32_t>(), 0, nchunks, vd, o, s,
                                 ctx_ncu(ctx), &k1_wgs));
@@ -752,6 +757,10 @@
         const int rc = enqueue_doc_order(ctx, dev_ids, N, ctx->stream2);
         if (rc) return rc;
     }
+    ctx->run_pack_kept = ctx->run_pack && df_keeps_packed(V, sbits);
+    if (ctx->run_pack && !ctx->run_pack_kept)
+        LCHK(launch_rec_unpack(ctx->rec_slot.as<uint32_t>(), ctx->rec_cnt.as<uint32_t>(), R_main, sbits, s));
+    const uint32_t df_pack = ctx->run_pack_kept ? sbits : 0u;
     const bool df_split = ctx->df_split && Q && R_main;
     ENSURE(ctx->df_local, (size_t)V * 4 + 4);
     ENSURE(ctx->df_global, (size_t)V * 4 + 4);
@@ -770,7 +779,8 @@
         HIPCHK(hipEventRecord(ctx->ev_vrank, s));
         HIPCHK(hipStreamWaitEvent(ctx->stream2, ctx->ev_vrank, 0));
         const int dl = launch_df_hist(ctx->rec_slot.as<uint32_t>(), R_main, nullptr, R_main, ctx->rank_of_slot.as<uint32_t>(),
-                                      r16, V, cap, (uint32_t*)(cnt + 3), ctx->df_local.as<uint32_t>(), da, ctx->stream2);
+                                      r16, V, cap, (uint32_t*)(cnt + 3), ctx->df_local.as<uint32_t>(), da, ctx->stream2,
+                                      false, df_pack);
         if (dl == -2) {
             ctx->df_scratch_min = da.peak + da.peak / 2 + 4096;
             return 1;
@@ -883,7 +893,7 @@
     } else {
         LCHK(launch_df_hist(ctx->rec_slot.as<uint32_t>(), R_main, merged_count, R_total,
                             ctx->rank_of_slot.as<uint32_t>(), r16, V, cap, (uint32_t*)(cnt + 3),
-                            ctx->df_local.as<uint32_t>(), ar, s));
+                            ctx->df_local.as<uint32_t>(), ar, s, false, df_pack));
     }
     ctx->run_V = V;
     ctx->run_cap = cap;
@@ -1107,7 +1117,9 @@
     }
     a.ndocs = N;
     a.nterms = V;
-    a.rank_bits = V > 1 ? 32u - (uint32_t)__builtin_clz(V - 1) : 1u;
+    a.rank_bits = k5_rank_bits(V);
+    a.rec_pack = ctx->run_pack_kept ? 1u : 0u;
+    a.pack_cb = ctx->run_pack_kept ? 32u - a.rank_bits : 0u;
     a.rec_total = R_total;
     a.slot_cap = cap;
     a.status = (uint32_t*)(cnt + 3);
@@ -1374,6 +1386,7 @@
     for (int i = 0; i < S_NSTAGES; ++i) info->ms_stage[i] = ctx->ms_stage[i];
     info->nstages = S_NSTAGES;
     info->flags = (ctx->k1_vs ? TFIDF_RUN_K1_VS : 0u) | (ctx->k1_sl ? TFIDF_RUN_K1_SL : 0u) |
+                  (ctx->run_pack ? TFIDF_RUN_REC_PACK : 0u) | (ctx->run_pack_kept ? TFIDF_RUN_REC_PACK_KEPT : 0u) |
                   (ctx->xp && ctx->last_dense ? TFIDF_RUN_XCHG_DENSE : 0u);
     info->device_allocs = g_dev_allocs.load(std::memory_order_relaxed);
     info->device_alloc_bytes = g_dev_alloc_bytes.load(std::memory_order_relaxed);
diff --git a/parallel-systems-mpi-tfidf_amd/csrc/engine_ctx.h b/parallel-systems-mpi-tfidf_amd/csrc/engine_ctx.h
--- a/parallel-systems-mpi-tfidf_amd/csrc/engine_ctx.h
+++ b/parallel-systems-mpi-tfidf_amd/csrc/engine_ctx.h
@@ -89,6 +89,9 @@
     bool idf_early = false;
     bool df_split = true;
     Event ev_vrank, ev_dfmain;
+    bool rec_pack = true;
+    bool run_pack = false;
+    bool run_pack_kept = false;
     DevBuf df_scratch;
     size_t df_scratch_min = 0;
     Arena arena2;
diff --git a/parallel-systems-mpi-tfidf_amd/csrc/finalize.hip b/parallel-systems-mpi-tfidf_amd/csrc/finalize.hip
--- a/parallel-systems-mpi-tfidf_amd/csrc/finalize.hip
+++ b/parallel-systems-mpi-tfidf_amd/csrc/finalize.hip
@@ -661,7 +661,7 @@
 #endif
 constexpr uint32_t DFH_CK = 1u << DFH_CK_BITS;
 __device__ __forceinline__ uint32_t dfh_cslot(uint32_t slot) { return (slot * 0x9E3779B1u) >> (32 - DFH_CK_BITS); }
-template <bool WIDE>
+template <bool WIDE, bool PACK>
 __global__ __launch_bounds__(DFH_NT) void k_df_hist_lds(uint32_t* __restrict__ rec_slot, uint64_t nrec,
                                                         const uint32_t* __restrict__ nrec_extra,
                                                         const uint32_t* __restrict__ rank_of_slot,
@@ -669,7 +669,7 @@
                                                         uint64_t slot_cap, uint64_t ranked_from,
                                                         uint32_t* __restrict__ status, uint64_t per,
                                                         uint32_t* __restrict__ part ,
-                                                        uint32_t* __restrict__ df) {
+                                                        uint32_t* __restrict__ df, uint32_t sbits, uint32_t cb) {
     extern __shared__ __attribute__((aligned(16))) uint32_t bins[];
     const uint32_t W = (V + 1) / 2;
     for (uint32_t k = threadIdx.x; k < W; k += DFH_NT) bins[k] = 0;
@@ -700,11 +700,20 @@
     };
     for (uint32_t j = threadIdx.x; j < nr; j += (uint32_t)DFH_B * DFH_NT) {
         uint32_t sl[DFH_B], r[DFH_B], g[DFH_B];
+        uint32_t pc[PACK ? DFH_B : 1];
         const uint32_t ofs = j * 4u;
 #pragma unroll
         for (int q = 0; q < DFH_B; ++q) {
             const uint32_t v = __builtin_amdgcn_raw_buffer_load_b32(rs, ofs + (uint32_t)q * DFH_NT * 4u, 0, 2 );
             sl[q] = j + (uint32_t)q * DFH_NT < nr ? v : 0xFFFFFFFFu;
+            if constexpr (PACK) {
+                if (j + (uint32_t)q * DFH_NT < rk) {
+                    pc[q] = v >> sbits;
+                    sl[q] = v & ((1u << sbits) - 1u);
+                } else {
+                    pc[q] = 0u;
+                }
+            }
         }
         store_prev();
         uint32_t miss = 0;
@@ -740,7 +749,8 @@
         pvalid = 0;
 #pragma unroll
         for (int q = 0; q < DFH_B; ++q) {
-            rp[q] = r[q];
+            if constexpr (PACK) rp[q] = (r[q] << cb) | pc[q];
+            else rp[q] = r[q];
             pvalid |= sl[q] != 0xFFFFFFFFu && j + (uint32_t)q * DFH_NT < rk ? 1u << q : 0u;
             if (sl[q] == 0xFFFFFFFFu) continue;
             const uint32_t sh = 16 * (r[q] & 1);
@@ -927,7 +937,9 @@
 
 int launch_df_hist(uint32_t* rec_slot, uint64_t nrec, const uint32_t* nrec_extra, uint64_t nrec_max,
                    const uint32_t* rank_of_slot, const uint16_t* rank16, uint32_t V, uint64_t slot_cap,
-                   uint32_t* status, uint32_t* df, Arena& ar, hipStream_t s, bool accumulate) {
+                   uint32_t* status, uint32_t* df, Arena& ar, hipStream_t s, bool accumulate, uint32_t pack_sbits) {
+    if (pack_sbits && !df_keeps_packed(V, pack_sbits)) return -1;
+    const uint32_t pack_cb = 32u - k5_rank_bits(V);
     const uint64_t ranked_from = nrec;
     if (V == 0) return 0;
     if (nrec_max < nrec) nrec_max = nrec;
@@ -943,12 +955,21 @@
         if (!part) return -2;
         if (!accumulate && hipMemsetAsync(df, 0, (size_t)V * 4, s) != hipSuccess) return -1;
         const size_t lds = (size_t)((W + 1) & ~1u) * 4 + (size_t)DFH_CK * 8;
-        if (per > DFH_RECS)
-            k_df_hist_lds<true><<<nparts, DFH_NT, lds, s>>>(rec_slot, nrec, nrec_extra, rank_of_slot, rank16, V,
-                                                            slot_cap, ranked_from, status, per, part, df);
+        if (pack_sbits) {
+            if (per > DFH_RECS)
+                k_df_hist_lds<true, true><<<nparts, DFH_NT, lds, s>>>(rec_slot, nrec, nrec_extra, rank_of_slot, rank16, V,
+                                                                      slot_cap, ranked_from, status, per, part, df,
+                                                                      pack_sbits, pack_cb);
+            else
+                k_df_hist_lds<false, true><<<nparts, DFH_NT, lds, s>>>(rec_slot, nrec, nrec_extra, rank_of_slot, rank16,
+                                                                       V, slot_cap, ranked_from, status, per, part, df,
+                                                                       pack_sbits, pack_cb);
+        } else if (per > DFH_RECS)
+            k_df_hist_lds<true, false><<<nparts, DFH_NT, lds, s>>>(rec_slot, nrec, nrec_extra, rank_of_slot, rank16, V,
+                                                                   slot_cap, ranked_from, status, per, part, df, 0u, 0u);
         else
-            k_df_hist_lds<false><<<nparts, DFH_NT, lds, s>>>(rec_slot, nrec, nrec_extra, rank_of_slot, rank16, V,
-                                                             slot_cap, ranked_from, status, per, part, df);
+            k_df_hist_lds<false, false><<<nparts, DFH_NT, lds, s>>>(rec_slot, nrec, nrec_extra, rank_of_slot, rank16, V,
+                                                                    slot_cap, ranked_from, status, per, part, df, 0u, 0u);
         k_df_colsum<<<dim3(grid_for(V), (nparts + DFC_G - 1) / DFC_G), NT, 0, s>>>(part, nparts, V, df);
         ar.release(m);
         return ok();
@@ -981,6 +1002,30 @@
     return ok();
 }
 
+__global__ void k_rec_unpack(uint32_t* __restrict__ rec_slot, uint32_t* __restrict__ rec_cnt, uint64_t n, uint32_t sbits) {
+    const uint64_t i0 = ((uint64_t)blockIdx.x * blockDim.x + threadIdx.x) * 4ull;
+    const uint32_t smask = (1u << sbits) - 1u;
+    if (i0 + 4 <= n && (((uintptr_t)rec_slot | (uintptr_t)rec_cnt) & 15u) == 0) {
+        const uint4 w = *reinterpret_cast<const uint4*>(rec_slot + i0);
+        *reinterpret_cast<uint4*>(rec_slot + i0) = make_uint4(w.x & smask, w.y & smask, w.z & smask, w.w & smask);
+        *reinterpret_cast<uint4*>(rec_cnt + i0) = make_uint4(w.x >> sbits, w.y >> sbits, w.z >> sbits, w.w >> sbits);
+        return;
+    }
+    for (uint64_t i = i0; i < n && i < i0 + 4; ++i) {
+        const uint32_t w = rec_slot[i];
+        rec_slot[i] = w & smask;
+        rec_cnt[i] = w >> sbits;
+    }
+}
+int launch_rec_unpack(uint32_t* rec_slot, uint32_t* rec_cnt, uint64_t n, uint32_t sbits, hipStream_t s) {
+    if (!n) return 0;
+    if (sbits == 0 || sbits >= 32) return -1;
+    const uint64_t nthreads = (n + 3) / 4, blocks = (nthreads + NT - 1) / NT;
+    if (blocks > 0x7FFFFFFFull) return -1;
+    k_rec_unpack<<<(unsigned)blocks, NT, 0, s>>>(rec_slot, rec_cnt, n, sbits);
+    return ok();
+}
+
 __global__ void k_df_mark(const uint32_t* __restrict__ df, uint32_t V, uint32_t* __restrict__ present) {
     uint32_t r = blockIdx.x * blockDim.x + threadIdx.x;
     if (r < V) present[df[r]] = 1u;
@@ -1093,13 +1138,15 @@
     return n <= K5_SMALL || (n <= K5_WAVE && a.rank_bits <= K5_WIDE_BITS);
 }
 
-__device__ __noinline__ void k5_radix(uint32_t rank_bits, const uint32_t* rec_cnt, const double* idf_rank,
+template <bool PACK>
+__device__ __noinline__ void k5_radix(uint32_t rank_bits, uint32_t lowb, const uint32_t* rec_cnt, const double* idf_rank,
                                       uint32_t* out_term, uint32_t* out_cnt, double* out_score, uint32_t* buf0,
                                       uint32_t* buf1, uint32_t* h, uint32_t n, uint64_t rb, uint64_t ob, double ds) {
     const uint32_t lane = threadIdx.x & 63;
     const uint64_t below = (1ull << lane) - 1ull;
+    if constexpr (!PACK) lowb = K5_IDX_BITS;
     uint32_t cur = 0;
-    for (uint32_t sh = K5_IDX_BITS; sh < K5_IDX_BITS + rank_bits; sh += 8) {
+    for (uint32_t sh = lowb; sh < lowb + rank_bits; sh += 8) {
         const uint32_t* src = cur ? buf1 : buf0;
         uint32_t* dst = cur ? buf0 : buf1;
         h[4 * lane] = 0; h[4 * lane + 1] = 0; h[4 * lane + 2] = 0; h[4 * lane + 3] = 0;
@@ -1153,14 +1200,15 @@
         }
 #pragma unroll
         for (int q = 0; q < K5_BATCH; ++q) {
-            cnt[q] = rec_cnt[rb + (key[q] & ((1u << K5_IDX_BITS) - 1u))];
-            idf[q] = G(idf_rank)[key[q] >> K5_IDX_BITS];
+            if constexpr (PACK) cnt[q] = key[q] & ((1u << lowb) - 1u);
+            else cnt[q] = rec_cnt[rb + (key[q] & ((1u << K5_IDX_BITS) - 1u))];
+            idf[q] = G(idf_rank)[key[q] >> lowb];
         }
 #pragma unroll
         for (int q = 0; q < K5_BATCH; ++q) {
             const uint32_t j = j0 + 64 * q + lane;
             if (j < n) {
-                sto(&out_term[ob + j], (uint32_t)(key[q] >> K5_IDX_BITS));
+                sto(&out_term[ob + j], (uint32_t)(key[q] >> lowb));
                 sto(&out_cnt[ob + j], (uint32_t)(cnt[q]));
                 sto(&out_score[ob + j], (double)(((double)cnt[q] / ds) * idf[q]));
             }
@@ -1170,6 +1218,25 @@
 
 constexpr int K5_PF = 8;
 constexpr int K5_RQ = K5_WAVE / 64;
+#ifndef K5_PF_PACK
+#define K5_PF_PACK K5_RQ
+#endif
+static_assert(K5_PF_PACK >= 1 && K5_PF_PACK <= K5_RQ, "prefetched rows of a packed document");
+template <int PF>
+__device__ __forceinline__ void k5_prefetch_packed(const K5Args& a, const uint4& m, uint32_t lane, uint32_t (&s)[PF]) {
+    const uint32_t n = m.z & 0x3FFFFFFFu;
+    const uint64_t rb = ((uint64_t)m.y << 32) | m.x;
+    const bool ok = n != 0u && n <= K5_WAVE && rb + n <= a.rec_total;
+#pragma unroll
+    for (int q = 0; q < PF; ++q) {
+        const uint32_t j = 64u * q + lane;
+        s[q] = (ok && j < n) ? a.rec_slot[rb + j] : 0u;
+    }
+}
+__device__ __forceinline__ uint32_t k5_word(const K5Args& a, uint32_t w) {
+    if ((w >> a.pack_cb) >= a.nterms) { atomicOr(a.status, ST_BOUNDS); w &= (1u << a.pack_cb) - 1u; }
+    return w;
+}
 __device__ __forceinline__ void k5_prefetch(const K5Args& a, const uint4& m, uint32_t lane, uint32_t (&s)[K5_PF],
                                             uint32_t (&c)[K5_PF]) {
     const uint32_t n = m.z & 0x3FFFFFFFu;
@@ -1190,9 +1257,11 @@
     return l;
 }
 
-template <bool WIDE, bool BYDF>
+template <bool WIDE, bool BYDF, bool PACK>
 __global__ __launch_bounds__(NT, WIDE ? K5_WPS_WIDE : K5_WPS) void k_score_wave(K5Args a) {
     static_assert(WIDE || !BYDF, "idf by df only with wide ranks (V > 2^21; k5_radix reads idf by rank)");
+    static_assert(!(WIDE && PACK), "a packed word needs no index bits: no wide form");
+    constexpr int PF = PACK ? K5_PF_PACK : K5_PF;
     __shared__ __attribute__((aligned(16))) uint32_t kb[NT / 64][2][K5_WAVE];
     __shared__ uint32_t hist[NT / 64][K5_NB];
     const uint32_t w = threadIdx.x >> 6, lane = threadIdx.x & 63;
@@ -1214,8 +1283,10 @@
     uint4 m_cur = li < lcount ? gload(a.meta + (i_cur)) : make_uint4(0, 0, 0, 0);
     uint4 m_nxt = li + stride < lcount ? gload(a.meta + (i_nxt)) : make_uint4(0, 0, 0, 0);
     uint64_t ob_cur = li < lcount ? G(a.out_off)[i_cur] : 0ull;
-    uint32_t s_cur[K5_PF], c_cur[K5_PF];
-    k5_prefetch(a, m_cur, lane, s_cur, c_cur);
+    uint32_t s_cur[PF], c_cur[PACK ? 1 : K5_PF];
+    if constexpr (PACK) k5_prefetch_packed<PF>(a, m_cur, lane, s_cur);
+    else k5_prefetch(a, m_cur, lane, s_cur, c_cur);
+    const uint32_t pcb = PACK ? a.pack_cb : 0u, pcm = (1u << pcb) - 1u;
     for (; li < lcount; li += stride) {
         const uint32_t lane = lane_id_fresh();
         const uint32_t i = i_cur;
@@ -1228,27 +1299,32 @@
         const bool small_doc = n != 0u && k5_by_wave(a, n, presorted) && rb + n <= a.rec_total;
         uint32_t r[K5_RQ];
 #pragma unroll
-        for (int q = 0; q < K5_PF; ++q) {
+        for (int q = 0; q < PF; ++q) {
             const uint32_t j = 64u * q + lane;
-            r[q] = (small_doc && j < n) ? k5_rank(a, s_cur[q]) : 0xFFFFFFFFu;
-            if (small_doc && j < n) buf0[j] = c_cur[q];
-        }
-        if (small_doc && n > 64u * K5_PF) {
-            uint32_t sx[K5_RQ - K5_PF];
-#pragma unroll
-            for (int q = K5_PF; q < K5_RQ; ++q) {
+            if constexpr (PACK) {
+                r[q] = (small_doc && j < n) ? (presorted ? k5_rank(a, s_cur[q]) : k5_word(a, s_cur[q])) : 0xFFFFFFFFu;
+            } else {
+                r[q] = (small_doc && j < n) ? k5_rank(a, s_cur[q]) : 0xFFFFFFFFu;
+                if (small_doc && j < n) buf0[j] = c_cur[q];
+            }
+        }
+        if (PF < K5_RQ && small_doc && n > 64u * PF) {
+            uint32_t sx[PF < K5_RQ ? K5_RQ - PF : 1];
+#pragma unroll
+            for (int q = PF; q < K5_RQ; ++q) {
                 const uint32_t j = 64u * q + lane;
-                sx[q - K5_PF] = j < n ? a.rec_slot[rb + j] : 0u;
-                if (j < n) buf0[j] = a.rec_cnt[rb + j];
-            }
-#pragma unroll
-            for (int q = K5_PF; q < K5_RQ; ++q) {
+                sx[q - PF] = j < n ? a.rec_slot[rb + j] : 0u;
+                if constexpr (!PACK) if (j < n) buf0[j] = a.rec_cnt[rb + j];
+            }
+#pragma unroll
+            for (int q = PF; q < K5_RQ; ++q) {
                 const uint32_t j = 64u * q + lane;
-                r[q] = j < n ? k5_rank(a, sx[q - K5_PF]) : 0xFFFFFFFFu;
+                if constexpr (PACK) r[q] = j < n ? (presorted ? k5_rank(a, sx[q - PF]) : k5_word(a, sx[q - PF])) : 0xFFFFFFFFu;
+                else r[q] = j < n ? k5_rank(a, sx[q - PF]) : 0xFFFFFFFFu;
             }
         } else {
 #pragma unroll
-            for (int q = K5_PF; q < K5_RQ; ++q) r[q] = 0xFFFFFFFFu;
+            for (int q = PF; q < K5_RQ; ++q) r[q] = 0xFFFFFFFFu;
         }
         __builtin_amdgcn_fence(__ATOMIC_RELEASE, "wavefront");
         __builtin_amdgcn_fence(__ATOMIC_ACQUIRE, "wavefront");
@@ -1259,7 +1335,8 @@
             ob_cur = inx < lcount ? G(a.out_off)[i_cur] : 0ull;
             i_nxt = inx + stride < lcount ? pos_of(inx + stride) : 0u;
             m_nxt = inx + stride < lcount ? gload(a.meta + (i_nxt)) : make_uint4(0, 0, 0, 0);
-            k5_prefetch(a, m_cur, lane, s_cur, c_cur);
+            if constexpr (PACK) k5_prefetch_packed<PF>(a, m_cur, lane, s_cur);
+            else k5_prefetch(a, m_cur, lane, s_cur, c_cur);
         }
         if (n == 0) continue;
         if (!k5_by_wave(a, n, presorted)) {
@@ -1271,7 +1348,11 @@
 #pragma unroll
             for (int q = 0; q < K5_RQ; ++q) {
                 const uint32_t j = 64u * q + lane;
-                if (j < n) k5_emit<BYDF>(a, ob + j, ds, r[q], buf0[j]);
+                if constexpr (PACK) {
+                    if (j < n) k5_emit<BYDF>(a, ob + j, ds, r[q], a.rec_cnt[rb + j]);
+                } else {
+                    if (j < n) k5_emit<BYDF>(a, ob + j, ds, r[q], buf0[j]);
+                }
             }
             continue;
         }
@@ -1302,14 +1383,14 @@
             }
             double idf[QC];
 #pragma unroll
-            for (int q = 0; q < QC; ++q) idf[q] = (64u * q + lane < n) ? k5_idf<BYDF>(a, r[q]) : 0.0;
+            for (int q = 0; q < QC; ++q) idf[q] = (64u * q + lane < n) ? k5_idf<BYDF>(a, r[q] >> pcb) : 0.0;
 #pragma unroll
             for (int q = 0; q < QC; ++q) {
                 const uint32_t j = 64u * q + lane;
                 if (j < n) {
                     const uint64_t o = ob + pos[q];
-                    const uint32_t cnt = buf0[j];
-                    sto(&a.out_term[o], (uint32_t)(r[q]));
+                    const uint32_t cnt = PACK ? (r[q] & pcm) : buf0[j];
+                    sto(&a.out_term[o], (uint32_t)(r[q] >> pcb));
                     sto(&a.out_cnt[o], (uint32_t)(cnt));
                     sto(&a.out_score[o], (double)(((double)cnt / ds) * idf[q]));
                 }
@@ -1319,7 +1400,7 @@
             continue;
         }
         if (n <= K5_SMALL) {
-            uint32_t key = r[0], val = lane < n ? buf0[lane] : 0u;
+            uint32_t key = r[0], val = (!PACK && lane < n) ? buf0[lane] : 0u;
 #pragma unroll
             for (uint32_t k = 2; k <= 64; k <<= 1) {
 #pragma unroll
@@ -1329,10 +1410,10 @@
                     if (take_min ? (pk < key) : (pk > key)) { key = pk; val = pv; }
                 }
             }
-            if (lane < n) k5_emit<BYDF>(a, ob + lane, ds, key, val);
+            if (lane < n) k5_emit<BYDF>(a, ob + lane, ds, key >> pcb, PACK ? (key & pcm) : val);
             continue;
         }
-        const uint32_t hsh = a.rank_bits > K5_NB_BITS ? a.rank_bits - K5_NB_BITS : 0u;
+        const uint32_t hsh = PACK ? 32u - K5_NB_BITS : a.rank_bits > K5_NB_BITS ? a.rank_bits - K5_NB_BITS : 0u;
 #pragma unroll
         for (uint32_t q = 0; q < K5_NB / 64; ++q) h[q * 64 + lane] = 0;
         __builtin_amdgcn_fence(__ATOMIC_RELEASE, "wavefront");
@@ -1409,19 +1490,19 @@
 #pragma unroll
             for (int q = 0; q < K5_RQ; ++q) {
                 const uint32_t j = 64u * q + lane;
-                if (j < n) buf0[j] = (r[q] << K5_IDX_BITS) | j;
+                if (j < n) buf0[j] = PACK ? r[q] : (r[q] << K5_IDX_BITS) | j;
             }
             __builtin_amdgcn_fence(__ATOMIC_RELEASE, "wavefront");
             __builtin_amdgcn_fence(__ATOMIC_ACQUIRE, "wavefront");
             if constexpr (!WIDE)
-                k5_radix(a.rank_bits, a.rec_cnt, a.idf_rank, a.out_term, a.out_cnt, a.out_score, buf0, buf1, h, n,
-                         rb, ob, ds);
+                k5_radix<PACK>(a.rank_bits, PACK ? pcb : K5_IDX_BITS, a.rec_cnt, a.idf_rank, a.out_term, a.out_cnt,
+                               a.out_score, buf0, buf1, h, n, rb, ob, ds);
             continue;
         }
 #pragma unroll
         for (int q = 0; q < K5_RQ; ++q) {
             const uint32_t j = 64u * q + lane;
-            if (j < n) buf1[atomicAdd(&h[r[q] >> hsh], 1u)] = (r[q] << K5_IDX_BITS) | j;
+            if (j < n) buf1[atomicAdd(&h[r[q] >> hsh], 1u)] = PACK ? r[q] : (r[q] << K5_IDX_BITS) | j;
         }
         __builtin_amdgcn_fence(__ATOMIC_RELEASE, "wavefront");
         __builtin_amdgcn_fence(__ATOMIC_ACQUIRE, "wavefront");
@@ -1431,7 +1512,7 @@
             const uint32_t j = 64u * q + lane;
             pp[q] = 0u;
             if (j < n) {
-                const uint32_t k = (r[q] << K5_IDX_BITS) | j, d = r[q] >> hsh;
+                const uint32_t k = PACK ? r[q] : (r[q] << K5_IDX_BITS) | j, d = r[q] >> hsh;
                 const uint32_t gs = d ? h[d - 1] : 0u, ge = h[d];
                 uint32_t less = 0;
                 for (uint32_t f = gs; f < ge; ++f) less += buf1[f] < k ? 1u : 0u;
@@ -1442,7 +1523,7 @@
         __builtin_amdgcn_fence(__ATOMIC_ACQUIRE, "wavefront");
 #pragma unroll
         for (int q = 0; q < K5_RQ; ++q)
-            if (64u * q + lane < n) buf1[pp[q]] = (r[q] << K5_IDX_BITS) | (64u * q + lane);
+            if (64u * q + lane < n) buf1[pp[q]] = PACK ? r[q] : (r[q] << K5_IDX_BITS) | (64u * q + lane);
         __builtin_amdgcn_fence(__ATOMIC_RELEASE, "wavefront");
         __builtin_amdgcn_fence(__ATOMIC_ACQUIRE, "wavefront");
         constexpr int EB = K5_EMIT;
@@ -1451,14 +1532,15 @@
 #pragma unroll
             for (int q = 0; q < EB; ++q) {
                 const uint32_t j = j0 + 64 * q + lane;
-                idf[q] = k5_idf<BYDF>(a, (j < n ? buf1[j] : 0u) >> K5_IDX_BITS);
+                idf[q] = k5_idf<BYDF>(a, (j < n ? buf1[j] : 0u) >> (PACK ? pcb : K5_IDX_BITS));
             }
 #pragma unroll
             for (int q = 0; q < EB; ++q) {
                 const uint32_t j = j0 + 64 * q + lane;
                 if (j < n) {
-                    const uint32_t key = buf1[j], cnt = buf0[key & ((1u << K5_IDX_BITS) - 1u)];
-                    sto(&a.out_term[ob + j], (uint32_t)(key >> K5_IDX_BITS));
+                    const uint32_t key = buf1[j];
+                    const uint32_t cnt = PACK ? (key & pcm) : buf0[key & ((1u << K5_IDX_BITS) - 1u)];
+                    sto(&a.out_term[ob + j], (uint32_t)(key >> (PACK ? pcb : K5_IDX_BITS)));
                     sto(&a.out_cnt[ob + j], (uint32_t)(cnt));
                     sto(&a.out_score[ob + j], (double)(((double)cnt / ds) * idf[q]));
                 }
@@ -1469,7 +1551,7 @@
     }
 }
 
-template <uint32_t MAXN, uint32_t NBB, bool BYDF>
+template <uint32_t MAXN, uint32_t NBB, bool BYDF, bool PACK>
 __global__ __launch_bounds__(NT) void k_score_large(K5Args a) {
     constexpr uint32_t NB = 1u << NBB;
     __shared__ uint32_t kbuf[2][MAXN];
@@ -1545,14 +1627,19 @@
         for (int e = 0; e < K5L_EB; ++e) {
             const uint32_t j = j0 + NT * e + tid;
             sl[e] = j < n ? a.rec_slot[rb + j] : 0u;
-            cn[e] = j < n ? a.rec_cnt[rb + j] : 0u;
+            if constexpr (!PACK) cn[e] = j < n ? a.rec_cnt[rb + j] : 0u;
         }
 #pragma unroll
         for (int e = 0; e < K5L_EB; ++e) {
             const uint32_t j = j0 + NT * e + tid;
             if (j < n) {
-                kbuf[0][j] = k5_rank(a, sl[e]);
-                vbuf[0][j] = cn[e];
+                if constexpr (PACK) {
+                    kbuf[0][j] = k5_rank(a, sl[e] >> a.pack_cb);
+                    vbuf[0][j] = sl[e] & ((1u << a.pack_cb) - 1u);
+                } else {
+                    kbuf[0][j] = k5_rank(a, sl[e]);
+                    vbuf[0][j] = cn[e];
+                }
             }
         }
     }
@@ -1728,7 +1815,7 @@
         ob = G(a.out_off)[i];
     }
 }
-template <bool BYDF>
+template <bool BYDF, bool PACK>
 __global__ __launch_bounds__(256, K5S_OCC) void k_score_small(K5Args a) {
     __shared__ __attribute__((aligned(16))) uint32_t kb[K5S_WG][K5_SMALL_DOC + 4];
     __shared__ uint4 bm[K5S_WG][64];
@@ -1788,13 +1875,17 @@
             const uint32_t j = 64u * q + lane;
             const bool v = j < d.n;
             r[q] = v ? a.rec_slot[d.rb + j] : 0xFFFFFFFFu;
-            c[q] = v ? a.rec_cnt[d.rb + j] : 0u;
+            c[q] = (v && (!PACK || d.presorted)) ? a.rec_cnt[d.rb + j] : 0u;
         }
     };
-    auto load_idf = [&](const K5SDoc& d, uint32_t (&r)[Q], double (&f)[Q]) {
+    auto load_idf = [&](const K5SDoc& d, uint32_t (&r)[Q], uint32_t (&c)[Q], double (&f)[Q]) {
 #pragma unroll
         for (int q = 0; q < Q; ++q) {
             const bool v = 64u * q + lane < d.n;
+            if (PACK && v && !d.presorted) {
+                c[q] = r[q] & ((1u << a.pack_cb) - 1u);
+                r[q] >>= a.pack_cb;
+            }
             if (v) r[q] = k5_rank(a, r[q]);
             f[q] = v ? k5_idf<BYDF>(a, r[q]) : 0.0;
         }
@@ -1804,7 +1895,7 @@
     double f0[Q];
     load_rec(D0, r0, c0);
     load_rec(D1, r1, c1);
-    load_idf(D0, r0, f0);
+    load_idf(D0, r0, c0, f0);
     for (uint32_t k = 0; k < cnt; ++k) {
         if (k && (k & 63u) == 0u) {
             bm[w][lane] = mnxt;
@@ -1818,7 +1909,7 @@
         uint32_t r2[Q], c2[Q];
         double f1[Q];
         load_rec(D2, r2, c2);
-        load_idf(D1, r1, f1);
+        load_idf(D1, r1, c1, f1);
         const uint32_t n = D0.n;
         uint32_t pos[Q];
 #pragma unroll
@@ -1904,9 +1995,10 @@
     }
 }
 static void launch_score_wave(const K5Args& a, bool wide, uint32_t wg, hipStream_t s) {
-    if (!wide) k_score_wave<false, false><<<wg, NT, 0, s>>>(a);
-    else if (a.idf_by_df) k_score_wave<true, true><<<wg, NT, 0, s>>>(a);
-    else k_score_wave<true, false><<<wg, NT, 0, s>>>(a);
+    if (a.rec_pack) k_score_wave<false, false, true><<<wg, NT, 0, s>>>(a);
+    else if (!wide) k_score_wave<false, false, false><<<wg, NT, 0, s>>>(a);
+    else if (a.idf_by_df) k_score_wave<true, true, false><<<wg, NT, 0, s>>>(a);
+    else k_score_wave<true, false, false><<<wg, NT, 0, s>>>(a);
 }
 static void launch_emit_split(const K5Args& a, int ncu, hipStream_t s) {
     if (a.idf_by_df) k_emit_split<true><<<(unsigned)ncu * 4u, 256, 0, s>>>(a);
@@ -1914,12 +2006,15 @@
 }
 static void launch_score_large(const K5Args& a, uint32_t grid, hipStream_t s) {
     static_assert(K5_MAX % 2 == 0 && K5_MAX / 2 >= 1024, "k_score_large instances");
-    if (a.idf_by_df) {
-        k_score_large<(uint32_t)K5_MAX / 2, 10, true><<<grid, NT, 0, s>>>(a);
-        k_score_large<(uint32_t)K5_MAX, 11, true><<<grid, NT, 0, s>>>(a);
+    if (a.rec_pack) {
+        k_score_large<(uint32_t)K5_MAX / 2, 10, false, true><<<grid, NT, 0, s>>>(a);
+        k_score_large<(uint32_t)K5_MAX, 11, false, true><<<grid, NT, 0, s>>>(a);
+    } else if (a.idf_by_df) {
+        k_score_large<(uint32_t)K5_MAX / 2, 10, true, false><<<grid, NT, 0, s>>>(a);
+        k_score_large<(uint32_t)K5_MAX, 11, true, false><<<grid, NT, 0, s>>>(a);
     } else {
-        k_score_large<(uint32_t)K5_MAX / 2, 10, false><<<grid, NT, 0, s>>>(a);
-        k_score_large<(uint32_t)K5_MAX, 11, false><<<grid, NT, 0, s>>>(a);
+        k_score_large<(uint32_t)K5_MAX / 2, 10, false, false><<<grid, NT, 0, s>>>(a);
+        k_score_large<(uint32_t)K5_MAX, 11, false, false><<<grid, NT, 0, s>>>(a);
     }
 }
 int launch_score_order(const K5Args& a, Arena& ar, hipStream_t s, hipStream_t s2, hipEvent_t ev_fork,
@@ -1949,7 +2044,8 @@
     }
     const int ncu = ncu_ctx ? (int)ncu_ctx : ncu_dev;
     const uint32_t wg_need = (a.ndocs + NT / 64 - 1) / (NT / 64);
-    const bool wide = a.rank_bits + K5_IDX_BITS > 32;
+    if (a.rec_pack && (a.pack_cb == 0 || a.pack_cb + a.rank_bits != 32 || a.idf_by_df)) return -1;
+    const bool wide = !a.rec_pack && a.rank_bits + K5_IDX_BITS > 32;
     const uint32_t wg_cu = wide ? (uint32_t)K5_WPS_WIDE : 4u;
     const uint32_t wg = wg_need < (uint32_t)ncu * wg_cu ? wg_need : (uint32_t)ncu * wg_cu;
     const uint32_t grid = a.ndocs < 2048u ? a.ndocs : 2048u;
@@ -1960,8 +2056,9 @@
     if (scan_excl_u32(a.cls_off, a.cls_off, 3ull * a.cls_nblk + 1, ar, s)) return -1;
     k_k5_scatter<<<a.cls_nblk, 256, 0, s>>>(a);
     if (a.idf_by_df && !wide) return -1;
-    if (a.idf_by_df) k_score_small<true><<<(unsigned)ncu * (unsigned)K5S_OCC, 256, 0, s>>>(a);
-    else k_score_small<false><<<(unsigned)ncu * (unsigned)K5S_OCC, 256, 0, s>>>(a);
+    if (a.rec_pack) k_score_small<false, true><<<(unsigned)ncu * (unsigned)K5S_OCC, 256, 0, s>>>(a);
+    else if (a.idf_by_df) k_score_small<true, false><<<(unsigned)ncu * (unsigned)K5S_OCC, 256, 0, s>>>(a);
+    else k_score_small<false, false><<<(unsigned)ncu * (unsigned)K5S_OCC, 256, 0, s>>>(a);
     launch_score_wave(a, wide, wg, s);
     if (a.split_count) launch_emit_split(a, ncu, s);
     launch_score_large(a, grid, s);
diff --git a/parallel-systems-mpi-tfidf_amd/csrc/kernels.h b/parallel-systems-mpi-tfidf_amd/csrc/kernels.h
--- a/parallel-systems-mpi-tfidf_amd/csrc/kernels.h
+++ b/parallel-systems-mpi-tfidf_amd/csrc/kernels.h
@@ -111,7 +111,7 @@
 #define K1_SL_MAX_CAP (1ull << 25)
 int launch_tokcount_sl(const CorpusDev& c, const uint64_t* chunk_start, const uint32_t* chunk_doc, uint64_t c0,
                        uint64_t c1, const VocabDev& v, const K1Out* o_dev, hipStream_t s, uint32_t ncu = 0,
-                       uint32_t* grid = nullptr);
+                       uint32_t* grid = nullptr, uint32_t pack = 0);
 
 
 int launch_vocab_flags(const VocabDev& v, uint64_t cap, uint32_t* flags, hipStream_t s);
@@ -158,9 +158,15 @@
                       uint32_t* rec_slot, uint32_t* rec_cnt, uint64_t* doc_recoff, uint32_t* doc_npairs,
                       uint8_t* doc_flags, Arena& ar, hipStream_t s);
 
+static inline uint32_t k5_rank_bits(uint32_t V) { return V > 1 ? 32u - (uint32_t)__builtin_clz(V - 1) : 1u; }
+static inline bool df_keeps_packed(uint32_t V, uint32_t sbits) {
+    return V != 0 && V <= DFH_MAXV && sbits != 0 && sbits < 32 && k5_rank_bits(V) <= sbits;
+}
 int launch_df_hist(uint32_t* rec_slot, uint64_t nrec, const uint32_t* nrec_extra, uint64_t nrec_max,
                    const uint32_t* rank_of_slot, const uint16_t* rank16, uint32_t V, uint64_t slot_cap,
-                   uint32_t* status, uint32_t* df, Arena& ar, hipStream_t s, bool accumulate = false);
+                   uint32_t* status, uint32_t* df, Arena& ar, hipStream_t s, bool accumulate = false,
+                   uint32_t pack_sbits = 0);
+int launch_rec_unpack(uint32_t* rec_slot, uint32_t* rec_cnt, uint64_t n, uint32_t sbits, hipStream_t s);
 size_t df_hist_scratch(uint64_t nrec_max, uint32_t V);
 int launch_df_mark(const uint32_t* df, uint32_t V, uint32_t* present, hipStream_t s);
 int launch_df_list(const uint32_t* present_scan, uint64_t nvals, uint32_t* vals, hipStream_t s);
@@ -202,6 +208,8 @@
     uint32_t* out_term;
     uint32_t* out_cnt;
     double* out_score;
+    uint32_t rec_pack;
+    uint32_t pack_cb;
 };
 int launch_score_order(const K5Args& a, Arena& ar, hipStream_t s, hipStream_t s2, hipEvent_t ev_fork,
                        hipEvent_t ev_join, uint32_t ncu = 0);
diff --git a/parallel-systems-mpi-tfidf_amd/csrc/tokcount_sl.hip b/parallel-systems-mpi-tfidf_amd/csrc/tokcount_sl.hip
--- a/parallel-systems-mpi-tfidf_amd/csrc/tokcount_sl.hip
+++ b/parallel-systems-mpi-tfidf_amd/csrc/tokcount_sl.hip
@@ -238,6 +238,10 @@
     return k;
 }
 
+#ifndef SL_PACK_STAGE
+#define SL_PACK_STAGE 0
+#endif
+template <bool PACK>
 __device__ __forceinline__ void sl_write_staged(SlShared& S, const K1Out* o, uint32_t gd0, uint32_t sb, uint32_t nrec,
                                                 uint32_t npart, unsigned long long rb, unsigned long long pb,
                                                 bool rec_ok, bool part_ok) {
@@ -249,11 +253,17 @@
     uint32_t* const part_cnt = o->part_cnt;
     const uint32_t smask = (1u << sb) - 1u;
     lds_barrier();
-    if (rec_ok && !SL_ABL_ST)
-        for (uint32_t i = (uint32_t)tid; i < nrec; i += NT) {
-            gmem(rec_slot)[rb + i] = S.TK[i] & smask;
-            gmem(rec_cnt)[rb + i] = S.TC[i];
-        }
+    if (rec_ok && !SL_ABL_ST) {
+        if constexpr (PACK) {
+            for (uint32_t i = (uint32_t)tid; i < nrec; i += NT)
+                gmem(rec_slot)[rb + i] = SL_PACK_STAGE ? S.TK[i] : (S.TC[i] << sb) | (S.TK[i] & smask);
+        } else {
+            for (uint32_t i = (uint32_t)tid; i < nrec; i += NT) {
+                gmem(rec_slot)[rb + i] = S.TK[i] & smask;
+                gmem(rec_cnt)[rb + i] = S.TC[i];
+            }
+        }
+    }
     if (part_ok && !SL_ABL_ST)
         for (uint32_t i = (uint32_t)tid; i < npart; i += NT) {
             const uint32_t k = S.TK[nrec + i];
@@ -267,6 +277,19 @@
     for (int j = tid; j < 2 * TB / 4; j += NT) t[j] = make_uint4(0, 0, 0, 0);
 }
 
+template <int N>
+__device__ __forceinline__ void sl_mark_wide(SlShared& S, const uint32_t (&ek)[N], const uint32_t (&ec)[N], uint32_t sb) {
+    const uint32_t lim = 1u << (32u - sb);
+    uint32_t any = 0;
+#pragma unroll
+    for (int j = 0; j < N; ++j) any |= ec[j];
+    if (__ballot(any >= lim) == 0ull) return;
+#pragma unroll
+    for (int j = 0; j < N; ++j)
+        if (ek[j] && ec[j] >= lim) S.dpart[(ek[j] & 0x7FFFFFFFu) >> sb] = 1;
+}
+
+template <bool PACK>
 __device__ __forceinline__ void sl_flush(SlShared& S, const K1Out* o, uint32_t gd0, uint32_t ng, uint32_t sb) {
     const int tid = threadIdx.x;
     lds_barrier();
@@ -279,6 +302,7 @@
         ec[j] = S.TC[j * NT + tid];
         if (ek[j]) wave_agg_add(&S.f.dcnt[0], (ek[j] & 0x7FFFFFFFu) >> sb);
     }
+    if constexpr (PACK) sl_mark_wide(S, ek, ec, sb);
     lds_barrier();
     uint32_t packed = 0;
     if ((uint32_t)tid < ng) {
@@ -321,11 +345,15 @@
             const uint32_t k = wave_agg_add_rtn(&S.f.drun[0], rel);
             const uint32_t dof = S.f.doff[rel];
             const uint32_t loc = (S.f.dstate[rel] == 2 ? (dof & 0xFFFFu) : nrec + (dof >> 16)) + k;
-            S.TK[loc] = key;
-            S.TC[loc] = ec[j];
-        }
-    }
-    sl_write_staged(S, o, gd0, sb, nrec, npart, rb, pb, rec_ok, part_ok);
+            if (PACK && SL_PACK_STAGE && loc < nrec) {
+                S.TK[loc] = (ec[j] << sb) | (key & ((1u << sb) - 1u));
+            } else {
+                S.TK[loc] = key;
+                S.TC[loc] = ec[j];
+            }
+        }
+    }
+    sl_write_staged<PACK>(S, o, gd0, sb, nrec, npart, rb, pb, rec_ok, part_ok);
 }
 
 constexpr uint32_t FEW = 8;
@@ -341,6 +369,7 @@
 #define SLF_STAMP(k) do {} while (0)
 #define SLF_ARGS
 #endif
+template <bool PACK>
 __device__ __forceinline__ void sl_flush_few(SlShared& S, const K1Out* o, uint32_t gd0, uint32_t ng, uint32_t sb SLF_ARGS) {
     const int tid = threadIdx.x;
     const int lane = tid & 63, w = tid >> 6;
@@ -353,6 +382,7 @@
         ec[j] = S.TC[j * NT + tid];
         c4 += (ek[j] >> 31) << (4u * ((ek[j] & 0x7FFFFFFFu) >> sb));
     }
+    if constexpr (PACK) sl_mark_wide(S, ek, ec, sb);
     static_assert(EPT < 16 && FEW == 8, "4-bit per-document entry counts of eight documents");
     uint32_t pk[FEW / 2], inc[FEW / 2];
 #pragma unroll
@@ -427,6 +457,7 @@
                                     rank[2] + (lb1.x | (lb1.y << 16)), rank[3] + (lb1.z | (lb1.w << 16)));
     }
     const uint16_t* const lr16 = reinterpret_cast<const uint16_t*>(&S.q.lrank[tid]);
+    const uint32_t nrec_st = S.fl_nrec;
     uint32_t run = 0;
 #pragma unroll
     for (int j = 0; j < EPT; ++j) {
@@ -435,12 +466,16 @@
             const uint32_t rel4 = 4u * ((key & 0x7FFFFFFFu) >> sb);
             const uint32_t loc = (uint32_t)lr16[rel4 >> 2] + ((run >> rel4) & 15u);
             run += 1u << rel4;
-            S.TK[loc] = key;
-            S.TC[loc] = ec[j];
+            if (PACK && SL_PACK_STAGE && loc < nrec_st) {
+                S.TK[loc] = (ec[j] << sb) | (key & ((1u << sb) - 1u));
+            } else {
+                S.TK[loc] = key;
+                S.TC[loc] = ec[j];
+            }
         }
     }
     const unsigned long long rb = S.rec_base, pb = S.part_base;
-    sl_write_staged(S, o, gd0, sb, S.fl_nrec, S.fl_npart, rb, pb, rb != ~0ull, pb != ~0ull);
+    sl_write_staged<PACK>(S, o, gd0, sb, S.fl_nrec, S.fl_npart, rb, pb, rb != ~0ull, pb != ~0ull);
 }
 
 #ifdef SL_STAMPS
@@ -623,7 +658,7 @@
 
 }
 
-template <bool FAST>
+template <bool FAST, bool PACK>
 __global__ __launch_bounds__(NT, WG_PER_CU * NT / 256) void k_tokcount_sl(CorpusDev c, const uint64_t* __restrict__ chunk_start,
                                                                const uint32_t* __restrict__ chunk_doc, uint64_t c0,
                                                                uint64_t c1, VocabDev v, const K1Out* __restrict__ o,
@@ -923,11 +958,11 @@
         SL_STAMP(7);
 #endif
 #ifdef SL_STAMPS
-        if (ng <= FEW) sl_flush_few(S, o, gd0, ng, sb, st_acc, st_t);
+        if (ng <= FEW) sl_flush_few<PACK>(S, o, gd0, ng, sb, st_acc, st_t);
 #else
-        if (ng <= FEW) sl_flush_few(S, o, gd0, ng, sb);
-#endif
-        else sl_flush(S, o, gd0, ng, sb);
+        if (ng <= FEW) sl_flush_few<PACK>(S, o, gd0, ng, sb);
+#endif
+        else sl_flush<PACK>(S, o, gd0, ng, sb);
         if ((uint32_t)tid < ng) {
             const uint32_t n = S.dsz[tid];
             if (n) {
@@ -960,13 +995,14 @@
 
 int launch_tokcount_sl(const CorpusDev& c, const uint64_t* chunk_start, const uint32_t* chunk_doc, uint64_t c0,
                        uint64_t c1, const VocabDev& v, const K1Out* o_dev, hipStream_t s, uint32_t ncu_ctx,
-                       uint32_t* grid_out) {
+                       uint32_t* grid_out, uint32_t pack) {
     if (grid_out) *grid_out = 0;
     if (c1 <= c0) return 0;
     if (v.mask >= (1ull << SLOT_BITS)) return -3;
     static_assert(sizeof(SlShared) * WG_PER_CU <= 163840, "LDS of WG_PER_CU workgroups per CU");
     static_assert(TB % NT == 0 && TB % BW == 0, "table rows");
     const uint32_t sbits = (uint32_t)__builtin_popcountll(v.mask);
+    if (pack && v.mask + 1 > K1_ST_MAX_CAP) return -1;
     const uint32_t gcap = (1u << (31u - sbits)) >= (uint32_t)GCAP ? (uint32_t)GCAP : (1u << (31u - sbits));
     static int ncu = 0;
     if (!ncu_ctx && !ncu) {
@@ -979,8 +1015,10 @@
     const uint64_t grid = (c1 - c0) < wgs ? (c1 - c0) : wgs;
     if (grid_out) *grid_out = (uint32_t)grid;
     if (v.mask + 1 > K1_ST_MAX_CAP)
-        k_tokcount_sl<false><<<(unsigned)grid, NT, 0, s>>>(c, chunk_start, chunk_doc, c0, c1, v, o_dev, sbits, gcap);
+        k_tokcount_sl<false, false><<<(unsigned)grid, NT, 0, s>>>(c, chunk_start, chunk_doc, c0, c1, v, o_dev, sbits, gcap);
+    else if (pack)
+        k_tokcount_sl<true, true><<<(unsigned)grid, NT, 0, s>>>(c, chunk_start, chunk_doc, c0, c1, v, o_dev, sbits, gcap);
     else
-        k_tokcount_sl<true><<<(unsigned)grid, NT, 0, s>>>(c, chunk_start, chunk_doc, c0, c1, v, o_dev, sbits, gcap);
+        k_tokcount_sl<true, false><<<(unsigned)grid, NT, 0, s>>>(c, chunk_start, chunk_doc, c0, c1, v, o_dev, sbits, gcap);
     return hipGetLastError() == hipSuccess ? 0 : -1;
 }
diff --git a/parallel-systems-mpi-tfidf_amd/python/tfidf_abi.py b/parallel-systems-mpi-tfidf_amd/python/tfidf_abi.py
--- a/parallel-systems-mpi-tfidf_amd/python/tfidf_abi.py
+++ b/parallel-systems-mpi-tfidf_amd/python/tfidf_abi.py
@@ -15,6 +15,8 @@
 UNIQUE_ID_BYTES = 128
 RUN_K1_VS = 2
 RUN_K1_ST = 4
+RUN_REC_PACK = 32
+RUN_REC_PACK_KEPT = 64
 RUN_K1_SL = 8
 RUN_XCHG_DENSE = 16
 ABI_VERSION = 2
```

Measured after the change: 359.9, median of 6. 1.05x the previous value.
